# micahvista/VACmap

Measured on AMD Instinct MI355X. Metric: aligned Gbp/s (whole node) + reads/s, 15 kb ONT-shape reads vs hg38-size ref, 1/2/4/8 MI355X, higher is better.
Workload: dtype i16/i32 DP + f64 chains

## Files before the change

include/vacmapx.h:

```cpp
#ifndef VACMAPX_H
#define VACMAPX_H
#include <stdint.h>
#ifdef __cplusplus
extern "C" {
#endif

typedef enum vm_status {
    VM_OK = 0,
    VM_ERR_ARG = -1,
    VM_ERR_NO_DEVICE = -2,
    VM_ERR_NO_CTX = -3,
    VM_ERR_OOM = -4,
    VM_ERR_IO = -5,
    VM_ERR_HIP = -6,
    VM_ERR_UNSUPPORTED = -7,
    VM_READ_RAISED = -10,
    VM_READ_CAPACITY = -20,
    VM_READ_FASTPATH = -21,
    VM_READ_UNSUPPORTED = -22
} vm_status;

enum { VM_MODE_H = 0, VM_MODE_L = 1, VM_MODE_S = 2, VM_MODE_R = 3,
       VM_MODE_ASM = 4 };

// ... 57 lines not shown
typedef struct vm_chains_out {
    int32_t* need_reverse;
    int32_t* mapq;
    double* score;
    int32_t* fast_used;
    int64_t* read_path_off;
    int64_t* path_off;
    int64_t* path_anchors;
    double* S; int64_t* P; int64_t* S_arg; int64_t* gmax; int64_t* opcount;
} vm_chains_out;
int vm_chain_global_batch(vm_ctx*, const vm_params*, int kmersize, int64_t n, const int64_t* anchors,
                          const int64_t* anchor_off, const int64_t* readlens, int want_raw, vm_chains_out* out);
void vm_chains_out_free(vm_chains_out*);

typedef struct vm_local_out {
    int32_t* status;
    int32_t* variant;
    double* score;
    int64_t* chain_off;
    int64_t* chain;
    int64_t* raw_off;
    int64_t* raw;
} vm_local_out;
int vm_local_chain_batch(vm_ctx*, const vm_index*, const vm_params*, int64_t n, const char* seqs, const int64_t* offsets,
                         const int64_t* read_path_off, const int64_t* path_off, const int64_t* path_anchors, vm_local_out* out);
void vm_local_out_free(vm_local_out*);

typedef struct vm_linked_out {
    int64_t gmax, n_hot, n_cold, opcount; double cold_max;
    double* S; int64_t* P; int64_t* S_arg_hot;
    int32_t carry_status, saved; int64_t n_carry; double* carry_S; int64_t* carry_P; int64_t* carry_rows; double carry_g_max_scores; int64_t carry_prereadloc;
} vm_linked_out;
int vm_chain_linked(vm_ctx*, int which, int kmersize, double skipcost, int maxdiff, int maxgap, int64_t n, const int64_t* rows, int64_t n_pre,
                    const double* pre_S, const int64_t* pre_P, double g_max_scores, int64_t g_max_index, int64_t prereadloc, vm_linked_out* out);
void vm_linked_out_free(vm_linked_out*);

typedef struct vm_score { int32_t match, mismatch, o1, e1, o2, e2; } vm_score;
int vm_k_cigar_batch(vm_ctx*, const vm_score*, int eqx, int64_t n, const char* t, const int64_t* t_off, const char* q,
                     const int64_t* q_off, char** cigars, int64_t** cigar_off, int32_t** scores);
int vm_k_cigar_batch_banded(vm_ctx*, const vm_score*, int eqx, int64_t n, const char* t, const int64_t* t_off, const char* q,
                            const int64_t* q_off, char** cigars, int64_t** cigar_off, int32_t** band_flag, int64_t* stats);
int vm_k_extend_batch(vm_ctx*, int match, int mismatch, int o, int e, int bw, int zdrop, int64_t n, const char* t,
                      const int64_t* t_off, const char* q, const int64_t* q_off, int32_t** t_e, int32_t** q_e, int32_t** score);
typedef struct vm_cigar_out { char* cigar; int32_t q_e, t_e, score; } vm_cigar_out;
int vm_k_cigar(vm_ctx*, const char* t, int64_t tl, const char* q, int64_t ql, const vm_score* sc, int bw, int zdrop,
               int eqx, vm_cigar_out* out);
int vm_edit_distance_batch(vm_ctx*, int64_t n, const char* q, const int64_t* q_off, const char* t, const int64_t* t_off,
                           int64_t** dist);
int64_t vm_edit_distance(vm_ctx*, const char* q, int64_t ql, const char* t, int64_t tl);
int vm_edit_distance_bound_batch(vm_ctx*, int tier, int64_t n, const char* q, const int64_t* q_off, const char* t, const int64_t* t_off,
                                 int64_t** bound);

typedef struct vm_record {
    int32_t read_idx;
    int32_t contig;
    int32_t strand;
    int32_t mapq;
    int64_t q_st, q_en;
    int64_t r_st, r_en;
    int64_t cigar_off, cigar_len;
} vm_record;

typedef struct vm_batch_stats {
    int64_t n_reads, read_bases, n_minimizers, n_hits, n_anchors, n_local_hits, n_local_anchors;
    int64_t n_segments, n_ed_problems, ed_cells, n_ext_problems, ext_cells, n_dp_problems, dp_cells;
    int64_t n_records, cigar_bytes, aligned_bases, n_unmapped, n_failed;
    int64_t dp_string_bytes;
    double ms_total;
    double ms_stage[16];
    double ms_gapfill_fill;
    double ms_gapfill_trace;
    int64_t n_gapfill_launches;
    int64_t n_ed_full;
    int64_t n_ed_tier2;
    int64_t n_ed_tier1;
    int64_t n_dp_redo;
    int64_t dp_redo_tb_bytes;
    double ms_local_seed;
    double ms_cluster;
    int64_t n_host_syncs;
    int64_t n_local_general;
    int64_t n_ext_retries;
    int64_t n_batch_retries;
} vm_batch_stats;

int vm_align_batch(vm_ctx*, const vm_index*, const vm_params*, int64_t n_reads, const char* seqs, const int64_t* offsets,
                   vm_record** recs, int64_t* n_recs, char** cigar_blob, int32_t* status_per_read, vm_batch_stats* stats);
typedef struct vm_reads vm_reads;
int vm_reads_upload(vm_ctx*, int64_t n_reads, const char* seqs, const int64_t* offsets, vm_reads** out);
int vm_reads_reupload(vm_ctx*, vm_reads*, int64_t n_reads, const char* seqs, const int64_t* offsets);
void vm_reads_free(vm_reads*);
int vm_align_resident(vm_ctx*, const vm_index*, const vm_params*, const vm_reads*, vm_record** recs, int64_t* n_recs,
                      char** cigar_blob, int32_t* status_per_read, vm_batch_stats* stats);

int vm_align_asm(vm_ctx*, const vm_index*, const vm_params* p, const char* contig, int64_t len, int64_t split_len, int64_t batch_anchors, int64_t window,
                 vm_record** recs, int64_t* n_recs, char** cigar_blob, int32_t* status);

int vm_align_trace(vm_ctx*, const vm_index*, const vm_params*, int64_t n_reads, const char* seqs, const int64_t* offsets, int stage,
                   int64_t** rows, int64_t** row_off);

typedef struct vm_sam_opts {
    int32_t md, shortcs, cigar2cg, markunbalancetra, hardclip, fakecigar;
    const char* rg_id;
    int32_t asm_mode;
} vm_sam_opts;
int vm_sam_emit(const vm_index*, const vm_sam_opts*, int64_t n_reads, const char* names, const int64_t* name_off, const char* seqs, const int64_t* seq_off,
                const char* quals, const int64_t* qual_off, const char* comments, const int64_t* com_off, const vm_record* recs, int64_t n_recs,
                const char* cigar_blob, const int32_t* status, int nthreads, char** text, int64_t** text_off, int64_t* n_lines, int64_t* n_skipped);
int64_t vm_blob_gather(const char* blob, const int64_t* off, const int64_t* idx, int64_t n, char* out, int64_t* out_off);
int64_t vm_blob_write_parts_mmap(int fd, int64_t file_off, const char* const* blobs, const int64_t* const* offs, const int32_t* part, const int64_t* idx, int64_t n, int nthreads);
int64_t vm_blob_gather_parts(const char* const* blobs, const int64_t* const* offs, const int32_t* part, const int64_t* idx, int64_t n, char* out);
void* vm_pinned_alloc(int64_t bytes, int device);
void vm_pinned_free(void* p);
int64_t vm_blob_write_parts(int fd, const char* const* blobs, const int64_t* const* offs, const int32_t* part, const int64_t* idx, int64_t n);
typedef struct vm_fastx vm_fastx;
int vm_fastx_open(const char* path, vm_fastx** out);
int vm_fastx_open_range(const char* path, int64_t begin, int64_t end, vm_fastx** out);
void vm_fastx_close(vm_fastx*);
int64_t vm_fastx_read(vm_fastx*, int64_t max_reads, int64_t max_bases, char** names, int64_t** name_off, char** seqs, int64_t** seq_off, char** quals,
                      int64_t** qual_off, char** comments, int64_t** com_off);

typedef struct vm_bam_writer vm_bam_writer;
int vm_bam_writer_create(vm_ctx*, const char* sam_header, int64_t len, vm_bam_writer** out);
void vm_bam_writer_free(vm_bam_writer*);
int vm_bam_header(vm_bam_writer*, char** out, int64_t* n);
int vm_bam_encode(vm_bam_writer*, const char* sam, int64_t len, char** out, int64_t* n);
int vm_bam_compress_parts(vm_bam_writer*, const char* const* blobs, const int64_t* const* offs, const int32_t* part, const int64_t* idx, int64_t n,
                          char** out, int64_t* n_out);
int vm_bgzf_compress(vm_ctx*, const void* in, int64_t n, char** out, int64_t* n_out);

int vm_bgzf_decompress(vm_ctx*, const void* in, int64_t n, char** out, int64_t* n_out);
typedef struct vm_bam_reader vm_bam_reader;
int vm_bam_reader_open(vm_ctx*, const char* path, vm_bam_reader** out);
int64_t vm_bam_reader_read(vm_bam_reader*, int64_t max_reads, int64_t max_bases, char** names, int64_t** name_off, char** seqs, int64_t** seq_off, char** quals,
                           int64_t** qual_off, char** comments, int64_t** com_off);
int vm_bam_reader_stats(const vm_bam_reader*, double* out, int n);
void vm_bam_reader_close(vm_bam_reader*);

typedef struct vm_bam_sorter vm_bam_sorter;
int vm_bam_sorter_create(vm_bam_writer*, int64_t chunk_bytes, vm_bam_sorter** out);
void vm_bam_sorter_free(vm_bam_sorter*);
int vm_bam_sorter_add_parts(vm_bam_sorter*, const char* const* blobs, const int64_t* const* offs, const int32_t* part, const int64_t* idx, int64_t n,
                            char** out, int64_t* n_out);
int vm_bam_sorter_plan(vm_bam_sorter*, const char* const* run_paths, int64_t n_paths, int64_t file_base, int64_t* n_chunks);
int vm_bam_sorter_chunk(vm_bam_sorter*, int64_t k, char** out, int64_t* n_out);
int vm_bam_sorter_index(vm_bam_sorter*, char** out, int64_t* n_out);

int64_t vm_table(vm_ctx*, int which, void** data);

void vm_free(void*);
const char* vm_last_error(void);
const char* vm_version(void);

#ifdef __cplusplus
}
#endif
#endif
```

vacmap_amd/csrc/k_dp.hip:

```cpp
#include "vmx_device.h"
#include "vmx_kernels.h"

__device__ __forceinline__ int vmx_tcode(uint8_t c) { return c < 4 ? (int)c : 6; }


__global__ void k_encode(const char* __restrict__ in, uint8_t* __restrict__ out, int64_t n) {
    int64_t i = (int64_t)blockIdx.x * blockDim.x + threadIdx.x;
    int64_t stride = (int64_t)gridDim.x * blockDim.x;
    for (; i < n; i += stride) out[i] = vmx_code((uint8_t)in[i]);
}

#define VMX_EXT_RING 512
__global__ void __launch_bounds__(64) k_extend(const uint8_t* __restrict__ tcodes, const int64_t* __restrict__ t_off,
                                               const uint8_t* __restrict__ qcodes, const int64_t* __restrict__ q_off, int n_prob,
                                               int match, int mismatch, int o, int e, int bw_in, int zdrop,
                                               int32_t* __restrict__ out_te, int32_t* __restrict__ out_qe, int32_t* __restrict__ out_sc, const int32_t* __restrict__ n_ptr) {
    if (n_ptr) n_prob = *n_ptr;
    __shared__ int sH[3][VMX_EXT_RING];
    __shared__ int sE[2][VMX_EXT_RING];
    __shared__ int sF[2][VMX_EXT_RING];
    const int lane = vmx_lane();
    const int RM = VMX_EXT_RING - 1;
    for (int p = blockIdx.x; p < n_prob; p += gridDim.x) {
        const uint8_t* T = tcodes + t_off[p];
// ... 278 lines not shown
        const uint8_t* T = tcodes + pr.t_off;
        const uint8_t* Q = qcodes + pr.q_off;
        const int tl = vmx_uniform_i32(pr.tl), ql = vmx_uniform_i32(pr.ql);
        const bool trivial = tl == 0 || ql == 0;
        if (trivial && lane == 0) out_score[p] = (tl + ql) ? vmx_gap_open_row(tl + ql, o1, e1, o2, e2) : 0;
        if (!SCORE && !trivial && lane == 0) out_score[p] = flag_value;
        uint8_t* tb = vmx_tb_ptr(tb_pool, redo_pool, pr.tb_off);
        int32_t* bH = bnd_pool + pr.bnd_off;
        int32_t* bE1 = bH + (ql + 1);
        int32_t* bE2 = bE1 + (ql + 1);
        const bool pk = !trivial && VMX_DP16_OK(tl, ql);
        const int W = ql + 63;
        const int nstr = (trivial || pk) ? 0 : (tl + 63) >> 6;
        int outH = 0;
        for (int s = 0; s < nstr; ++s) {
            const int i = s * 64 + lane + 1;
            const int ti = i <= tl ? (int)T[i - 1] : 4;
            int Hleft = vmx_gap_open_row(i, o1, e1, o2, e2);
            int F1 = VMX_NEG, F2 = VMX_NEG;
            int Hdiag = (i - 1 == 0) ? 0 : vmx_gap_open_row(i - 1, o1, e1, o2, e2);
            int outE1 = VMX_NEG, outE2 = VMX_NEG;
            outH = 0;
            int qc_cur = 4;
            int sH = 0, sE1 = 0, sE2 = 0;
            const bool store_bnd = s + 1 < nstr;
            uint8_t* tbs = tb + (size_t)s * (size_t)W * 64 + lane;
#define VMX_GF_STEP(PRED)                                                                                             \
            {                                                                                                         \
                const int upH = vmx_shr1_in(outH, cH), upE1 = vmx_shr1_in(outE1, cE1), upE2 = vmx_shr1_in(outE2, cE2); \
                qc_cur = vmx_shr1_in(qc_cur, qchunk);                                                                 \
                cH = vmx_rol1(cH); cE1 = vmx_rol1(cE1); cE2 = vmx_rol1(cE2); qchunk = vmx_rol1(qchunk);               \
                if (PRED) {                                                                                           \
                    int b = 0;                                                                                        \
                    const int a1 = upH - o1, a2 = upH - o2;                                                           \
                    if (upE1 > a1) b |= 8;                                                                            \
                    if (upE2 > a2) b |= 16;                                                                           \
                    const int e1v = (a1 > upE1 ? a1 : upE1) - e1, e2v = (a2 > upE2 ? a2 : upE2) - e2;                 \
                    const int c1 = Hleft - o1, c2 = Hleft - o2;                                                       \
                    if (F1 > c1) b |= 32;                                                                             \
                    if (F2 > c2) b |= 64;                                                                             \
                    F1 = (c1 > F1 ? c1 : F1) - e1; F2 = (c2 > F2 ? c2 : F2) - e2;                                     \
                    int h = Hdiag + ((ti == qc_cur && ti < 4) ? match : mismatch);                                    \
                    int src = 0;                                                                                      \
                    if (e1v > h) { h = e1v; src = 1; }                                                                \
                    if (F1 > h) { h = F1; src = 3; }                                                                  \
                    if (e2v > h) { h = e2v; src = 2; }                                                                \
                    if (F2 > h) { h = F2; src = 4; }                                                                  \
                    tbs[(size_t)t * 64] = (uint8_t)(b | src);                                                         \
                    Hdiag = upH; Hleft = h;                                                                           \
                    outH = h; outE1 = e1v; outE2 = e2v;                                                               \
                }                                                                                                     \
                if (store_bnd) {                                                                                      \
                    sH = vmx_ror1(lane == 63 ? outH : sH); sE1 = vmx_ror1(lane == 63 ? outE1 : sE1); sE2 = vmx_ror1(lane == 63 ? outE2 : sE2); \
                    const int j63 = t - 62;                                         \
                    if (j63 >= 1 && j63 <= ql && ((j63 & 63) == 0 || j63 == ql)) {                                    \
                        const int col = j63 - lane;                      \
                        if (col > ((j63 - 1) & ~63)) { bH[col] = sH; bE1[col] = sE1; bE2[col] = sE2; }                \
                    }                                                                                                 \
                }                                                                                                     \
            }
            for (int t0 = 0; t0 < W; t0 += 64) {
                const int jj = t0 + lane;
                int qchunk = jj < ql ? (int)Q[jj] : 4;
                int cH = 0, cE1 = VMX_NEG, cE2 = VMX_NEG;
                if (jj + 1 <= ql) {
                    if (s == 0) cH = vmx_gap_open_row(jj + 1, o1, e1, o2, e2);
                    else { cH = bH[jj + 1]; cE1 = bE1[jj + 1]; cE2 = bE2[jj + 1]; }
                }
                if (t0 >= 64 && t0 + 64 <= ql) {
                    for (int tt = 0; tt < 64; ++tt) { const int t = t0 + tt; VMX_GF_STEP(true) }
                } else {
                    int tend = W - t0; if (tend > 64) tend = 64;
                    for (int tt = 0; tt < tend; ++tt) { const int t = t0 + tt; const int j = t - lane + 1; VMX_GF_STEP(j >= 1 && j <= ql) }
                }
            }
#undef VMX_GF_STEP
            __syncthreads();
        }
        if (!trivial && !pk && lane == ((tl - 1) & 63)) out_score[p] = outH;
        int32_t sink = 0;
        if (pk) vmx_gapfill_fill16(T, Q, tl, ql, match, mismatch, o1, e1, o2, e2, tb, bH, SCORE ? &out_score[p] : &sink, lane);
}

template <bool SCORE>
__device__ __forceinline__ void vmx_gapfill_fill_body(const uint8_t* __restrict__ tcodes, const uint8_t* __restrict__ qcodes,
                                                     const vmx_dp_prob* __restrict__ probs, int n_prob, int match, int mismatch,
                                                     int o1, int e1, int o2, int e2, uint8_t* __restrict__ tb_pool,
                                                     int32_t* __restrict__ bnd_pool, int32_t* __restrict__ out_score,
                                                     const int32_t* __restrict__ order, int32_t* __restrict__ counter,
                                                     int32_t* __restrict__ redo_list = nullptr, int32_t* __restrict__ redo_cnt = nullptr, int redo_pass = 0,
                                                     uint8_t* __restrict__ redo_pool = nullptr) {
    const int lane = vmx_lane();
    int static_next = 4 * (int)blockIdx.x;
    if (redo_pass) {
        n_prob = redo_cnt[0]; order = redo_list; counter = redo_cnt + 1;
        while (true) {
            int q; { int v = 0; if (lane == 0) v = atomicAdd(redo_cnt + 2, 1); q = vmx_bcast0(v); }
            if (q >= n_prob) break;
            const int p = order[q];
            const int tl = probs[p].tl, ql = probs[p].ql;
            if (VMX_REDO_PK(tl, ql)) vmx_gapfill_fill_one<SCORE>(tcodes, qcodes, probs, p, match, mismatch, o1, e1, o2, e2, tb_pool, bnd_pool, out_score, lane, VMX_PK_FLAG, redo_pool);
        }
    }
    while (true) {
        int q0;
        if (order) { int v = 0; if (lane == 0) v = atomicAdd(counter, 4); q0 = vmx_bcast0(v); }
        else { q0 = static_next; static_next += 4 * (int)gridDim.x; }
        if (q0 >= n_prob) break;
        const int qg = q0 + (lane >> 4);
        const int pg = qg < n_prob ? (order ? order[qg] : qg) : -1;
        bool x4 = false, skip = false;
        {
            vmx_dp_prob pr; pr.tl = 0; pr.ql = 0; pr.t_off = 0; pr.q_off = 0; pr.tb_off = 0; pr.bnd_off = 0;
            if (pg >= 0) pr = probs[pg];
            skip = redo_pass && pg >= 0 && VMX_REDO_PK(pr.tl, pr.ql);
            x4 = pg >= 0 && !skip && pr.tl > 0 && pr.ql > 0 && VMX_DP16X4_OK(pr.tl, pr.ql);
            if (!SCORE && x4 && (lane & 15) == 0) out_score[pg] = 0;
            if (__any(x4))
                vmx_gapfill_fill16x4<SCORE>(tcodes + pr.t_off, qcodes + pr.q_off, x4 ? pr.tl : 0, x4 ? pr.ql : 0, match, mismatch, o1, e1, o2, e2, vmx_tb_ptr(tb_pool, redo_pool, pr.tb_off),
                                            bnd_pool + pr.bnd_off, &out_score[pg < 0 ? 0 : pg], lane);
        }
        for (int gk = 0; gk < 4; ++gk) {
            const int p = vmx_readlane(pg, 16 * gk);
            if (p < 0 || vmx_readlane((int)(x4 || skip), 16 * gk)) continue;
            vmx_gapfill_fill_one<SCORE>(tcodes, qcodes, probs, p, match, mismatch, o1, e1, o2, e2, tb_pool, bnd_pool, out_score, lane, 0, redo_pool);
        }
    }
}

__device__ __forceinline__ void vmx_gapfill_ad_pass(const uint8_t* __restrict__ tcodes, const uint8_t* __restrict__ qcodes, vmx_dp_prob* __restrict__ probs, int n_prob,
                                                   int match, int mismatch, int o1, int e1, int o2, int e2, uint8_t* __restrict__ tb_pool, int32_t* __restrict__ bnd_pool,
                                                   int32_t* __restrict__ out_score, const int32_t* __restrict__ order, const int32_t* __restrict__ range, int32_t* __restrict__ counter,
                                                   int32_t* __restrict__ redo_list, int32_t* __restrict__ redo_cnt, int ad_pct, unsigned long long* __restrict__ redo_bytes,
                                                   unsigned long long redo_cap, int tb_by_ns) {
    const int lane = vmx_lane();
    const int pct = ad_pct & 0xffff, pct_min = (ad_pct >> 16) & 0xffff;
    const bool ad_ok = vmx_ad_scores_ok(match, mismatch, o1, e1, o2, e2);
    const int n_head = range[0] < n_prob ? range[0] : n_prob;
    bool head = n_head > 0;
    while (true) {
        int pX = -1, pY = -1;
        if (head) {
            int q; { int v = 0; if (lane == 0) v = atomicAdd(counter + 1, 1); q = vmx_bcast0(v); }
            if (q >= n_head) { head = false; continue; }
            if (lane < 16) pX = order[q];
        } else {
            int q0; { int v = 0; if (lane == 0) v = atomicAdd(counter, 8); q0 = n_head + vmx_bcast0(v); }
            if (q0 >= n_prob) break;
            const int qX = q0 + 2 * (lane >> 4), qY = qX + 1;
            if (qX < n_prob) pX = order[qX];
            if (qY < n_prob) pY = order[qY];
        }
        vmx_dp_prob prX, prY;
        prX.tl = 0; prX.ql = 0; prX.t_off = 0; prX.q_off = 0; prX.tb_off = 0; prY = prX;
        if (pX >= 0) prX = probs[pX];
        if (pY >= 0) prY = probs[pY];
        const bool x4X = pX >= 0 && prX.tl > 0 && prX.ql > 0 && VMX_DP16X4_OK(prX.tl, prX.ql), x4Y = pY >= 0 && prY.tl > 0 && prY.ql > 0 && VMX_DP16X4_OK(prY.tl, prY.ql);
        const int nsX = x4X && ad_ok ? vmx_ad_ns(prX.tl, prX.ql, match, o1, e1, o2, e2, pct, pct_min) : 0, nsY = x4Y && ad_ok ? vmx_ad_ns(prY.tl, prY.ql, match, o1, e1, o2, e2, pct, pct_min) : 0;
        const int ns = vmx_uniform_i32(vmx_wave_max_i32(nsX > nsY ? nsX : nsY));
        bool keepX = false, keepY = false, triedX = false, triedY = false;
        if (ns > 0) {
            int dloX = 0, dloY = 0;
            const bool fitX = !tb_by_ns || VMX_AD_W(nsX) == VMX_AD_W(ns), fitY = !tb_by_ns || VMX_AD_W(nsY) == VMX_AD_W(ns);
            const int gX = (nsX > 0 && fitX) ? vmx_ad_geom(prX.tl, prX.ql, ns, &dloX) : 0, gY = (nsY > 0 && fitY) ? vmx_ad_geom(prY.tl, prY.ql, ns, &dloY) : 0;
            const int tlX = gX > 0 ? prX.tl : 0, qlX = gX > 0 ? prX.ql : 0, tlY = gY > 0 ? prY.tl : 0, qlY = gY > 0 ? prY.ql : 0;
            int scX = 0, scY = 0;
#define VMX_AD_RUN(NSV) vmx_gapfill_fill_ad<NSV>(tcodes + prX.t_off, qcodes + prX.q_off, tlX, qlX, dloX, tb_pool + prX.tb_off, tcodes + prY.t_off, qcodes + prY.q_off, tlY, qlY, dloY, \
                                                 tb_pool + prY.tb_off, match, mismatch, o1, e1, o2, e2, lane, scX, scY)
            if (ns == 1) VMX_AD_RUN(1); else if (ns == 2) VMX_AD_RUN(2); else if (ns == 3) VMX_AD_RUN(3); else VMX_AD_RUN(4);
#undef VMX_AD_RUN
            triedX = gX > 0; triedY = gY > 0;
            keepX = gX > 0 && vmx_ad_proven(scX, prX.tl, prX.ql, gX, match, o1, e1, o2, e2);
            keepY = gY > 0 && vmx_ad_proven(scY, prY.tl, prY.ql, gY, match, o1, e1, o2, e2);
        }
        if ((lane & 15) == 0) {
            if (x4X) {
                out_score[pX] = keepX ? VMX_AD_FLAG + ns : 0;
                if (!keepX) {
                    if (triedX) atomicAdd(redo_cnt + 3, 1);
                    const unsigned long long need = (unsigned long long)VMX_REDO_TB_BYTES(prX.tl, prX.ql), at = atomicAdd(redo_bytes, need);
                    if (at + need > redo_cap) { probs[pX].tl = 0; probs[pX].ql = 0; probs[pX].tb_off = 0; }
                    else { probs[pX].tb_off = -(int64_t)at - 1; redo_list[atomicAdd(redo_cnt, 1)] = pX; }
                }
            }
            if (x4Y) {
                out_score[pY] = keepY ? VMX_AD_FLAG + ns : 0;
                if (!keepY) {
                    if (triedY) atomicAdd(redo_cnt + 3, 1);
                    const unsigned long long need = (unsigned long long)VMX_REDO_TB_BYTES(prY.tl, prY.ql), at = atomicAdd(redo_bytes, need);
                    if (at + need > redo_cap) { probs[pY].tl = 0; probs[pY].ql = 0; probs[pY].tb_off = 0; }
                    else { probs[pY].tb_off = -(int64_t)at - 1; redo_list[atomicAdd(redo_cnt, 1)] = pY; }
                }
            }
        }
        for (int gk = 0; gk < 8; ++gk) {
            const int p = vmx_readlane((gk & 1) ? pY : pX, 16 * (gk >> 1));
            if (p < 0 || vmx_readlane((int)((gk & 1) ? x4Y : x4X), 16 * (gk >> 1))) continue;
            vmx_gapfill_fill_one<false>(tcodes, qcodes, probs, p, match, mismatch, o1, e1, o2, e2, tb_pool, bnd_pool, out_score, lane);
        }
    }
}

__global__ void __launch_bounds__(64) k_gapfill_fill(const uint8_t* __restrict__ tcodes, const uint8_t* __restrict__ qcodes,
                                                     const vmx_dp_prob* __restrict__ probs, int n_prob, int match, int mismatch,
                                                     int o1, int e1, int o2, int e2, uint8_t* __restrict__ tb_pool,
                                                     int32_t* __restrict__ bnd_pool, int32_t* __restrict__ out_score,
                                                     const int32_t* __restrict__ order, int32_t* __restrict__ counter) {
    vmx_gapfill_fill_body<true>(tcodes, qcodes, probs, n_prob, match, mismatch, o1, e1, o2, e2, tb_pool, bnd_pool, out_score, order, counter);
}
__global__ void __launch_bounds__(64, 4) k_gapfill_fill_ns(const uint8_t* __restrict__ tcodes, const uint8_t* __restrict__ qcodes,
                                                        vmx_dp_prob* __restrict__ probs, int n_prob, int match, int mismatch,
                                                        int o1, int e1, int o2, int e2, uint8_t* __restrict__ tb_pool,
                                                        int32_t* __restrict__ bnd_pool, int32_t* __restrict__ out_score,
                                                        const int32_t* __restrict__ order, const int32_t* __restrict__ range, int32_t* __restrict__ counter,
                                                        int32_t* __restrict__ redo_list, int32_t* __restrict__ redo_cnt, int redo_pass, int ad_pct,
                                                        uint8_t* __restrict__ redo_pool, unsigned long long* __restrict__ redo_bytes, const int32_t* __restrict__ n_ptr,
                                                        unsigned long long redo_cap, int tb_by_ns) {
    if (n_ptr) n_prob = *n_ptr;
    if (redo_pass) vmx_gapfill_fill_body<false>(tcodes, qcodes, probs, n_prob, match, mismatch, o1, e1, o2, e2, tb_pool, bnd_pool, out_score, order, counter, redo_list, redo_cnt, 1, redo_pool);
    else vmx_gapfill_ad_pass(tcodes, qcodes, probs, n_prob, match, mismatch, o1, e1, o2, e2, tb_pool, bnd_pool, out_score, order, range, counter, redo_list, redo_cnt, ad_pct, redo_bytes, redo_cap, tb_by_ns);
}

__global__ void k_gapfill_trace(const uint8_t* __restrict__ tcodes, const uint8_t* __restrict__ qcodes,
                                const vmx_dp_prob* __restrict__ probs, int n_prob, int eqx, const uint8_t* __restrict__ tb_pool,
                                uint32_t* __restrict__ run_pool, char* __restrict__ cig_pool, int32_t* __restrict__ cig_len,
                                const int32_t* __restrict__ band_flag, const uint8_t* __restrict__ redo_pool, int spread, int32_t* __restrict__ cig_q,
                                const int32_t* __restrict__ n_ptr) {
    VMX_SETPRIO(3);
    if (n_ptr) n_prob = *n_ptr;
    const int gt = (int)(blockIdx.x * blockDim.x + threadIdx.x);
    if (spread > 1 && gt % spread) return;
    int p = spread > 1 ? gt / spread : gt;
    if (p >= n_prob) return;
    const vmx_dp_prob pr = probs[p];
    const uint8_t* T = tcodes + pr.t_off;
    const uint8_t* Q = qcodes + pr.q_off;
    const int tl = pr.tl, ql = pr.ql;
    const uint8_t* tb = vmx_tb_ptr(tb_pool, redo_pool, pr.tb_off);
    uint32_t* runs = run_pool + pr.run_off;
    char* cig = cig_pool + pr.cig_off;
    bool x4 = tl > 0 && ql > 0 && VMX_DP16X4_OK(tl, ql);
    bool pk = !x4 && tl > 0 && ql > 0 && VMX_DP16_OK(tl, ql);
    const int flag = (x4 && band_flag != nullptr) ? band_flag[p] : 0;
    const int ns = flag > VMX_AD_FLAG ? flag - VMX_AD_FLAG : 0;
    if (flag == VMX_PK_FLAG) { x4 = false; pk = true; }
    int dlo = 0;
    if (ns) vmx_ad_geom(tl, ql, ns, &dlo);
    const int AW = ns ? VMX_AD_W(ns) : 4;
    const int W = x4 ? VMX_X4_W(ql) : ql + (pk ? 127 : 63);
    int nruns = 0; int cur_op = -1; uint32_t cur_len = 0;
#define VMX_EMIT(op)                                                                   \
    do {                                                                               \
        if ((op) == cur_op) ++cur_len;                                                 \
        else { if (cur_op >= 0) runs[nruns++] = (cur_len << 8) | (uint32_t)cur_op; cur_op = (op); cur_len = 1; } \
    } while (0)
    int i = tl, j = ql, state = 0;
    while (i > 0 && j > 0) {
        int b;
        if (ns && state == 0) {
            const int x = (j - i) - dlo, l = x / (2 * ns), k = (x - 2 * ns * l) >> 1;
            const uint8_t* cell = tb + VMX_AD_TB_OFF_W(0, l, AW) + k;
            const int s0 = i + j - 1;
            int m = i < j ? i : j; if (m > 8) m = 8;
            uint8_t bb[8], ta[8], qa[8];
#pragma unroll
            for (int u = 0; u < 8; ++u) if (u < m) { bb[u] = cell[VMX_AD_TB_OFF_W(s0 - 2 * u, 0, AW)]; if (eqx) { ta[u] = T[i - 1 - u]; qa[u] = Q[j - 1 - u]; } }
            int u = 0;
#pragma unroll
            for (int v = 0; v < 8; ++v) {
                if (v == u && v < m) {
                    const int src = bb[v] & 7;
                    if (src == 0) { int op = 'M'; if (eqx) op = (ta[v] == qa[v] && ta[v] < 4) ? '=' : 'X'; VMX_EMIT(op); --i; --j; ++u; }
                    else state = src;
                }
            }
            if (state == 0) continue;
        }
        if (ns) { const int x = (j - i) - dlo, l = x / (2 * ns), k = (x - 2 * ns * l) >> 1; b = tb[VMX_AD_TB_OFF_W(i + j - 1, l, AW) + k]; }
        else if (x4) { const int s = (i - 1) >> 5, r = (i - 1) & 31, t = (j - 1) + r; b = tb[(((size_t)s * (size_t)W + (size_t)t) * 16 + (r >> 1)) * 2 + (r & 1)]; }
        else if (pk) { const int s = (i - 1) >> 7, r = (i - 1) & 127, t = (j - 1) + r; b = tb[(((size_t)s * (size_t)W + (size_t)t) * 64 + (r >> 1)) * 2 + (r & 1)]; }
        else { const int s = (i - 1) >> 6, l = (i - 1) & 63, t = (j - 1) + l; b = tb[((size_t)s * (size_t)W + (size_t)t) * 64 + l]; }
        if (state == 0) {
            int src = b & 7;
            if (src == 0) {
                int op = 'M';
                if (eqx) { uint8_t a = T[i - 1], c = Q[j - 1]; op = (a == c && a < 4) ? '=' : 'X'; }
                VMX_EMIT(op); --i; --j;
            } else state = src;
        } else if (state <= 2) {
            VMX_EMIT('D');
            int ext = state == 1 ? (b >> 3) & 1 : (b >> 4) & 1;
            --i; if (!ext) state = 0;
        } else {
            VMX_EMIT('I');
            int ext = state == 3 ? (b >> 5) & 1 : (b >> 6) & 1;
            --j; if (!ext) state = 0;
        }
    }
    while (i > 0) { VMX_EMIT('D'); --i; }
    while (j > 0) { VMX_EMIT('I'); --j; }
    if (cur_op >= 0) runs[nruns++] = (cur_len << 8) | (uint32_t)cur_op;
#undef VMX_EMIT
    int w = 0; long long qsum = 0;
// ... 13 lines not shown
```

vacmap_amd/csrc/vmx_align.hip:

```cpp
#include "vmx_host.h"
#include "vmx_stage.h"
#include "vmx_select.h"
#include "vmx_ext_state.h"
#include "vmx_round.h"
#include <algorithm>
#include <cstdio>
#include <cstdlib>
#include <cstddef>
#include <cstring>
#include <string>

using namespace vmx;

__global__ void k_orient(const uint8_t* codes, const int64_t* roff, const double* gscore, int n_reads, uint8_t* ocodes);
__global__ void k_scan_i64(const int64_t* in, int64_t* out, int64_t n, int pow2_round);
__global__ void k_ext_phase(vmx_ext_args A, int phase);
__global__ void k_ed_anchor_bound(vmx_ext_args A, const int32_t* probread, const uint8_t* qpool, const int64_t* qoff, const uint8_t* tpool, const int64_t* toff,
                                  int64_t* ub_out);
__global__ void k_desc_lens(const vmx_pair_desc* desc, const int32_t* n_prob, int64_t* tl, int64_t* ql);
__global__ void k_gather(const vmx_pair_desc* desc, const int32_t* n_prob, const int32_t* prob_read, const uint8_t* ocodes, const int64_t* roff,
                         const uint8_t* ref, const int64_t* t_off, const int64_t* q_off, uint8_t* tpool, uint8_t* qpool, int64_t pool_cap, vmx_ext_read* er);
__global__ void k_prob_owner(const vmx_ext_read* er, int n_reads, int use_dp, int32_t* prob_read);
__global__ void k_dp_sizes(const vmx_pair_desc* desc, const int32_t* n_prob, int64_t* tb_sz, int64_t* bnd_sz, int64_t* run_sz, int64_t* cig_sz);
__global__ void k_dp_table(const vmx_pair_desc* desc, const int32_t* n_prob, const int64_t* t_off, const int64_t* q_off, const int64_t* tb_off,
// ... 76 lines not shown
    const HostTables& T = host_tables();
    {
        if (prm->global_maxdiff > 62) { set_error("global_maxdiff > 62 unsupported"); return VM_ERR_UNSUPPORTED; }
        std::vector<double> gap(64, 0.0);
        for (int g = 1; g <= prm->global_maxdiff; ++g) gap[g] = (0.01 * k * g + 0.5 * T.log2int[g]);
        VMX_TRY(vmx_push(c, B.gap, gap.data(), 64));
    }
    if (rmode == 1) { VMX_TRY(B.fp.reserve(8 * (size_t)(tot + 1))); VMX_TRY(B.pp.reserve(8 * (size_t)(tot + 1))); }
    constexpr int NB = 10;
    const int caps[NB] = {384, 512, 768, 1024, 1536, 2048, 3072, 4096, 8192, 13056};
    std::vector<int32_t> lists[NB + 1];
    std::vector<int64_t> asm_long;
    static const int gc_lds_env = [] { const char* e = getenv("VMX_GC_LDS_MAX"); return e ? atoi(e) : -1; }();
    const int gc_lds_max = gc_lds_env >= 0 ? gc_lds_env : VMX_CHAIN_LDS_MAX_SHARED;
    const bool rows_kernel = vmx_chain_rows_on() && rmode != 2;
    for (int64_t r = 0; r < n; ++r) {
        int64_t m = h_aoff[r + 1] - h_aoff[r]; const int64_t L = h_roff[r + 1] - h_roff[r];
        if (m <= 2) continue;
        if (prm->mode == VM_MODE_ASM && L >= 500000) { asm_long.push_back(r); continue; }
        if ((double)m / (double)L > 5.0) continue;
        int bk = NB; for (int q = 0; q < NB; ++q) if (m <= caps[q] && caps[q] <= gc_lds_max) { bk = q; break; }
        if (rows_kernel) bk = NB;
        lists[bk].push_back((int32_t)r);
    }
    {
        std::vector<int32_t> rl; int64_t rl_off[NB + 2];
        for (int q = 0; q <= NB; ++q) {
            std::stable_sort(lists[q].begin(), lists[q].end(), [&](int32_t a, int32_t b) { return h_aoff[a + 1] - h_aoff[a] > h_aoff[b + 1] - h_aoff[b]; });
            rl_off[q] = (int64_t)rl.size(); rl.insert(rl.end(), lists[q].begin(), lists[q].end());
        }
        VMX_TRY(vmx_push(c, B.rl, rl.data(), rl.size()));
        VMX_HIP(hipMemsetAsync(B.gmax.p, 0xff, 8 * (size_t)n, c->stream));
        { static const int64_t kUnsupported = -4; for (int64_t r : asm_long) VMX_HIP(hipMemcpyAsync(B.gmax.as<int64_t>() + r, &kUnsupported, 8, hipMemcpyHostToDevice, c->stream)); }
#ifndef VMX_EMU
        VMX_HIP(hipFuncSetAttribute((const void*)k_chain_global, hipFuncAttributeMaxDynamicSharedMemorySize, (int)((size_t)caps[NB - 1] * VMX_GC_BYTES_PER_ANCHOR + 64)));
#endif
        vmx_fork fk(c);
        for (int q = NB; q >= 0; --q) {
            int cnt = (int)lists[q].size(); if (!cnt) continue;
            int cap = q < NB ? caps[q] : 0; size_t shmem = (size_t)cap * VMX_GC_BYTES_PER_ANCHOR + 64;
            if (rows_kernel) {
                hipLaunchKernelGGL((vmx_chain_rows_win3() ? k_chain_global_rows_w3 : k_chain_global_rows), dim3((unsigned)((cnt + 3) / 4)), dim3(64), 0, fk.next(), B.sorted.as<vmx_anchor>(), B.aoff.as<int64_t>(),
                                   B.rl.as<int32_t>() + rl_off[q], cnt, c->tables, B.gap.as<double>(), prm->global_skipcost, prm->global_maxdiff, 1000, B.S.as<double>(),
                                   B.P.as<int32_t>(), B.SA.as<int32_t>(), B.cov.as<uint8_t>(), B.gmax.as<int64_t>(), B.opc.as<int64_t>(), rmode, B.fp.as<double>(), B.pp.as<double>(),
                                   vmx_chain_dbg());
                continue;
            }
            hipLaunchKernelGGL(k_chain_global, dim3((unsigned)cnt), dim3(64), shmem, fk.next(), B.sorted.as<vmx_anchor>(), B.aoff.as<int64_t>(),
                               B.rl.as<int32_t>() + rl_off[q], cnt, cap, c->tables, B.gap.as<double>(), prm->global_skipcost, prm->global_maxdiff, 1000, B.S.as<double>(),
                               B.P.as<int32_t>(), B.SA.as<int32_t>(), B.cov.as<uint8_t>(), B.gmax.as<int64_t>(), B.opc.as<int64_t>(), rmode, B.fp.as<double>(), B.pp.as<double>());
        }
        fk.join();
        vmx_chain_dbg_report(c->stream);
        VMX_TRY(B.si.reserve(4 * (size_t)(tot + 1))); VMX_TRY(B.tg.reserve(8 * (size_t)(tot + 1))); VMX_TRY(B.cntp.reserve(4 * (size_t)(total_bases + 50 * n + 64)));
        hipLaunchKernelGGL(k_chain_global_fast, dim3((unsigned)n), dim3(64), 0, c->stream, B.sorted.as<vmx_anchor>(), B.aoff.as<int64_t>(), (int)n, d_roff, c->tables,
                           B.gap.as<double>(), prm->global_skipcost, prm->global_maxdiff, 1000, B.S.as<double>(), B.P.as<int32_t>(), B.SA.as<int32_t>(), B.cov.as<uint8_t>(),
                           B.si.as<int32_t>(), B.tg.as<int64_t>(), B.cntp.as<int32_t>(), B.gmax.as<int64_t>(), d_ran, rmode, B.fp.as<double>(), B.pp.as<double>());
    }
    VMX_TRY(B.scr.reserve((size_t)stt + 64)); VMX_TRY(vmx_push(c, B.soff, soff.data(), (size_t)n + 1));
    VMX_TRY(B.res.reserve(16 * (size_t)(n + 2) + 64));
    double* d_gscore; int32_t* d_mapq; int32_t* d_np; vmx_res_ptrs(B, n, &d_gscore, &d_mapq, &d_np);
    VMX_TRY(B.plen.reserve(4 * (size_t)(tot + 1))); VMX_TRY(B.prow.reserve(sizeof(vmx_anchor) * (size_t)(tot + 1)));
    return vmx_launch_chain_select(c, n, h_aoff.data(), B.sellist, B.sorted.as<vmx_anchor>(), B.aoff.as<int64_t>(), B.lens.as<int64_t>(), B.S.as<double>(), B.P.as<int32_t>(), B.SA.as<int32_t>(),
                                   B.gmax.as<int64_t>(), B.flip.as<int32_t>(), prm->mode, B.scr.as<char>(), B.soff.as<int64_t>(), d_mapq, d_gscore, d_np, B.plen.as<int32_t>(), B.prow.as<vmx_anchor>());
}

void vmx_gapfill_chunk(vm_ctx* c, vmx_batch_bufs& B, const vm_score& sc, int ad_pct, int eqx, int p0, int64_t pn, const int32_t* n_ptr, int64_t tb_off0,
                       int32_t* ctl, int32_t* redo_list, int64_t redo_cap, hipEvent_t* ke) {
    int fill_waves = 16;
    if (const char* e = getenv("VMX_FILL_WAVES")) { const int v = atoi(e); if (v >= 1 && v <= 32) fill_waves = v; }
    static const int tr_spread = [] { const char* e = getenv("VMX_TRACE_SPREAD"); const int v = e ? atoi(e) : 1; return v >= 1 && v <= 64 ? v : 1; }();
    int32_t* d_range = ctl; int32_t* d_cnt = ctl + 4; int32_t* d_redo_cnt = ctl + 12;
    unsigned long long* d_redo_bytes = (unsigned long long*)(ctl + 16); int32_t* scratch = ctl + 32;
    uint8_t* tb_base = B.tb.as<uint8_t>() - tb_off0;
    vmx_dp_prob* probs = B.dptab.as<vmx_dp_prob>() + p0; int32_t* score = B.dpscore.as<int32_t>() + p0;
    const unsigned Gs = (unsigned)std::max<int64_t>(1, std::min<int64_t>((pn + 1023) / 1024, (int64_t)c->num_cu * 2));
    hipLaunchKernelGGL(k_size_hist, dim3(Gs), dim3(256), 0, c->stream, B.dpsz[0].as<int64_t>() + p0, n_ptr, (int64_t)((1LL << 42) - 1), scratch);
    hipLaunchKernelGGL(k_size_scatter, dim3(Gs), dim3(256), 0, c->stream, B.dpsz[0].as<int64_t>() + p0, n_ptr, (const int32_t*)scratch, scratch + 257, B.order.as<int32_t>(), d_range, d_cnt);
    if (ke) (void)hipEventRecord(ke[0], c->stream);
    {
        vmx_lowprio lp(c);
        hipLaunchKernelGGL(k_gapfill_fill_ns, dim3((unsigned)std::max<int64_t>(1, std::min<int64_t>(pn, (int64_t)c->num_cu * fill_waves))), dim3(64), 0, lp.stream(), B.tpool.as<uint8_t>(), B.qpool.as<uint8_t>(),
                           probs, (int)pn, sc.match, sc.mismatch, sc.o1, sc.e1, sc.o2, sc.e2, tb_base, B.bnd.as<int32_t>(), score, B.order.as<int32_t>(), d_range, d_cnt,
                           redo_list, d_redo_cnt, 0, ad_pct, (uint8_t*)nullptr, d_redo_bytes, n_ptr, (unsigned long long)redo_cap, 1);
        lp.join();
    }
    hipLaunchKernelGGL(k_gapfill_fill_ns, dim3((unsigned)std::max<int64_t>(1, std::min<int64_t>(pn, (int64_t)c->num_cu * 4))), dim3(64), 0, c->stream, B.tpool.as<uint8_t>(), B.qpool.as<uint8_t>(),
                       probs, (int)pn, sc.match, sc.mismatch, sc.o1, sc.e1, sc.o2, sc.e2, tb_base, B.bnd.as<int32_t>(), score, B.order.as<int32_t>(), d_range, d_cnt,
                       redo_list, d_redo_cnt, 1, ad_pct, B.tbredo.as<uint8_t>(), d_redo_bytes, n_ptr, (unsigned long long)redo_cap, 1);
    if (ke) (void)hipEventRecord(ke[1], c->stream);
    hipLaunchKernelGGL(k_gapfill_trace, dim3((unsigned)std::max<int64_t>(1, (pn * tr_spread + 63) / 64)), dim3(64), 0, c->stream, B.tpool.as<uint8_t>(), B.qpool.as<uint8_t>(), probs, (int)pn, eqx,
                       tb_base, B.run.as<uint32_t>(), B.cig.as<char>(), B.ciglen.as<int32_t>() + p0, score, B.tbredo.as<uint8_t>(), tr_spread, B.cigq.as<int32_t>() + p0, n_ptr);
    if (ke) (void)hipEventRecord(ke[2], c->stream);
}

#define LAUNCH1D(kernel, n, ...) hipLaunchKernelGGL(kernel, dim3((unsigned)std::max<int64_t>(1, std::min<int64_t>(((n) + 255) / 256, 4096))), dim3(256), 0, c->stream, __VA_ARGS__)

__global__ void k_ext_geometry(const int32_t* la_cnt, const int64_t* roff, int n, int mul, int tmask, long long tdiv, long long capA, long long capS, long long capB, int64_t* coff3,
                               int64_t* soff2, int64_t* bloboff, int64_t* tot);
__global__ void k_scan_part_dev(const int64_t* in, int64_t* part, const int32_t* n_ptr);
__global__ void k_scan_apply_dev(const int64_t* in, int64_t* out, const int64_t* part_off, const int32_t* n_ptr);
__global__ void k_scan_part(const int64_t* in, int64_t* part, int64_t n, int64_t chunk);
__global__ void k_scan_apply(const int64_t* in, int64_t* out, const int64_t* part_off, int64_t n, int64_t chunk);

static int dev_scan(vm_ctx* c, vmx_batch_bufs& B, const int64_t* in, int64_t* out, int64_t n) {
    if (n <= 16384) { hipLaunchKernelGGL(k_scan_i64, dim3(1), dim3(256), 0, c->stream, in, out, n, 0); return 0; }
    int64_t chunk = (n + 511) / 512; const int64_t nb = (n + chunk - 1) / chunk;
    VMX_TRY(B.scanpart.reserve(8 * (size_t)(nb + 2))); VMX_TRY(B.scanoff.reserve(8 * (size_t)(nb + 2)));
    hipLaunchKernelGGL(k_scan_part, dim3((unsigned)nb), dim3(256), 0, c->stream, in, B.scanpart.as<int64_t>(), n, chunk);
    hipLaunchKernelGGL(k_scan_i64, dim3(1), dim3(256), 0, c->stream, B.scanpart.as<int64_t>(), B.scanoff.as<int64_t>(), nb, 0);
    hipLaunchKernelGGL(k_scan_apply, dim3((unsigned)nb), dim3(256), 0, c->stream, in, out, B.scanoff.as<int64_t>(), n, chunk);
    return 0;
}

static int dev_scan_dev(vm_ctx* c, vmx_batch_bufs& B, const int64_t* in, int64_t* out, const int32_t* n_ptr) {
    const int nb = 512;
    VMX_TRY(B.scanpart.reserve(8 * (size_t)(nb + 2))); VMX_TRY(B.scanoff.reserve(8 * (size_t)(nb + 2)));
    hipLaunchKernelGGL(k_scan_part_dev, dim3(nb), dim3(256), 0, c->stream, in, B.scanpart.as<int64_t>(), n_ptr);
    hipLaunchKernelGGL(k_scan_i64, dim3(1), dim3(256), 0, c->stream, B.scanpart.as<int64_t>(), B.scanoff.as<int64_t>(), (int64_t)nb, 0);
    hipLaunchKernelGGL(k_scan_apply_dev, dim3(nb), dim3(256), 0, c->stream, in, out, B.scanoff.as<int64_t>(), n_ptr);
    return 0;
}

static const vm_score gf_score = {2, -4, 4, 2, 24, 1};

static int ext_gather_round(vm_ctx* c, vmx_batch_bufs& B, const vm_index_view& ix, int64_t n, const uint8_t* d_ocodes, const int64_t* d_roff, int cur, int redo_only,
                            int64_t round_cap, int64_t pool_cap, int stat_slot, bool dp, int64_t tb_limit, const int64_t* caps = nullptr, int64_t* plan_out = nullptr, int ad_pct = 0) {
    (void)n; (void)redo_only; (void)round_cap;
    if (!B.roundpart.p) { VMX_TRY(B.roundpart.reserve(8 * (size_t)VMX_ROUND_PART_WORDS)); VMX_HIP(hipMemsetAsync(B.roundpart.p, 0, 8 * (size_t)VMX_ROUND_PART_WORDS, c->stream)); }
    vmx_round_args R; memset(&R, 0, sizeof R);
    R.desc = B.desc[cur].as<vmx_pair_desc>(); R.n_prob = c->rc_cur;
    R.off[0] = B.toff.as<int64_t>(); R.off[1] = B.qoff.as<int64_t>();
    R.part = B.roundpart.as<int64_t>(); R.stat_out = B.statblk.as<int32_t>() + stat_slot; R.epoch = ++c->round_epoch;
    if (dp) {
        for (int i = 0; i < 4; ++i) R.off[2 + i] = B.dpoff[i].as<int64_t>();
        R.tb_size = B.dpsz[0].as<int64_t>(); R.probs = B.dptab.as<vmx_dp_prob>(); R.plan_out = plan_out; R.tb_limit = tb_limit;
        if (caps) for (int i = 0; i < 4; ++i) R.cap[i] = caps[i];
        R.ad_on = 1; R.ad_match = gf_score.match; R.ad_o1 = gf_score.o1; R.ad_e1 = gf_score.e1; R.ad_o2 = gf_score.o2; R.ad_e2 = gf_score.e2; R.ad_pct = ad_pct;
        hipLaunchKernelGGL(k_round_prep<true>, dim3(VMX_ROUND_WGS), dim3(256), 0, c->stream, R);
    } else
        hipLaunchKernelGGL(k_round_prep<false>, dim3(VMX_ROUND_WGS), dim3(256), 0, c->stream, R);
    hipLaunchKernelGGL(k_gather, dim3((unsigned)((int64_t)c->num_cu * 8)), dim3(256), 0, c->stream, B.desc[cur].as<vmx_pair_desc>(), c->rc_cur,
                       B.probread.as<int32_t>(), d_ocodes, d_roff, ix.codes, B.toff.as<int64_t>(), B.qoff.as<int64_t>(), B.tpool.as<uint8_t>(), B.qpool.as<uint8_t>(), pool_cap,
                       B.er.as<vmx_ext_read>());
    return 0;
}

struct vmx_seg_trace { int stage; std::vector<int64_t> rows, off; };
int vmx_asm_resolve_ties(vm_ctx* c, const vm_index* mi, int64_t n, const std::vector<int64_t>& h_roff, const std::vector<int64_t>& h_aoff, const uint8_t* d_codes,
                         const vmx_anchor* d_sorted, const double* d_S, const int32_t* d_P, const int32_t* d_SA, const int64_t* d_gmax, const int32_t* d_flip,
                         int32_t* d_mapq, double* d_gscore, int32_t* d_np, int32_t* d_plen, vmx_anchor* d_prow, std::vector<int32_t>& status_override);
int vmx_align_batch_asm_mixed(vm_ctx* c, const vm_index* mi, const vm_params* prm, int64_t n, const char* seqs, const int64_t* offsets, vm_record** recs, int64_t* n_recs,
                              char** cigar_blob, int32_t* status_per_read, vm_batch_stats* stats);
int align_device(vm_ctx* c, const vm_index* mi, const vm_params* prm, int64_t n, const uint8_t* d_codes, const int64_t* d_roff, const std::vector<int64_t>& h_roff,
                 vm_record** recs, int64_t* n_recs, char** cigar_blob, int32_t* status_per_read, vm_batch_stats* stats, vmx_seg_trace* trace = nullptr, const vmx_preset* preset = nullptr);

#define VMX_EXT_EXACT_INTERNAL (-9002)
#define VMX_RETRY_BATCH (-9003)
#define VMX_EXT_SHORT_INTERNAL (-9001)
static int align_device_once(vm_ctx* c, const vm_index* mi, const vm_params* prm, int64_t n, const uint8_t* d_codes, const int64_t* d_roff, const std::vector<int64_t>& h_roff,
                             vm_record** recs, int64_t* n_recs, char** cigar_blob, int32_t* status_per_read, vm_batch_stats* stats, vmx_seg_trace* trace, const vmx_preset* preset);
__global__ void k_side_codes(const uint8_t* __restrict__ codes, const int64_t* __restrict__ roff, const int32_t* __restrict__ pick, const int64_t* __restrict__ soff, int n, uint8_t* __restrict__ out) {
    for (int j = blockIdx.x; j < n; j += gridDim.x) {
        const int64_t a = roff[pick[j]], len = roff[pick[j] + 1] - a; const uint8_t* s = codes + a; uint8_t* d = out + soff[j];
        for (int64_t i = threadIdx.x; i < len; i += blockDim.x) d[i] = s[i];
    }
}
int align_device(vm_ctx* c, const vm_index* mi, const vm_params* prm, int64_t n, const uint8_t* d_codes, const int64_t* d_roff, const std::vector<int64_t>& h_roff,
                 vm_record** recs, int64_t* n_recs, char** cigar_blob, int32_t* status_per_read, vm_batch_stats* stats, vmx_seg_trace* trace, const vmx_preset* preset) {
    c->ext_mul = 1;
    std::vector<int32_t> status((size_t)n + 1, 0);
    vm_batch_stats st; memset(&st, 0, sizeof st);
// ... 317 lines not shown
            const bool all_tiers = c->force_exact || always_all;
            hipLaunchKernelGGL(k_ed_flag, dim3((unsigned)std::min<int64_t>((cnt + 255) / 256, 1024)), dim3(256), 0, c->stream, B.dpsz[1].as<int64_t>(), B.qoff.as<int64_t>(), B.toff.as<int64_t>(),
                               c->rc_cur, prm->maxdivergence, B.dpsz[0].as<int64_t>(), B.edout.as<int64_t>(), d_n1, 1, B.probread.as<int32_t>(), all_tiers ? (vmx_ext_read*)nullptr : B.er.as<vmx_ext_read>());
            if (all_tiers) {
            vmx_size_order_wide(c, B.dpsz[0].as<int64_t>(), c->rc_cur, cnt, (int64_t)VMX_ED_LONG, B.order.as<int32_t>(), d_range, d_cnt, B.szh.as<int32_t>());
            hipLaunchKernelGGL(k_ed_banded4, dim3((unsigned)std::min<int64_t>((cnt + 3) / 4, (int64_t)c->num_cu * 16)), dim3(64), 0, c->stream, B.qpool.as<uint8_t>(), B.qoff.as<int64_t>(),
                               B.tpool.as<uint8_t>(), B.toff.as<int64_t>(), B.order.as<int32_t>(), d_range, d_cnt + 2, B.dpsz[1].as<int64_t>());
            hipLaunchKernelGGL(k_ed_flag, dim3((unsigned)std::min<int64_t>((cnt + 255) / 256, 1024)), dim3(256), 0, c->stream, B.dpsz[1].as<int64_t>(), B.qoff.as<int64_t>(), B.toff.as<int64_t>(),
                               c->rc_cur, prm->maxdivergence, B.dpsz[0].as<int64_t>(), B.edout.as<int64_t>(), d_n2, 0, (const int32_t*)nullptr, (vmx_ext_read*)nullptr);
            vmx_size_order_wide(c, B.dpsz[0].as<int64_t>(), c->rc_cur, cnt, (int64_t)VMX_ED_LONG, B.order.as<int32_t>(), d_range, d_cnt, B.szh.as<int32_t>());
            hipLaunchKernelGGL(k_ed_banded, dim3((unsigned)std::min<int64_t>(cnt, (int64_t)c->num_cu * 16)), dim3(64), 0, c->stream, B.qpool.as<uint8_t>(), B.qoff.as<int64_t>(),
                               B.tpool.as<uint8_t>(), B.toff.as<int64_t>(), B.order.as<int32_t>(), d_range, d_cnt + 2, B.dpsz[1].as<int64_t>());
            hipLaunchKernelGGL(k_ed_flag, dim3((unsigned)std::min<int64_t>((cnt + 255) / 256, 1024)), dim3(256), 0, c->stream, B.dpsz[1].as<int64_t>(), B.qoff.as<int64_t>(), B.toff.as<int64_t>(),
                               c->rc_cur, prm->maxdivergence, B.dpsz[0].as<int64_t>(), B.edout.as<int64_t>(), d_nfull, 0, (const int32_t*)nullptr, (vmx_ext_read*)nullptr);
            vmx_size_order_wide(c, B.dpsz[0].as<int64_t>(), c->rc_cur, cnt, (int64_t)VMX_ED_LONG, B.order.as<int32_t>(), d_range, d_cnt, B.szh.as<int32_t>());
            for (int which = 0; which < 2; ++which)
                hipLaunchKernelGGL(k_edit_distance, dim3((unsigned)std::min<int64_t>(cnt, ed_wgs * (which == 0 ? 1 : 2))), dim3(which == 0 ? 64 * VMX_ED_WAVES : 256), 0, c->stream,
                                   B.qpool.as<uint8_t>(), B.qoff.as<int64_t>(), B.tpool.as<uint8_t>(), B.toff.as<int64_t>(),
                                   B.carry.as<int8_t>() + (which ? (size_t)VMX_ED_WAVES * (size_t)carry_stride * (size_t)ed_wgs : 0), B.order.as<int32_t>(), d_range, d_cnt, which,
                                   B.edout.as<int64_t>(), carry_stride, B.oflow.as<int32_t>());
            }
        }
        cur ^= 1;
    }
    VMX_HIP(hipEventRecord(ev[nev++], c->stream));
    phase(1); VMX_TRY(ext_round(0));
    phase(2); VMX_TRY(ext_round(0));
    phase(3); VMX_TRY(ext_round(0));
    phase(4); VMX_TRY(ext_round(0));
    VMX_HIP(hipEventRecord(ev[nev++], c->stream));
    phase(5); VMX_TRY(gapfill(0));
    VMX_HIP(hipEventRecord(ev[nev++], c->stream));
    int64_t test_side_every = 0; if (const char* e = getenv("VMX_TEST_SIDE_EVERY")) test_side_every = atoll(e);
    static const bool always_pass1 = getenv("VMX_FORCE_PASS1") != nullptr;
    const bool do_pass1 = c->run_pass1 || always_pass1;
    if (do_pass1) {
        A.redo_only = 1;
        phase(3); phase(4); phase(5); VMX_TRY(gapfill(1));
        A.redo_only = 0;
    }
    VMX_HIP(hipEventRecord(ev[nev++], c->stream));

    VMX_TRY(B.dpsz[0].reserve(8 * (size_t)(n + 2))); VMX_TRY(B.dpsz[1].reserve(8 * (size_t)(n + 2))); VMX_TRY(B.dpoff[0].reserve(8 * (size_t)(n + 2))); VMX_TRY(B.dpoff[1].reserve(8 * (size_t)(n + 2)));
    hipLaunchKernelGGL(k_res_sizes, dim3(gridR), dim3(64), 0, c->stream, B.er.as<vmx_ext_read>(), B.rec.as<vm_record>(), B.soff2.as<int64_t>(), (int)n, B.dpsz[0].as<int64_t>(), B.dpsz[1].as<int64_t>());
    hipLaunchKernelGGL(k_scan_i64, dim3(1), dim3(256), 0, c->stream, B.dpsz[0].as<int64_t>(), B.dpoff[0].as<int64_t>(), n, 0);
    hipLaunchKernelGGL(k_scan_i64, dim3(1), dim3(256), 0, c->stream, B.dpsz[1].as<int64_t>(), B.dpoff[1].as<int64_t>(), n, 0);
    int64_t nr = 0, nb = 0; int32_t oflow = 0;
    int32_t n_full = 0, n_t2 = 0, n_t1 = 0;
    int64_t fin[14]; int64_t hstat[8];
    hipLaunchKernelGGL(k_final_scalars, dim3(1), dim3(1), 0, c->stream, B.dpoff[0].as<int64_t>() + n, B.dpoff[1].as<int64_t>() + n, B.oflow.as<int32_t>(), B.qrange.as<int32_t>() + 8,
                       B.statblk.as<int32_t>(), B.statblk.as<int64_t>() + 32);
    VMX_TRY(B.totals.reserve(sizeof(vm_record) * (size_t)(cS + 1))); VMX_TRY(B.dupd.reserve((size_t)cB + 64));
    hipLaunchKernelGGL(k_res_pack, dim3((unsigned)std::min<int64_t>(n, (int64_t)c->num_cu * 8)), dim3(64), 0, c->stream, B.er.as<vmx_ext_read>(), B.rec.as<vm_record>(), B.blob.as<char>(),
                       B.soff2.as<int64_t>(), B.bloboff.as<int64_t>(), (int)n, B.dpoff[0].as<int64_t>(), B.dpoff[1].as<int64_t>(), B.totals.as<vm_record>(), B.dupd.as<char>());
    int64_t g_nr = std::min<int64_t>(cS, (int64_t)(c->res_rec_per_read * 2.0 * (double)n) + 256), g_nb = std::min<int64_t>(cB, (int64_t)(c->res_blob_per_base * 1.5 * (double)total_bases) + 65536);
    if (c->res_rec_per_read <= 0.0) { g_nr = 0; g_nb = 0; }
    std::vector<vmx_ext_read> er((size_t)n);
    std::vector<int64_t> h_gmax((size_t)n);
    *recs = (vm_record*)malloc(sizeof(vm_record) * (size_t)std::max<int64_t>(g_nr, 1)); *cigar_blob = (char*)malloc((size_t)std::max<int64_t>(g_nb, 1));
    struct OutGuard { vm_record** r; char** b; bool keep = false; ~OutGuard() { if (!keep) { free(*r); free(*b); *r = nullptr; *b = nullptr; } } } out_guard{recs, cigar_blob};
    if (!*recs || !*cigar_blob) { set_error("out of host memory"); return VM_ERR_OOM; }
    VMX_TRY(vmx_fetch(c, fin, B.statblk.as<int64_t>() + 32, 14));
    int64_t geo[8] = {0, 0, 0, 0, 0, 0, 0, 0};
    if (fast_local) VMX_TRY(vmx_fetch(c, geo, B.geotot.p, 6));
    std::vector<int32_t> h_ctl(gfctl_bytes / 4);
    VMX_TRY(vmx_fetch(c, h_ctl.data(), B.gfctl.p, h_ctl.size()));
    VMX_TRY(vmx_fetch(c, er.data(), B.er.p, (size_t)n)); VMX_TRY(vmx_fetch(c, h_gmax.data(), B.gmax.p, (size_t)n));
    VMX_TRY(vmx_fetch(c, *recs, B.totals.p, (size_t)g_nr)); VMX_TRY(vmx_fetch(c, *cigar_blob, B.dupd.p, (size_t)g_nb));
    VMX_HIP(hipEventRecord(ev[nev++], c->stream));
    VMX_HIP(vmx_stream_sync(c));
    VMX_HIP(hipGetLastError());
    nr = fin[0]; nb = fin[1]; oflow = (int32_t)fin[2]; n_full = (int32_t)fin[3]; n_t2 = (int32_t)fin[4]; n_t1 = (int32_t)fin[5];
    if (fast_local) {
        st.n_local_anchors = geo[4];
        if (geo[5] > 0 || geo[3] + 16 > c->geo_cap[3]) c->geo_valid = false;
        if (geo[5] && getenv("VMX_DBG_POOLS")) fprintf(stderr, "[pools] extend stage: %lld read(s) did not fit the history-sized pools (run again alone)\n", (long long)geo[5]);
    }
    {
        bool again = false; int64_t need_max = 0, ad_failed = 0;
        for (int pass = 0; pass < 2; ++pass)
            for (int q = 0; q < gf_chunks[pass]; ++q) {
                const int32_t* ctl = h_ctl.data() + (size_t)(pass * (VMX_MAX_CHUNKS + 1) + q) * VMX_GF_SLOT;
                unsigned long long rb = 0; memcpy(&rb, ctl + 16, 8);
                st.n_dp_redo += ctl[12]; st.dp_redo_tb_bytes += (int64_t)rb; st.dp_cells += (int64_t)rb; ad_failed += ctl[15];
                need_max = std::max<int64_t>(need_max, (int64_t)rb);
            }
        c->redo_need_max = std::max<long long>(c->redo_need_max, need_max);
        if (need_max > gf_redo_cap) { again = true; if (getenv("VMX_DBG_POOLS")) fprintf(stderr, "[pools] gap fill: a chunk's second launch needs %.3f GB of traceback space, the pool held %.3f: running the batch again\n", need_max / 1e9, gf_redo_cap / 1e9); }
        if (again) return VMX_RETRY_BATCH;
        if (!ad_pinned && !c->force_exact && st.n_dp_problems >= 2000) {
            const double f = (double)ad_failed / (double)st.n_dp_problems;
            std::lock_guard<std::mutex> g(ad_m);
            if (ad_cur == adr.pct) {
                if (f > 0.03 && adr.pct < 100) { adr.pct = std::min(100, adr.pct + 10); adr.floor = adr.pct; adr.hold = 256; }
                else if (adr.hold > 0) { if (--adr.hold == 0) adr.floor = 20; }
                else if (f < 0.025 && adr.pct > adr.floor) adr.pct = std::max(adr.floor, adr.pct - (f < 0.01 ? 20 : 10));
            }
        }
    }
    for (int i = 0; i < 8; ++i) hstat[i] = fin[6 + i];
    st.n_segments = hstat[0]; st.n_ed_problems = hstat[0]; st.n_ext_problems = (int64_t)hstat[1] + hstat[2] + hstat[3] + hstat[4];
    st.n_ed_full = n_full; st.n_ed_tier2 = n_t2; st.n_ed_tier1 = n_t1;
    if (oflow) { set_error("extend stage: a per-batch work pool overflowed"); return VM_ERR_OOM; }
    if (nr > g_nr || nb > g_nb) {
        if (nr > g_nr) { vm_record* p2 = (vm_record*)realloc(*recs, sizeof(vm_record) * (size_t)nr); if (!p2) { set_error("out of host memory"); return VM_ERR_OOM; } *recs = p2;
                         VMX_TRY(vmx_fetch(c, *recs + g_nr, B.totals.as<vm_record>() + g_nr, (size_t)(nr - g_nr))); }
        if (nb > g_nb) { char* p2 = (char*)realloc(*cigar_blob, (size_t)nb); if (!p2) { set_error("out of host memory"); return VM_ERR_OOM; } *cigar_blob = p2;
                         VMX_TRY(vmx_fetch(c, *cigar_blob + g_nb, B.dupd.as<char>() + g_nb, (size_t)(nb - g_nb))); }
        VMX_HIP(vmx_stream_sync(c));
    }
    if (n > 0 && total_bases > 0) { c->res_rec_per_read = std::max(c->res_rec_per_read, (double)nr / (double)n); c->res_blob_per_base = std::max(c->res_blob_per_base, (double)nb / (double)total_bases); }
    for (int64_t r = 0; r < n; ++r) {
        int stt2 = er[r].status == VMX_EXT_CAPACITY_DEV ? VMX_EXT_SHORT_INTERNAL : (er[r].status == VMX_EXT_NEED_EXACT_DEV ? VMX_EXT_EXACT_INTERNAL : er[r].status);
        if (fast_local && (er[r].status == VM_READ_CAPACITY_DEV || er[r].status == VM_READ_BANDFALL_DEV)) stt2 = VMX_EXT_EXACT_INTERNAL;
        if (stt2 == 0 && !do_pass1 && er[r].active && er[r].redo == 1 && er[r].pass == 1) stt2 = VMX_EXT_EXACT_INTERNAL;
        if (stt2 == 0 && test_side_every > 0 && !c->force_exact && r % test_side_every == 0) stt2 = VMX_EXT_EXACT_INTERNAL;
        if (h_gmax[r] == -2 && (h_aoff[r + 1] - h_aoff[r]) > 2) stt2 = VM_READ_RAISED;
        if (h_gmax[r] == -4) stt2 = VM_READ_UNSUPPORTED;
        if (!asm_override.empty() && asm_override[(size_t)r] != 0) stt2 = asm_override[(size_t)r];
        if (rmode == 1 && (h_aoff[r + 1] - h_aoff[r]) <= 2) stt2 = VM_READ_RAISED;
        if (status_per_read) status_per_read[r] = stt2;
        if (stt2 != 0) { st.n_failed++; continue; }
        if (er[r].nrec == 0) st.n_unmapped++;
    }
    for (int64_t i = 0; i < nr; ++i) { st.aligned_bases += (*recs)[i].q_en - (*recs)[i].q_st; st.cigar_bytes += (*recs)[i].cigar_len; }
    *n_recs = nr; st.n_records = nr;
    float ms = 0;
    hipEventElapsedTime(&ms, ev[0], ev[nev - 1]); st.ms_total = ms;
    for (int i = 1; i < nev && i < 16; ++i) { hipEventElapsedTime(&ms, ev[i - 1], ev[i]); st.ms_stage[i - 1] = ms; }
    if ((c->kev_set & 1) && hipEventElapsedTime(&ms, c->kev[0], c->kev[1]) == hipSuccess) st.ms_local_seed = ms;
    if ((c->kev_set & 2) && hipEventElapsedTime(&ms, c->kev[2], c->kev[3]) == hipSuccess) st.ms_cluster = ms;
    st.n_host_syncs = c->n_syncs; st.n_local_general = c->n_bandfall;
    st.ms_stage[14] = (float)((c->sync_wait_ns + download_wait_ns()) * 1e-6);
    st.ms_stage[15] = (float)((std::chrono::duration_cast<std::chrono::nanoseconds>(std::chrono::steady_clock::now().time_since_epoch()).count() - c->call_t0_ns) * 1e-6);
    for (int pass = 0; pass < 2; ++pass)
        for (int q = 0; q < c->n_gev[pass]; ++q) {
            hipEvent_t* ke = c->gev + 24 * pass + 3 * q;
            if (hipEventElapsedTime(&ms, ke[0], ke[1]) == hipSuccess) st.ms_gapfill_fill += ms;
            if (hipEventElapsedTime(&ms, ke[1], ke[2]) == hipSuccess) st.ms_gapfill_trace += ms;
            st.n_gapfill_launches++;
        }
    if (stats) *stats = st;
    if (getenv("VMX_DBG_POOLS")) {
        const DevBuf* bb = (const DevBuf*)&B; size_t tot = 0;
        for (size_t i = 0; i < sizeof(B) / sizeof(DevBuf); ++i) { tot += bb[i].cap; if (bb[i].cap > ((size_t)128 << 20)) fprintf(stderr, "[pools] batch[%zu] %.2f GB\n", i, bb[i].cap / 1e9); }
        fprintf(stderr, "[pools] batch bufs total %.2f GB\n", tot / 1e9);
        const DevBuf* lb = (const DevBuf*)&L; size_t lt = 0; const size_t nl = (size_t)((const char*)&L.la_pool_rows - (const char*)&L) / sizeof(DevBuf);
        for (size_t i = 0; i < nl; ++i) { lt += lb[i].cap; if (lb[i].cap > ((size_t)128 << 20)) fprintf(stderr, "[pools] local[%zu] %.2f GB\n", i, lb[i].cap / 1e9); }
        fprintf(stderr, "[pools] local bufs total %.2f GB\n", lt / 1e9);
        fprintf(stderr, "[pools] process so far: %lld first allocations, %lld re-allocations, %.3f s in hipFree + hipMalloc\n", (long long)vmx::devbuf_stats().first.load(),
                (long long)vmx::devbuf_stats().grows.load(), vmx::devbuf_stats().ns.load() * 1e-9);
    }
    if (stats) *stats = st;
    out_guard.keep = true;
    return VM_OK;
}

template <class RunOne>
static int align_in_sub_batches(int64_t n, const int64_t* offsets, int64_t max_bases, RunOne run_one, vm_record** recs, int64_t* n_recs, char** cigar_blob, vm_batch_stats* stats) {
    if (n <= VMX_MAX_BATCH_READS && offsets[n] - offsets[0] <= max_bases) {
        const int rc = run_one(0, n, recs, n_recs, cigar_blob, stats);
        if (rc != VM_ERR_OOM || n <= 1) return rc;
        free(*recs); free(*cigar_blob);
    }
    *recs = nullptr; *n_recs = 0; *cigar_blob = nullptr;
    std::vector<vm_record> all; std::string blob;
    vm_batch_stats tot; memset(&tot, 0, sizeof tot);
    std::vector<std::pair<int64_t, int64_t>> work;
    for (int64_t a = 0; a < n;) {
        int64_t b = a + 1;
        while (b < n && b - a < VMX_MAX_BATCH_READS && offsets[b + 1] - offsets[a] <= max_bases) ++b;
        work.emplace_back(a, b); a = b;
    }
    for (size_t wi = 0; wi < work.size(); ++wi) {
        const int64_t a = work[wi].first, b = work[wi].second;
        vm_record* r = nullptr; int64_t nr = 0; char* cb = nullptr; vm_batch_stats st;
        const int rc = run_one(a, b, &r, &nr, &cb, &st);
        if (rc == VM_ERR_OOM && b - a > 1) {
            free(r); free(cb);
            vmx::devbuf_retired().flush();
            const int64_t mid = a + (b - a) / 2;
            work[wi] = std::make_pair(a, mid); work.insert(work.begin() + (std::ptrdiff_t)wi + 1, std::make_pair(mid, b));
            --wi; continue;
        }
        if (rc < 0) { free(r); free(cb); return rc; }
        int64_t bl = 0; for (int64_t i = 0; i < nr; ++i) bl = std::max(bl, r[i].cigar_off + r[i].cigar_len);
        for (int64_t i = 0; i < nr; ++i) { vm_record x = r[i]; x.read_idx += (int32_t)a; x.cigar_off += (int64_t)blob.size(); all.push_back(x); }
        blob.append(cb, (size_t)bl); blob.push_back('\0');
        free(r); free(cb);
        {
            int64_t* d = (int64_t*)&tot; const int64_t* s2 = (const int64_t*)&st;
            for (size_t i = 0; i < offsetof(vm_batch_stats, ms_total) / 8; ++i) d[i] += s2[i];
            tot.ms_total += st.ms_total; for (int i = 0; i < 16; ++i) tot.ms_stage[i] += st.ms_stage[i];
            tot.ms_gapfill_fill += st.ms_gapfill_fill; tot.ms_gapfill_trace += st.ms_gapfill_trace; tot.n_gapfill_launches += st.n_gapfill_launches;
            tot.n_ed_full += st.n_ed_full; tot.n_ed_tier2 += st.n_ed_tier2; tot.n_ed_tier1 += st.n_ed_tier1;
            tot.n_dp_redo += st.n_dp_redo; tot.dp_redo_tb_bytes += st.dp_redo_tb_bytes; tot.ms_local_seed += st.ms_local_seed; tot.ms_cluster += st.ms_cluster; tot.n_host_syncs += st.n_host_syncs; tot.n_local_general += st.n_local_general; tot.n_ext_retries += st.n_ext_retries; tot.n_batch_retries += st.n_batch_retries;
        }
    }
    *recs = (vm_record*)malloc(sizeof(vm_record) * std::max<size_t>(all.size(), 1)); *cigar_blob = (char*)malloc(std::max<size_t>(blob.size(), 1));
    if (!*recs || !*cigar_blob) { free(*recs); free(*cigar_blob); *recs = nullptr; *cigar_blob = nullptr; set_error("out of host memory"); return VM_ERR_OOM; }
    memcpy(*recs, all.data(), sizeof(vm_record) * all.size()); memcpy(*cigar_blob, blob.data(), blob.size());
    *n_recs = (int64_t)all.size();
    if (stats) *stats = tot;
    return VM_OK;
}
static int64_t vmx_pass_bases() {
    static const int64_t v = [] { const char* e = getenv("VMX_MAX_BATCH_BASES"); const long long x = e ? atoll(e) : 0; return x > 0 ? (int64_t)x : (int64_t)VMX_MAX_BATCH_BASES; }();
    return v;
}

extern "C" {

int vm_reads_upload(vm_ctx* c, int64_t n, const char* seqs, const int64_t* offsets, vm_reads** out) {
    *out = nullptr;
    if (!c) { set_error("no context"); return VM_ERR_NO_CTX; }
    VMX_HIP(hipSetDevice(c->device));
    vm_reads* R = new vm_reads(); R->ctx = c; R->n = n; R->h_off.assign(offsets, offsets + n + 1);
    const int64_t tot = offsets[n];
    int rc = 0;
    if ((rc = upload(R->raw, seqs, (size_t)tot, c->stream)) < 0 || (rc = R->codes.reserve((size_t)tot + 64)) < 0 || (rc = upload(R->off, offsets, (size_t)n + 1, c->stream)) < 0) { delete R; return rc; }
    if (tot) LAUNCH1D(k_encode, tot, R->raw.as<char>(), R->codes.as<uint8_t>(), tot);
    VMX_HIP(vmx_stream_sync(c));
    R->raw.release();
    *out = R;
    return VM_OK;
}
int vm_reads_reupload(vm_ctx* c, vm_reads* R, int64_t n, const char* seqs, const int64_t* offsets) {
    if (!c || !R) { set_error("no context / reads object"); return VM_ERR_NO_CTX; }
    VMX_HIP(hipSetDevice(c->device));
    R->n = n; R->h_off.assign(offsets, offsets + n + 1);
    const int64_t tot = offsets[n];
    VMX_TRY(upload(R->raw, seqs, (size_t)tot, c->stream)); VMX_TRY(R->codes.reserve((size_t)tot + 64)); VMX_TRY(upload(R->off, offsets, (size_t)n + 1, c->stream));
    if (tot) LAUNCH1D(k_encode, tot, R->raw.as<char>(), R->codes.as<uint8_t>(), tot);
    VMX_HIP(vmx_stream_sync(c));
    return VM_OK;
}
void vm_reads_free(vm_reads* R) { if (!R) return; R->raw.release(); R->codes.release(); R->off.release(); delete R; }

int vm_align_resident(vm_ctx* c, const vm_index* mi, const vm_params* prm, const vm_reads* R, vm_record** recs, int64_t* n_recs, char** cigar_blob,
                      int32_t* status_per_read, vm_batch_stats* stats) {
    if (!c) { set_error("no context"); return VM_ERR_NO_CTX; }
    VMX_HIP(hipSetDevice(c->device));
    if (R->n <= VMX_MAX_BATCH_READS && R->h_off[(size_t)R->n] <= vmx_pass_bases())
        return align_device(c, mi, prm, R->n, R->codes.as<uint8_t>(), R->off.as<int64_t>(), R->h_off, recs, n_recs, cigar_blob, status_per_read, stats);
    vmx_batch_bufs& B = *vmx_ctx_batch_bufs(c);
    auto run_one = [&](int64_t a, int64_t b, vm_record** r, int64_t* nr, char** cb, vm_batch_stats* st) -> int {
        std::vector<int64_t> h((size_t)(b - a) + 1);
        for (int64_t i = a; i <= b; ++i) h[(size_t)(i - a)] = R->h_off[(size_t)i] - R->h_off[(size_t)a];
        VMX_TRY(vmx_push(c, B.off, h.data(), h.size()));
        return align_device(c, mi, prm, b - a, R->codes.as<uint8_t>() + R->h_off[(size_t)a], B.off.as<int64_t>(), h, r, nr, cb, status_per_read ? status_per_read + a : nullptr, st);
    };
    return align_in_sub_batches(R->n, R->h_off.data(), vmx_pass_bases(), run_one, recs, n_recs, cigar_blob, stats);
}

int vm_align_trace(vm_ctx* c, const vm_index* mi, const vm_params* prm, int64_t n, const char* seqs, const int64_t* offsets, int stage, int64_t** rows, int64_t** row_off) {
    *rows = nullptr; *row_off = nullptr;
    if (!c) { set_error("no context"); return VM_ERR_NO_CTX; }
    if (stage != 0 && stage != 3 && stage != 5) { set_error("vm_align_trace: stage must be 0, 3 or 5"); return VM_ERR_ARG; }
    VMX_HIP(hipSetDevice(c->device));
    vmx_batch_bufs& B = *vmx_ctx_batch_bufs(c);
    const int64_t tot = offsets[n];
    VMX_TRY(upload(B.raw, seqs, (size_t)tot, c->stream)); VMX_TRY(B.codes.reserve((size_t)tot + 64)); VMX_TRY(upload(B.off, offsets, (size_t)n + 1, c->stream));
    if (tot) LAUNCH1D(k_encode, tot, B.raw.as<char>(), B.codes.as<uint8_t>(), tot);
    std::vector<int64_t> h_off(offsets, offsets + n + 1);
    vmx_seg_trace tr; tr.stage = stage;
    vm_record* recs = nullptr; int64_t nrec = 0; char* blob = nullptr;
    std::vector<int32_t> status((size_t)n + 1);
    const int rc = align_device(c, mi, prm, n, B.codes.as<uint8_t>(), B.off.as<int64_t>(), h_off, &recs, &nrec, &blob, status.data(), nullptr, &tr);
    free(recs); free(blob);
    if (rc < 0) return rc;
    if (tr.off.empty()) tr.off.assign((size_t)n + 1, 0);
    *rows = (int64_t*)malloc(8 * std::max<size_t>(tr.rows.size(), 1)); *row_off = (int64_t*)malloc(8 * tr.off.size());
    memcpy(*rows, tr.rows.data(), 8 * tr.rows.size()); memcpy(*row_off, tr.off.data(), 8 * tr.off.size());
    return VM_OK;
}

static int align_batch_one(vm_ctx* c, const vm_index* mi, const vm_params* prm, int64_t n, const char* seqs, const int64_t* offsets, vm_record** recs, int64_t* n_recs,
                           char** cigar_blob, int32_t* status_per_read, vm_batch_stats* stats) {
    vmx_batch_bufs& B = *vmx_ctx_batch_bufs(c);
// ... 26 lines not shown
```

vacmap_amd/csrc/vmx_capi.hip:

```cpp
#include "vmx_host.h"
#include <time.h>
#include "vmx_select.h"
#include "vmx_stage.h"
#include "vmx_round.h"
#include <algorithm>
#include <cmath>
#include <cstdlib>
#include <cstring>
#include <numeric>

namespace vmx {
static thread_local std::string g_err;
void set_error(const std::string& s) { g_err = s; }
int hip_fail(hipError_t e, const char* what, const char* file, int line) {
    g_err = std::string("HIP error: ") + hipGetErrorString(e) + " at " + what + " (" + file + ":" + std::to_string(line) + ")";
    return e == hipErrorOutOfMemory ? VM_ERR_OOM : VM_ERR_HIP;
}
}
using namespace vmx;

void vmx_ctx_free_local_bufs(vm_ctx* c);
void vmx_ctx_free_batch_bufs(vm_ctx* c);

static inline int grid_for(const vm_ctx* c, int64_t n_items, int per_cu = 8) {
// ... 447 lines not shown
                     const int64_t* q_off, char** cigars, int64_t** cigar_off, int32_t** scores) {
    if (!c) { set_error("no context"); return VM_ERR_NO_CTX; }
    if (n > 0x7fffffff) { set_error("too many problems"); return VM_ERR_ARG; }
    VMX_HIP(hipSetDevice(c->device));
    VMX_TRY(upload_encode(c, t, t_off, n, c->b[0], c->b[1], c->b[2]));
    VMX_TRY(upload_encode(c, q, q_off, n, c->b[3], c->b[4], c->b[5]));
    std::vector<vmx_dp_prob> probs((size_t)n);
    int64_t tb = 0, bnd = 0, run = 0, cig = 0;
    for (int64_t i = 0; i < n; ++i) {
        vmx_dp_prob& p = probs[i];
        p.t_off = t_off[i]; p.q_off = q_off[i]; p.tl = (int32_t)(t_off[i + 1] - t_off[i]); p.ql = (int32_t)(q_off[i + 1] - q_off[i]);
        p.tb_off = tb; p.bnd_off = bnd; p.run_off = run; p.cig_off = cig;
        tb += VMX_TB_BYTES((int64_t)p.tl, (int64_t)p.ql);
        bnd += 3 * (int64_t)(p.ql + 1); run += (int64_t)p.tl + p.ql + 2; cig += 2 * ((int64_t)p.tl + p.ql) + 16;
    }
    VMX_TRY(upload(c->b[6], probs.data(), (size_t)n, c->stream));
    VMX_TRY(c->b[7].reserve((size_t)tb + 64)); VMX_TRY(c->b[8].reserve(sizeof(int32_t) * (size_t)(bnd + 4)));
    VMX_TRY(c->b[9].reserve(sizeof(uint32_t) * (size_t)(run + 4))); VMX_TRY(c->b[10].reserve((size_t)cig + 16));
    VMX_TRY(c->b[11].reserve(sizeof(int32_t) * 2 * (size_t)(n + 1)));
    int32_t* d_score = c->b[11].as<int32_t>(); int32_t* d_len = d_score + n;
    if (n) {
        hipLaunchKernelGGL(k_gapfill_fill, dim3(grid_for(c, n, 16)), dim3(64), 0, c->stream, c->b[1].as<uint8_t>(), c->b[4].as<uint8_t>(),
                           c->b[6].as<vmx_dp_prob>(), (int)n, sc->match, sc->mismatch, sc->o1, sc->e1, sc->o2, sc->e2, c->b[7].as<uint8_t>(),
                           c->b[8].as<int32_t>(), d_score, (const int32_t*)nullptr, (int32_t*)nullptr);
        hipLaunchKernelGGL(k_gapfill_trace, dim3((unsigned)((n + 63) / 64)), dim3(64), 0, c->stream, c->b[1].as<uint8_t>(), c->b[4].as<uint8_t>(),
                           c->b[6].as<vmx_dp_prob>(), (int)n, eqx, c->b[7].as<uint8_t>(), c->b[9].as<uint32_t>(), c->b[10].as<char>(), d_len, (const int32_t*)nullptr, (const uint8_t*)nullptr, 1, (int32_t*)nullptr);
    }
    std::vector<char> hc((size_t)cig + 16); std::vector<int32_t> hl((size_t)n);
    *scores = host_alloc<int32_t>((size_t)n);
    VMX_TRY(download(hc.data(), c->b[10].p, (size_t)cig, c->stream));
    VMX_TRY(download(hl.data(), d_len, (size_t)n, c->stream));
    VMX_TRY(download(*scores, d_score, (size_t)n, c->stream));
    VMX_HIP(hipStreamSynchronize(c->stream));
    VMX_HIP(hipGetLastError());
    cigar_strings(n, probs.data(), hc.data(), hl.data(), cigars, cigar_off);
    return VM_OK;
}

int vm_k_cigar_batch_banded(vm_ctx* c, const vm_score* sc, int eqx, int64_t n, const char* t, const int64_t* t_off, const char* q,
                            const int64_t* q_off, char** cigars, int64_t** cigar_off, int32_t** band_flag, int64_t* stats) {
    if (!c) { set_error("no context"); return VM_ERR_NO_CTX; }
    if (n > 0x7fffffff) { set_error("too many problems"); return VM_ERR_ARG; }
    VMX_HIP(hipSetDevice(c->device));
    vmx_fetch_scope fetch_scope(c);
    vmx_batch_bufs& B = *vmx_ctx_batch_bufs(c);
    VMX_TRY(upload_encode(c, t, t_off, n, c->b[0], B.tpool, c->b[2]));
    VMX_TRY(upload_encode(c, q, q_off, n, c->b[3], B.qpool, c->b[5]));
    const int ad_pct = vmx_ad_pct_env();
    vmx_round_args R; memset(&R, 0, sizeof R);
    R.ad_on = 1; R.ad_match = sc->match; R.ad_o1 = sc->o1; R.ad_e1 = sc->e1; R.ad_o2 = sc->o2; R.ad_e2 = sc->e2; R.ad_pct = ad_pct;
    std::vector<vmx_dp_prob> probs((size_t)n);
    std::vector<int64_t> keys((size_t)n);
    int64_t tb = 0, bnd = 0, run = 0, cig = 0, redo = 0;
    for (int64_t i = 0; i < n; ++i) {
        vmx_dp_prob& p = probs[i];
        p.t_off = t_off[i]; p.q_off = q_off[i]; p.tl = (int32_t)(t_off[i + 1] - t_off[i]); p.ql = (int32_t)(q_off[i + 1] - q_off[i]);
        p.tb_off = tb; p.bnd_off = bnd; p.run_off = run; p.cig_off = cig;
        tb += vmx_round_tb_bytes(R, p.tl, p.ql); keys[i] = vmx_round_key(R, p.tl, p.ql);
        if (p.tl > 0 && p.ql > 0 && VMX_DP16X4_OK(p.tl, p.ql)) redo += VMX_REDO_TB_BYTES((int64_t)p.tl, (int64_t)p.ql);
        bnd += 3 * (int64_t)(p.ql + 1); run += (int64_t)p.tl + p.ql + 2; cig += 2 * ((int64_t)p.tl + p.ql) + 16;
    }
    const int32_t nn = (int32_t)n;
    VMX_TRY(upload(B.dptab, probs.data(), (size_t)n, c->stream)); VMX_TRY(upload(B.dpsz[0], keys.data(), (size_t)n, c->stream)); VMX_TRY(upload(B.chunkn, &nn, 1, c->stream));
    VMX_TRY(B.tb.reserve((size_t)tb + 64)); VMX_TRY(B.tbredo.reserve((size_t)redo + 64)); VMX_TRY(B.bnd.reserve(sizeof(int32_t) * (size_t)(bnd + 4)));
    VMX_TRY(B.run.reserve(sizeof(uint32_t) * (size_t)(run + 4))); VMX_TRY(B.cig.reserve((size_t)cig + 16));
    VMX_TRY(B.ciglen.reserve(4 * (size_t)(n + 1))); VMX_TRY(B.cigq.reserve(4 * (size_t)(n + 1))); VMX_TRY(B.dpscore.reserve(4 * (size_t)(n + 1)));
    VMX_TRY(B.order.reserve(4 * (size_t)(2 * n + 64)));
    VMX_TRY(B.gfctl.reserve(4 * VMX_GF_SLOT)); VMX_HIP(hipMemsetAsync(B.gfctl.p, 0, 4 * VMX_GF_SLOT, c->stream));
    if (n) vmx_gapfill_chunk(c, B, *sc, ad_pct, eqx, 0, n, B.chunkn.as<int32_t>(), 0, B.gfctl.as<int32_t>(), B.order.as<int32_t>() + n + 32, redo, nullptr);
    std::vector<char> hc((size_t)cig + 16); std::vector<int32_t> hl((size_t)n), flag((size_t)n), ctl(32);
    VMX_TRY(download(hc.data(), B.cig.p, (size_t)cig, c->stream));
    VMX_TRY(download(hl.data(), B.ciglen.p, (size_t)n, c->stream));
    VMX_TRY(download(flag.data(), B.dpscore.p, (size_t)n, c->stream));
    VMX_TRY(download(ctl.data(), B.gfctl.p, ctl.size(), c->stream));
    VMX_HIP(vmx_stream_sync(c));
    VMX_HIP(hipGetLastError());
    int64_t nb = 0, eligible = 0, small = 0;
    for (int64_t i = 0; i < n; ++i) {
        const bool sm = probs[i].tl > 0 && probs[i].ql > 0 && VMX_DP16X4_OK(probs[i].tl, probs[i].ql);
        if (!sm) flag[i] = 0;
        small += sm; nb += sm && flag[i] > VMX_AD_FLAG;
        eligible += sm && vmx_ad_ns(probs[i].tl, probs[i].ql, sc->match, sc->o1, sc->e1, sc->o2, sc->e2, ad_pct & 0xffff, (ad_pct >> 16) & 0xffff) > 0;
    }
    if (stats) { stats[0] = eligible; stats[1] = nb; stats[2] = ctl[12]; stats[3] = n - small; }
    if (band_flag) { *band_flag = host_alloc<int32_t>((size_t)n); memcpy(*band_flag, flag.data(), sizeof(int32_t) * (size_t)n); }
    cigar_strings(n, probs.data(), hc.data(), hl.data(), cigars, cigar_off);
    return VM_OK;
}

int vm_k_cigar(vm_ctx* c, const char* t, int64_t tl, const char* q, int64_t ql, const vm_score* sc, int bw, int zdrop, int eqx, vm_cigar_out* out) {
    memset(out, 0, sizeof(*out));
    int64_t to[2] = {0, tl}, qo[2] = {0, ql};
    if (zdrop < 0) {
        char* cg = nullptr; int64_t* co = nullptr; int32_t* s = nullptr;
        int rc = vm_k_cigar_batch(c, sc, eqx, 1, t, to, q, qo, &cg, &co, &s);
        if (rc < 0) return rc;
        out->cigar = cg; out->q_e = (int32_t)ql; out->t_e = (int32_t)tl; out->score = s[0];
        free(co); free(s);
        return VM_OK;
    }
    if (sc->o1 != sc->o2 || sc->e1 != sc->e2) { set_error("vm_k_cigar: z-drop extension needs identical gap pieces (the reference calls it with 4,4,4,4)"); return VM_ERR_UNSUPPORTED; }
    int32_t *te = nullptr, *qe = nullptr, *s = nullptr;
    int rc = vm_k_extend_batch(c, sc->match, sc->mismatch, sc->o1, sc->e1, bw, zdrop, 1, t, to, q, qo, &te, &qe, &s);
    if (rc < 0) return rc;
    out->cigar = (char*)calloc(1, 1); out->t_e = te[0]; out->q_e = qe[0]; out->score = s[0];
    free(te); free(qe); free(s);
    return VM_OK;
}

void vm_chains_out_free(vm_chains_out* o) {
    free(o->need_reverse); free(o->mapq); free(o->score); free(o->fast_used); free(o->read_path_off); free(o->path_off);
    free(o->path_anchors); free(o->S); free(o->P); free(o->S_arg); free(o->gmax); free(o->opcount);
    memset(o, 0, sizeof(*o));
}

int vm_chain_global_batch(vm_ctx* c, const vm_params* prm, int kmersize, int64_t n, const int64_t* anchors, const int64_t* aoff,
                          const int64_t* readlens, int want_raw, vm_chains_out* out) {
    memset(out, 0, sizeof(*out));
    if (!c) { set_error("no context"); return VM_ERR_NO_CTX; }
    if (prm->global_maxdiff > 62) { set_error("global_maxdiff > 62 unsupported"); return VM_ERR_UNSUPPORTED; }
    const int64_t tot = aoff[n];
    if (const int64_t bad = vmx_rows_misfit(anchors, tot); bad >= 0) {
        char msg[192]; snprintf(msg, sizeof msg, "vm_chain_global_batch: anchor row %lld does not fit the device row (l in 0 ... 65535, q and q + l in int32, s in int16)", (long long)bad);
        set_error(msg); return VM_ERR_UNSUPPORTED;
    }
    VMX_HIP(hipSetDevice(c->device));
    vmx_fetch_scope fetch_scope(c);
    vmx_batch_bufs& B = *vmx_ctx_batch_bufs(c);
    const std::vector<int64_t> h_aoff(aoff, aoff + n + 1);
    std::vector<int64_t> h_roff((size_t)n + 1, 0);
    for (int64_t r = 0; r < n; ++r) h_roff[(size_t)r + 1] = h_roff[(size_t)r] + readlens[r];
    VMX_TRY(upload(B.rows, anchors, (size_t)tot * 4, c->stream)); VMX_TRY(upload(B.aoff, aoff, (size_t)n + 1, c->stream));
    VMX_TRY(upload(B.lens, readlens, (size_t)n, c->stream)); VMX_TRY(upload(B.off, h_roff.data(), (size_t)n + 1, c->stream));
    DevBuf& d_ran = c->b[0];
    VMX_TRY(d_ran.reserve(4 * (size_t)(n + 1))); VMX_HIP(hipMemsetAsync(d_ran.p, 0, 4 * (size_t)n, c->stream));
    const int rmode = prm->mode == VM_MODE_R ? 1 : (prm->mode == VM_MODE_ASM ? 2 : 0);
    double* d_score = nullptr; int32_t* d_mapq = nullptr; int32_t* d_np = nullptr;
    if (n) {
        VMX_TRY(vmx_global_stage(c, B, prm, kmersize, n, B.off.as<int64_t>(), h_roff, h_aoff, rmode, d_ran.as<int32_t>()));
        vmx_res_ptrs(B, n, &d_score, &d_mapq, &d_np);
    }
    std::vector<int32_t> h_np((size_t)n), h_plen((size_t)tot);
    std::vector<vmx_anchor> h_prow((size_t)tot);
    out->need_reverse = host_alloc<int32_t>((size_t)n); out->mapq = host_alloc<int32_t>((size_t)n); out->score = host_alloc<double>((size_t)n);
    out->fast_used = host_alloc<int32_t>((size_t)n); out->gmax = host_alloc<int64_t>((size_t)n); out->opcount = host_alloc<int64_t>((size_t)n);
    VMX_TRY(download(out->need_reverse, B.flip.p, (size_t)n, c->stream)); VMX_TRY(download(out->mapq, d_mapq, (size_t)n, c->stream));
    VMX_TRY(download(out->score, d_score, (size_t)n, c->stream)); VMX_TRY(download(h_np.data(), d_np, (size_t)n, c->stream));
    VMX_TRY(download(h_plen.data(), B.plen.p, (size_t)tot, c->stream)); VMX_TRY(download(h_prow.data(), B.prow.p, (size_t)tot, c->stream));
    VMX_TRY(download(out->gmax, B.gmax.p, (size_t)n, c->stream)); VMX_TRY(download(out->opcount, B.opc.p, (size_t)n, c->stream));
    VMX_TRY(download(out->fast_used, d_ran.p, (size_t)n, c->stream));
    std::vector<int32_t> hP, hSA;
    if (want_raw) {
        out->S = host_alloc<double>((size_t)tot); out->P = host_alloc<int64_t>((size_t)tot); out->S_arg = host_alloc<int64_t>((size_t)tot);
        hP.resize((size_t)tot); hSA.resize((size_t)tot);
        VMX_TRY(download(out->S, B.S.p, (size_t)tot, c->stream)); VMX_TRY(download(hP.data(), B.P.p, (size_t)tot, c->stream));
        VMX_TRY(download(hSA.data(), B.SA.p, (size_t)tot, c->stream));
    }
    VMX_HIP(vmx_stream_sync(c));
    VMX_HIP(hipGetLastError());
    if (want_raw) for (int64_t i = 0; i < tot; ++i) { out->P[i] = hP[i]; out->S_arg[i] = hSA[i]; }
    for (int64_t r = 0; r < n; ++r) if (h_np[r] < 0) h_np[r] = 0;
    int64_t npaths = 0, nrows = 0;
    for (int64_t r = 0; r < n; ++r) { npaths += h_np[r]; for (int p = 0; p < h_np[r]; ++p) nrows += h_plen[aoff[r] + p]; }
    out->read_path_off = host_alloc<int64_t>((size_t)n + 1); out->path_off = host_alloc<int64_t>((size_t)npaths + 1);
    out->path_anchors = host_alloc<int64_t>((size_t)nrows * 4);
    int64_t pi = 0, ro = 0;
    for (int64_t r = 0; r < n; ++r) {
// ... 17 lines not shown
```

vacmap_amd/csrc/vmx_device.h:

```cpp
#ifndef VMX_DEVICE_H
#define VMX_DEVICE_H
#ifdef VMX_EMU
#include "hip_emu.h"
#define VMX_DYN_SHARED(type, name) type* name = (type*)hipemu::cur()->dynshared
#else
#include <hip/hip_runtime.h>
#define VMX_DYN_SHARED(type, name) extern __shared__ __attribute__((aligned(16))) type name[]
#endif
#include <stdint.h>

#define VMX_WAVE 64
#define VMX_NEG (-(1 << 28))
#define VMX_NOPRE (-9999999)

__device__ __forceinline__ int vmx_lane() { return (int)(threadIdx.x & 63); }

#ifdef VMX_EMU
__device__ __forceinline__ int vmx_shr1(int v) { return __shfl_up(v, 1); }
__device__ __forceinline__ int vmx_readlane(int v, int l) { return __shfl(v, l); }
#define VMX_SPIN_PAUSE() hipemu::yield()
#define VMX_CLOCK() 0LL
#else
__device__ __forceinline__ int vmx_shr1(int v) { return __builtin_amdgcn_update_dpp(v, v, 0x138, 0xf, 0xf, false); }
__device__ __forceinline__ int vmx_readlane(int v, int l) { return __builtin_amdgcn_readlane(v, l); }
#define VMX_SPIN_PAUSE() __builtin_amdgcn_s_sleep(1)
#define VMX_CLOCK() ((long long)wall_clock64())
#endif
#ifdef VMX_EMU
__device__ __forceinline__ int vmx_shr1_in(int v, int in) { int e = __shfl_up(v, 1); return vmx_lane() == 0 ? in : e; }
__device__ __forceinline__ int vmx_rol1(int v) { return __shfl(v, (vmx_lane() + 1) & 63); }
__device__ __forceinline__ int vmx_ror1(int v) { return __shfl(v, (vmx_lane() + 63) & 63); }
#else
__device__ __forceinline__ int vmx_shr1_in(int v, int in) { return __builtin_amdgcn_update_dpp(in, v, 0x138, 0xf, 0xf, false); }
__device__ __forceinline__ int vmx_rol1(int v) { return __builtin_amdgcn_update_dpp(v, v, 0x134, 0xf, 0xf, false); }
__device__ __forceinline__ int vmx_ror1(int v) { return __builtin_amdgcn_update_dpp(v, v, 0x13C, 0xf, 0xf, false); }
#endif
#ifdef VMX_EMU
__device__ __forceinline__ unsigned vmx_pk(int lo, int hi) { return ((unsigned)lo & 0xffffu) | ((unsigned)hi << 16); }
__device__ __forceinline__ int vmx_pk_lo(unsigned a) { return (int)(short)(a & 0xffffu); }
__device__ __forceinline__ int vmx_pk_hi(unsigned a) { return (int)(short)(a >> 16); }
__device__ __forceinline__ unsigned vmx_pk_add(unsigned a, unsigned b) { return vmx_pk(vmx_pk_lo(a) + vmx_pk_lo(b), vmx_pk_hi(a) + vmx_pk_hi(b)); }
__device__ __forceinline__ unsigned vmx_pk_sub(unsigned a, unsigned b) { return vmx_pk(vmx_pk_lo(a) - vmx_pk_lo(b), vmx_pk_hi(a) - vmx_pk_hi(b)); }
__device__ __forceinline__ unsigned vmx_pk_max(unsigned a, unsigned b) {
    const int l = vmx_pk_lo(a) > vmx_pk_lo(b) ? vmx_pk_lo(a) : vmx_pk_lo(b), h = vmx_pk_hi(a) > vmx_pk_hi(b) ? vmx_pk_hi(a) : vmx_pk_hi(b);
    return vmx_pk(l, h);
}
__device__ __forceinline__ unsigned vmx_pk_neg(unsigned a) { return (vmx_pk_lo(a) < 0 ? 0xffffu : 0u) | (vmx_pk_hi(a) < 0 ? 0xffff0000u : 0u); }
__device__ __forceinline__ unsigned vmx_pk_min_u16(unsigned a, unsigned b) { const unsigned al = a & 0xffffu, bl = b & 0xffffu, ah = a >> 16, bh = b >> 16; return (al < bl ? al : bl) | ((ah < bh ? ah : bh) << 16); }
__device__ __forceinline__ unsigned vmx_pk_max_u16(unsigned a, unsigned b) { const unsigned al = a & 0xffffu, bl = b & 0xffffu, ah = a >> 16, bh = b >> 16; return (al > bl ? al : bl) | ((ah > bh ? ah : bh) << 16); }
__device__ __forceinline__ unsigned vmx_pk_mad(unsigned a, unsigned b, unsigned c) { return vmx_pk(vmx_pk_lo(a) * vmx_pk_lo(b) + vmx_pk_lo(c), vmx_pk_hi(a) * vmx_pk_hi(b) + vmx_pk_hi(c)); }
__device__ __forceinline__ unsigned vmx_alignbit16(unsigned hi, unsigned lo) { return (hi << 16) | (lo >> 16); }
#else
typedef short vmx_v2s __attribute__((ext_vector_type(2)));
__device__ __forceinline__ unsigned vmx_pk(int lo, int hi) { return ((unsigned)lo & 0xffffu) | ((unsigned)hi << 16); }
__device__ __forceinline__ int vmx_pk_lo(unsigned a) { return (int)(short)(a & 0xffffu); }
__device__ __forceinline__ int vmx_pk_hi(unsigned a) { return (int)(short)(a >> 16); }
__device__ __forceinline__ unsigned vmx_pk_add(unsigned a, unsigned b) { return __builtin_bit_cast(unsigned, (vmx_v2s)(__builtin_bit_cast(vmx_v2s, a) + __builtin_bit_cast(vmx_v2s, b))); }
__device__ __forceinline__ unsigned vmx_pk_sub(unsigned a, unsigned b) { return __builtin_bit_cast(unsigned, (vmx_v2s)(__builtin_bit_cast(vmx_v2s, a) - __builtin_bit_cast(vmx_v2s, b))); }
__device__ __forceinline__ unsigned vmx_pk_max(unsigned a, unsigned b) { return __builtin_bit_cast(unsigned, __builtin_elementwise_max(__builtin_bit_cast(vmx_v2s, a), __builtin_bit_cast(vmx_v2s, b))); }
__device__ __forceinline__ unsigned vmx_pk_neg(unsigned a) { unsigned r; asm("v_pk_ashrrev_i16 %0, 15, %1 op_sel_hi:[0,1]" : "=v"(r) : "v"(a)); return r; }
__device__ __forceinline__ unsigned vmx_pk_min_u16(unsigned a, unsigned b) { unsigned r; asm("v_pk_min_u16 %0, %1, %2" : "=v"(r) : "v"(a), "v"(b)); return r; }
typedef unsigned short vmx_v2u __attribute__((ext_vector_type(2)));
__device__ __forceinline__ unsigned vmx_pk_max_u16(unsigned a, unsigned b) { return __builtin_bit_cast(unsigned, __builtin_elementwise_max(__builtin_bit_cast(vmx_v2u, a), __builtin_bit_cast(vmx_v2u, b))); }
__device__ __forceinline__ unsigned vmx_pk_mad(unsigned a, unsigned b, unsigned c) { unsigned r; asm("v_pk_mad_i16 %0, %1, %2, %3" : "=v"(r) : "v"(a), "v"(b), "v"(c)); return r; }
__device__ __forceinline__ unsigned vmx_alignbit16(unsigned hi, unsigned lo) { return __builtin_amdgcn_alignbit(hi, lo, 16); }
#endif
#ifdef VMX_EMU
__device__ __forceinline__ unsigned vmx_pk_bytes(unsigned b) { return (b & 0xffu) | ((b >> 8) & 0xff00u); }
#else
__device__ __forceinline__ unsigned vmx_pk_bytes(unsigned b) { return __builtin_amdgcn_perm(b, b, 0x0c0c0200u); }
#endif
#if defined(VMX_EMU) || defined(VMX_NOPRIO)
#define VMX_SETPRIO(p) ((void)0)
#else
#define VMX_SETPRIO(p) __builtin_amdgcn_s_setprio(p)
#endif
#ifdef VMX_EMU
__device__ __forceinline__ void vmx_wave_lds_fence() { __syncthreads(); }
#else
__device__ __forceinline__ void vmx_wave_lds_fence() { asm volatile("" ::: "memory"); }
#endif
__device__ __forceinline__ unsigned vmx_bfi(unsigned m, unsigned a, unsigned b) { return (m & a) | (~m & b); }
#ifdef VMX_EMU
__device__ __forceinline__ int vmx_uniform_i32(int v) { return v; }
#else
__device__ __forceinline__ int vmx_uniform_i32(int v) { return __builtin_amdgcn_readfirstlane(v); }
#endif
__device__ __forceinline__ long long vmx_uniform_i64(long long v) {
    union { long long d; int i[2]; } u; u.d = v;
    u.i[0] = vmx_uniform_i32(u.i[0]); u.i[1] = vmx_uniform_i32(u.i[1]);
    return u.d;
}
__device__ __forceinline__ double vmx_uniform_f64(double v) {
    union { double d; int i[2]; } u; u.d = v;
    u.i[0] = vmx_uniform_i32(u.i[0]); u.i[1] = vmx_uniform_i32(u.i[1]);
    return u.d;
}
#ifdef VMX_EMU
#define VMX_GLOBAL_PTR(T, p) (p)
#else
#define VMX_GLOBAL_PTR(T, p) ((T*)(__attribute__((address_space(1))) T*)(unsigned long long)vmx_uniform_i64((long long)(p)))
#endif
#ifdef VMX_EMU
__device__ __forceinline__ int vmx_bcast0(int v) { return __shfl(v, 0); }
#else
__device__ __forceinline__ int vmx_bcast0(int v) { return __builtin_amdgcn_readfirstlane(v); }
#endif
__device__ __forceinline__ double vmx_shr1_f64(double v) {
    union { double d; int i[2]; } u; u.d = v;
    u.i[0] = vmx_shr1(u.i[0]); u.i[1] = vmx_shr1(u.i[1]);
    return u.d;
}
__device__ __forceinline__ long long vmx_shr1_i64(long long v) {
    union { long long d; int i[2]; } u; u.d = v;
    u.i[0] = vmx_shr1(u.i[0]); u.i[1] = vmx_shr1(u.i[1]);
    return u.d;
// ... 380 lines not shown
```

vacmap_amd/csrc/vmx_dp_ad.h:

```cpp
#ifndef VMX_DP_AD_H
#define VMX_DP_AD_H

#ifdef VMX_EMU
__device__ __forceinline__ int vmx_r16_shl1_in(int v, int in) { const int l = vmx_lane(); const int e = __shfl(v, (l & 48) | ((l + 1) & 15)); return (l & 15) == 15 ? in : e; }
__device__ __forceinline__ unsigned vmx_perm(unsigned s0, unsigned s1, unsigned sel) {
    unsigned r = 0;
    for (int b = 0; b < 4; ++b) {
        const unsigned c = (sel >> (8 * b)) & 0xffu;
        const unsigned v = c < 4 ? (s1 >> (8 * c)) & 0xffu : c < 8 ? (s0 >> (8 * (c - 4))) & 0xffu : 0u;
        r |= v << (8 * b);
    }
    return r;
}
#else
__device__ __forceinline__ int vmx_r16_shl1_in(int v, int in) { return __builtin_amdgcn_update_dpp(in, v, 0x101, 0xf, 0xf, false); }
__device__ __forceinline__ unsigned vmx_perm(unsigned s0, unsigned s1, unsigned sel) { return __builtin_amdgcn_perm(s0, s1, sel); }
#endif

#define VMX_AD_NEGINF (-4096)
#define VMX_AD_CSH 12
#define VMX_AD_TE1 6u
#define VMX_AD_TF1 3u
#define VMX_AD_TE2 1u
#define VMX_AD_TF2 0u
__host__ __device__ constexpr long long vmx_ad_imax(long long a, long long b) { return a > b ? a : b; }
__host__ __device__ constexpr long long vmx_ad_imin(long long a, long long b) { return a < b ? a : b; }
__host__ __device__ constexpr long long vmx_ad_bias(int mismatch, int o1, int e1, int o2, int e2) {
    return -((long long)VMX_AD_NEGINF - (long long)(VMX_DP16X4_MAX + 1) * vmx_ad_imax(e1, e2) - vmx_ad_imax(vmx_ad_imax(o1, o2), -(long long)mismatch));
}
__host__ __device__ constexpr bool vmx_ad_scores_ok(int match, int mismatch, int o1, int e1, int o2, int e2) {
    return match >= 0 && mismatch <= match && 8LL * (match - mismatch) <= (1 << VMX_AD_CSH) && o1 >= 0 && e1 >= 0 && o2 >= 0 && e2 >= 0 &&
           (long long)match * (VMX_DP16X4_MAX / 2 + 1) + vmx_ad_bias(mismatch, o1, e1, o2, e2) <= 8191 &&
           vmx_ad_imin(mismatch, 0) * (VMX_DP16X4_MAX / 2) - vmx_ad_imin(o1 + (long long)e1 * VMX_DP16X4_MAX, o2 + (long long)e2 * VMX_DP16X4_MAX)
               - vmx_ad_imax(o1, o2) - vmx_ad_imax(e1, e2) > (long long)VMX_AD_NEGINF + vmx_ad_imax(o1, o2);
}
static_assert(vmx_ad_scores_ok(2, -4, 4, 2, 24, 1), "the gap fill's own scoring (vmx_align.hip: gf_score) must fit the tagged 16-bit domain");
struct vmx_ad_consts { unsigned O1, O2, E1, E2, MATCH, PEN, NH, NE1, NE2, NF1, NF2; };

__device__ __forceinline__ void vmx_ad_cell(const vmx_ad_consts& K, unsigned upH, unsigned upE1, unsigned upE2, unsigned leftH, unsigned leftF1,
                                            unsigned leftF2, unsigned tc, unsigned qc, unsigned& H, unsigned& E1, unsigned& E2, unsigned& F1, unsigned& F2,
                                            unsigned (&w)[5]) {
    const unsigned e1v = vmx_pk_max_u16(upH - K.O1, upE1) - K.E1, e2v = vmx_pk_max_u16(upH - K.O2, upE2) - K.E2;
    const unsigned f1v = vmx_pk_max_u16(leftH - K.O1, leftF1) - K.E1, f2v = vmx_pk_max_u16(leftH - K.O2, leftF2) - K.E2;
    E1 = e1v & ~((7u ^ VMX_AD_TE1) * 0x00010001u); E2 = e2v & ~((7u ^ VMX_AD_TE2) * 0x00010001u);
    F1 = f1v & ~((7u ^ VMX_AD_TF1) * 0x00010001u); F2 = f2v & ~((7u ^ VMX_AD_TF2) * 0x00010001u);
    const unsigned hd = H + K.MATCH - vmx_pk_min_u16(tc ^ qc, K.PEN);
    const unsigned h = vmx_pk_max_u16(vmx_pk_max_u16(hd, E1), vmx_pk_max_u16(vmx_pk_max_u16(F1, E2), F2));
    H = h | 0x00070007u;
    w[0] = h; w[1] = e1v; w[2] = e2v; w[3] = f1v; w[4] = f2v;
}

__device__ __forceinline__ unsigned vmx_ad_bytes(const unsigned (&a)[5], const unsigned (&b)[5]) {
    constexpr unsigned SEL = 0x06020400u;
    const unsigned gh = vmx_perm(b[0], a[0], SEL), ge1 = vmx_perm(b[1], a[1], SEL), ge2 = vmx_perm(b[2], a[2], SEL);
    const unsigned gf1 = vmx_perm(b[3], a[3], SEL), gf2 = vmx_perm(b[4], a[4], SEL);
    const unsigned src = vmx_perm(0x00010000u, 0x03000204u, gh & 0x07070707u);
    unsigned op = vmx_bfi(0x01010101u, ge1, ge2);
    op = vmx_bfi(0x04040404u, gf1, op);
    op = vmx_bfi(0x08080808u, (gf2 << 3) | (gf2 >> 29), op);
    return src | (((op & 0x0f0f0f0fu) ^ 0x0f0f0f0fu) << 3);
}

template <int NS>
__device__ __forceinline__ void vmx_ad_pack(const unsigned (&w)[NS][5], unsigned& w01, unsigned& w23) {
    w01 = vmx_ad_bytes(w[0], w[NS > 1 ? 1 : 0]);
    w23 = 0;
    if (NS > 2) w23 = vmx_ad_bytes(w[NS > 2 ? 2 : 0], w[NS > 3 ? 3 : 0]);
    if (NS == 3) w23 &= 0x00ff00ffu;
}

template <int NS>
__device__ __forceinline__ unsigned vmx_ad_pick(const unsigned (&v)[NS], int k) {
    unsigned r = 0;
#pragma unroll
    for (int i = 0; i < NS; ++i) r |= v[i] & (unsigned)-(int)(k == i);
    return r;
}

template <int NS>
__device__ __forceinline__ void vmx_gapfill_fill_ad(const uint8_t* __restrict__ TX, const uint8_t* __restrict__ QX, int tlX, int qlX, int dloX, uint8_t* __restrict__ tbX,
                                                   const uint8_t* __restrict__ TY, const uint8_t* __restrict__ QY, int tlY, int qlY, int dloY, uint8_t* __restrict__ tbY,
                                                   int match, int mismatch, int o1, int e1, int o2, int e2, int lane, int& scoreX, int& scoreY) {
    const int l = lane & 15;
    vmx_ad_consts K;
    K.O1 = vmx_pk(8 * o1, 8 * o1); K.O2 = vmx_pk(8 * o2, 8 * o2); K.E1 = vmx_pk(8 * e1, 8 * e1); K.E2 = vmx_pk(8 * e2, 8 * e2);
    K.MATCH = vmx_pk(8 * match, 8 * match); K.PEN = vmx_pk(8 * (match - mismatch), 8 * (match - mismatch));
    const int bias = (int)vmx_ad_bias(mismatch, o1, e1, o2, e2);
    const unsigned neg = 8u * (unsigned)(VMX_AD_NEGINF + bias);
    K.NH = (neg + 7u) * 0x00010001u; K.NE1 = (neg + VMX_AD_TE1) * 0x00010001u; K.NE2 = (neg + VMX_AD_TE2) * 0x00010001u;
    K.NF1 = (neg + VMX_AD_TF1) * 0x00010001u; K.NF2 = (neg + VMX_AD_TF2) * 0x00010001u;
    const int afX = (tlX > 0 && qlX > 0) ? tlX + qlX : 0, afY = (tlY > 0 && qlY > 0) ? tlY + qlY : 0;
    const int total = vmx_uniform_i32(vmx_wave_max_i32(afX > afY ? afX : afY));
    const int npairs = (total + 1) >> 1;
    const int poX = (afX + 1) >> 1, peX = afX >> 1, poY = (afY + 1) >> 1, peY = afY >> 1;
    const int hX = dloX >> 1, hY = dloY >> 1;
    auto tcf = [&](const uint8_t* T, int tl, int i) -> int { return ((i >= 1 && i <= tl) ? vmx_tcode(T[i - 1]) : 5) << VMX_AD_CSH; };
    auto qcf = [&](const uint8_t* Q, int ql, int j) -> int { return ((j >= 1 && j <= ql) ? (int)Q[j - 1] : 4) << VMX_AD_CSH; };
    unsigned tcode[NS], qcode[NS];
#pragma unroll
    for (int k = 0; k < NS; ++k) {
        tcode[k] = vmx_pk(tcf(TX, tlX, -hX - NS * l - k), tcf(TY, tlY, -hY - NS * l - k));
        qcode[k] = vmx_pk(qcf(QX, qlX, hX + NS * l + k), qcf(QY, qlY, hY + NS * l + k));
    }
    unsigned HA[NS], E1A[NS], E2A[NS], F1A[NS], F2A[NS], HC[NS], E1C[NS], E2C[NS], F1C[NS], F2C[NS];
    {
        const int l0X = (-dloX) / (2 * NS), k0X = ((-dloX) % (2 * NS)) >> 1, l0Y = (-dloY) / (2 * NS), k0Y = ((-dloY) % (2 * NS)) >> 1;
#pragma unroll
        for (int k = 0; k < NS; ++k) {
            const unsigned m = ((l == l0X && k == k0X) ? 0xffffu : 0u) | ((l == l0Y && k == k0Y) ? 0xffff0000u : 0u);
            HA[k] = vmx_bfi(m, (8u * (unsigned)bias + 7u) * 0x00010001u, K.NH);
            E1A[k] = K.NE1; E2A[k] = K.NE2; F1A[k] = K.NF1; F2A[k] = K.NF2;
            HC[k] = K.NH; E1C[k] = K.NE1; E2C[k] = K.NE2; F1C[k] = K.NF1; F2C[k] = K.NF2;
        }
    }
    const int xfX = (qlX - tlX) - dloX, xfY = (qlY - tlY) - dloY;
    const int lfX = xfX / (2 * NS), kfX = (xfX % (2 * NS)) >> 1, lfY = xfY / (2 * NS), kfY = (xfY % (2 * NS)) >> 1;
    int finX = 0, finY = 0;
    constexpr int W = VMX_AD_W(NS);
    uint8_t* const pX = tbX + VMX_AD_TB_OFF_W(0, l, W);
    uint8_t* const pY = tbY + VMX_AD_TB_OFF_W(0, l, W);
    auto put = [&](uint8_t* at, unsigned w01, unsigned w23, bool hi) {
        if constexpr (W == 1) *at = (uint8_t)(hi ? (w01 >> 16) : w01);
        else if constexpr (W == 2) *(uint16_t*)at = (uint16_t)(hi ? (w01 >> 16) : w01);
        else *(uint32_t*)at = vmx_perm(w23, w01, hi ? 0x07060302u : 0x05040100u);
    };
    auto load_chunks = [&](int b16, unsigned& tch, unsigned& qch) {
        tch = vmx_pk(tcf(TX, tlX, b16 + 1 + l - hX), tcf(TY, tlY, b16 + 1 + l - hY));
        qch = vmx_pk(qcf(QX, qlX, b16 + 15 - l + hX + 16 * NS), qcf(QY, qlY, b16 + 15 - l + hY + 16 * NS));
    };
    unsigned tch, qch, ntch, nqch;
    load_chunks(0, ntch, nqch);
    for (int p0 = 0; p0 < npairs; p0 += 16) {
        tch = ntch; qch = nqch;
        load_chunks(p0 + 16, ntch, nqch);
        int pend = npairs - p0; if (pend > 16) pend = 16;
        for (int pp = 0; pp < pend; ++pp) {
            const int p = p0 + pp + 1;
            {
                const unsigned in = (unsigned)vmx_r16_shl1_in((int)qcode[0], (int)qch);
#pragma unroll
                for (int k = 0; k + 1 < NS; ++k) qcode[k] = qcode[k + 1];
                qcode[NS - 1] = in;
                qch = (unsigned)vmx_r16_ror1((int)qch);
            }
            unsigned w[NS][5];
            {
                const unsigned nH = (unsigned)vmx_r16_shl1_in((int)HA[0], (int)K.NH), nE1 = (unsigned)vmx_r16_shl1_in((int)E1A[0], (int)K.NE1),
                               nE2 = (unsigned)vmx_r16_shl1_in((int)E2A[0], (int)K.NE2);
#pragma unroll
                for (int k = 0; k < NS; ++k) {
                    const unsigned uH = k + 1 < NS ? HA[k + 1 < NS ? k + 1 : 0] : nH, uE1 = k + 1 < NS ? E1A[k + 1 < NS ? k + 1 : 0] : nE1, uE2 = k + 1 < NS ? E2A[k + 1 < NS ? k + 1 : 0] : nE2;
                    vmx_ad_cell(K, uH, uE1, uE2, HA[k], F1A[k], F2A[k], tcode[k], qcode[k], HC[k], E1C[k], E2C[k], F1C[k], F2C[k], w[k]);
                }
            }
            {
                unsigned w01, w23;
                vmx_ad_pack<NS>(w, w01, w23);
                const size_t so = VMX_AD_TB_OFF_W(2 * p - 2, 0, W);
                if (p <= poX) put(pX + so, w01, w23, false);
                if (p <= poY) put(pY + so, w01, w23, true);
            }
            {
                const unsigned in = (unsigned)vmx_r16_shr1_in((int)tcode[NS - 1], (int)tch);
#pragma unroll
                for (int k = NS - 1; k > 0; --k) tcode[k] = tcode[k - 1];
                tcode[0] = in;
                tch = (unsigned)vmx_r16_rol1((int)tch);
            }
            {
                const unsigned nH = (unsigned)vmx_r16_shr1_in((int)HC[NS - 1], (int)K.NH), nF1 = (unsigned)vmx_r16_shr1_in((int)F1C[NS - 1], (int)K.NF1),
                               nF2 = (unsigned)vmx_r16_shr1_in((int)F2C[NS - 1], (int)K.NF2);
#pragma unroll
                for (int k = 0; k < NS; ++k) {
                    const unsigned lH = k > 0 ? HC[k > 0 ? k - 1 : 0] : nH, lF1 = k > 0 ? F1C[k > 0 ? k - 1 : 0] : nF1, lF2 = k > 0 ? F2C[k > 0 ? k - 1 : 0] : nF2;
                    vmx_ad_cell(K, HC[k], E1C[k], E2C[k], lH, lF1, lF2, tcode[k], qcode[k], HA[k], E1A[k], E2A[k], F1A[k], F2A[k], w[k]);
                }
            }
            {
                unsigned w01, w23;
                vmx_ad_pack<NS>(w, w01, w23);
                const size_t so = VMX_AD_TB_OFF_W(2 * p - 1, 0, W);
                if (p <= peX) put(pX + so, w01, w23, false);
                if (p <= peY) put(pY + so, w01, w23, true);
            }
            if (__any(p == poX || p == poY)) {
                const unsigned aX = vmx_ad_pick<NS>(HA, kfX), cX = vmx_ad_pick<NS>(HC, kfX), aY = vmx_ad_pick<NS>(HA, kfY), cY = vmx_ad_pick<NS>(HC, kfY);
                const unsigned vX = (afX & 1) ? cX : aX, vY = (afY & 1) ? cY : aY;
                if (p == poX && l == lfX) finX = (int)((vX & 0xffffu) >> 3) - bias;
                if (p == poY && l == lfY) finY = (int)(vY >> 19) - bias;
            }
        }
    }
    scoreX = __shfl(finX, (lane & 48) | (lfX & 15));
    scoreY = __shfl(finY, (lane & 48) | (lfY & 15));
}

__device__ __forceinline__ bool vmx_ad_proven(int score, int tl, int ql, int g, int match, int o1, int e1, int o2, int e2) {
    const int mn = tl < ql ? tl : ql;
    if (g < 1) return false;
    if (g > mn) return true;
    const long long U = (long long)match * mn - vmx_ad_margin(g, match, o1, e1, o2, e2);
    return (long long)score > U;
}
#endif
```

vacmap_amd/csrc/vmx_host.h:

```cpp
#ifndef VMX_HOST_H
#define VMX_HOST_H
#include "vmx_device.h"
#include "vmx_kernels.h"
#include "../../include/vacmapx.h"
#include <algorithm>
#include <map>
#include <cstring>
#include <string>
#include <vector>
#include <chrono>
#include <atomic>
#include <mutex>
#include <execinfo.h>

namespace vmx {

void set_error(const std::string& s);
int hip_fail(hipError_t e, const char* what, const char* file, int line);

#define VMX_HIP(expr)                                                              \
    do {                                                                           \
        hipError_t _e = (expr);                                                    \
        if (_e != hipSuccess) return vmx::hip_fail(_e, #expr, __FILE__, __LINE__);  \
    } while (0)
// ... 162 lines not shown
    m.up_used = at;
    if (A.n) hipLaunchKernelGGL(k_import, dim3((unsigned)std::max<unsigned long long>(1, std::min<unsigned long long>((tot + 16383ULL) >> 14, 32ULL))), dim3(256), 0, c->stream, A);
    return 0;
}
template <class T> int vmx_push(vm_ctx* c, vmx::DevBuf& b, const T* host, size_t n, int line = __builtin_LINE(), const char* file = __builtin_FILE()) {
    const size_t bytes = sizeof(T) * n;
    if (!c->mb.on || !n) return vmx::upload(b, host, n, c->stream, line, file);
    VMX_TRY(b.reserve(bytes));
    vmx::copy_census().add(file, line, bytes);
    const vmx_push_piece pc{b.p, host, bytes};
    return vmx_push_pieces(c, &pc, 1);
}
struct vmx_push_req { vmx::DevBuf* b; const void* host; size_t bytes; };
static inline int vmx_push_many(vm_ctx* c, const vmx_push_req* rq, int np) {
    vmx_push_piece pc[4];
    for (int i = 0; i < np; ++i) { VMX_TRY(rq[i].b->reserve(rq[i].bytes ? rq[i].bytes : 1)); pc[i] = vmx_push_piece{rq[i].b->p, rq[i].host, rq[i].bytes}; }
    return vmx_push_pieces(c, pc, np);
}
template <class T> int vmx_push_to(vm_ctx* c, void* dev, const T* host, size_t n) {
    if (!n) return 0;
    const vmx_push_piece pc{dev, host, sizeof(T) * n};
    return vmx_push_pieces(c, &pc, 1);
}
int vmx_fetch_bytes(vm_ctx* c, void* host, const void* dev, size_t bytes);
template <class T> int vmx_fetch(vm_ctx* c, T* host, const void* dev, size_t n, int line = __builtin_LINE(), const char* file = __builtin_FILE()) {
    if (!n) return 0;
    if (!c->mb.on) return vmx::download(host, dev, n, c->stream, line, file);
    vmx::copy_census().add(file, -line, sizeof(T) * n);
    return vmx_fetch_bytes(c, (void*)host, dev, sizeof(T) * n);
}
struct vmx_fetch_scope {
    vm_ctx* c;
    explicit vmx_fetch_scope(vm_ctx* ctx) : c(ctx) { drop(); }
    ~vmx_fetch_scope() { drop(); }
    void drop() { c->mb.pend.clear(); c->mb.dn_used = 0; c->mb.big_used = 0; }
};

struct vmx_fork {
    vm_ctx* c; int used = 0;
    explicit vmx_fork(vm_ctx* ctx) : c(ctx) { (void)hipEventRecord(c->fork_ev, c->stream); }
    hipStream_t next() {
        hipStream_t s = c->aux[used & 3];
        if (used < 4) (void)hipStreamWaitEvent(s, c->fork_ev, 0);
        ++used;
        return s;
    }
    void join() {
        const int n = used < 4 ? used : 4;
        for (int i = 0; i < n; ++i) { (void)hipEventRecord(c->join_ev[i], c->aux[i]); (void)hipStreamWaitEvent(c->stream, c->join_ev[i], 0); }
        used = 0;
    }
};

__global__ void k_encode(const char* in, uint8_t* out, int64_t n);
__global__ void k_edit_distance(const uint8_t* qcodes, const int64_t* q_off, const uint8_t* tcodes, const int64_t* t_off,
                                int8_t* carry_pool, const int32_t* order, const int32_t* range, int32_t* counters, int which, int64_t* out,
                                int64_t carry_stride, int32_t* oflow);
__global__ void k_size_order(const int64_t* size, const int32_t* n_ptr, int64_t thresh, int32_t* order, int32_t* range, int32_t* counters);
__global__ void k_size_hist(const int64_t* size, const int32_t* n_ptr, int64_t thresh, int32_t* ghist);
__global__ void k_size_scatter(const int64_t* size, const int32_t* n_ptr, const int32_t* ghist, int32_t* gcur, int32_t* order, int32_t* range, int32_t* counters);
static inline void vmx_size_order_wide(vm_ctx* c, const int64_t* size, const int32_t* n_ptr, int64_t n_upper, int64_t thresh, int32_t* order, int32_t* range, int32_t* counters,
                                       int32_t* scratch) {
    static const bool one_wg = getenv("VMX_SIZE_ORDER_ONE") != nullptr;
    if (one_wg) { hipLaunchKernelGGL(k_size_order, dim3(1), dim3(1024), 0, c->stream, size, n_ptr, thresh, order, range, counters); return; }
    (void)hipMemsetAsync(scratch, 0, 4 * 513, c->stream);
    const unsigned G = (unsigned)std::max<int64_t>(1, std::min<int64_t>((n_upper + 1023) / 1024, (int64_t)c->num_cu * 2));
    hipLaunchKernelGGL(k_size_hist, dim3(G), dim3(256), 0, c->stream, size, n_ptr, thresh, scratch);
    hipLaunchKernelGGL(k_size_scatter, dim3(G), dim3(256), 0, c->stream, size, n_ptr, (const int32_t*)scratch, scratch + 257, order, range, counters);
}
__global__ void k_ed_banded(const uint8_t* qcodes, const int64_t* q_off, const uint8_t* tcodes, const int64_t* t_off, const int32_t* order,
                            const int32_t* range, int32_t* counter, int64_t* ub_out);
struct vmx_ext_args;
__global__ void k_ed_banded4(const uint8_t* qcodes, const int64_t* q_off, const uint8_t* tcodes, const int64_t* t_off, const int32_t* order,
                             const int32_t* range, int32_t* counter, int64_t* ub_out);
__global__ void k_ed_flag(const int64_t* ub, const int64_t* q_off, const int64_t* t_off, const int32_t* n_ptr, double maxdiv, int64_t* sizes,
                          int64_t* ed_out, int32_t* n_flagged, int first, const int32_t* prob_read, struct vmx_ext_read* er);
__global__ void k_extend(const uint8_t* tcodes, const int64_t* t_off, const uint8_t* qcodes, const int64_t* q_off, int n_prob,
                         int match, int mismatch, int o, int e, int bw_in, int zdrop, int32_t* out_te, int32_t* out_qe, int32_t* out_sc, const int32_t* n_ptr);
__global__ void k_gapfill_fill(const uint8_t* tcodes, const uint8_t* qcodes, const vmx_dp_prob* probs, int n_prob, int match,
                               int mismatch, int o1, int e1, int o2, int e2, uint8_t* tb_pool, int32_t* bnd_pool, int32_t* out_score,
                               const int32_t* order, int32_t* counter);
__global__ void k_gapfill_fill_ns(const uint8_t* tcodes, const uint8_t* qcodes, vmx_dp_prob* probs, int n_prob, int match,
                                  int mismatch, int o1, int e1, int o2, int e2, uint8_t* tb_pool, int32_t* bnd_pool, int32_t* out_score,
                                  const int32_t* order, const int32_t* range, int32_t* counter, int32_t* redo_list, int32_t* redo_cnt, int redo_pass, int ad_pct,
                                  uint8_t* redo_pool, unsigned long long* redo_bytes, const int32_t* n_ptr = nullptr, unsigned long long redo_cap = ~0ULL, int tb_by_ns = 0);
static inline int vmx_ad_pct_env(int mode = 0) {
    int pct = mode == 1 ? 40 : 90, pmin = mode == 1 ? 40 : VMX_AD_PCT_MIN_DEFAULT;
    if (const char* e = getenv("VMX_AD_PCT")) { const int v = atoi(e); if (v >= 0 && v <= 60000) pct = v; }
    if (const char* e = getenv("VMX_AD_PCT_MIN")) { const int v = atoi(e); if (v >= 0 && v <= 60000) pmin = v; }
    return pct | (pmin << 16);
}
__global__ void k_gapfill_trace(const uint8_t* tcodes, const uint8_t* qcodes, const vmx_dp_prob* probs, int n_prob, int eqx,
                                const uint8_t* tb_pool, uint32_t* run_pool, char* cig_pool, int32_t* cig_len, const int32_t* band_flag, const uint8_t* redo_pool, int spread, int32_t* cig_q, const int32_t* n_ptr = nullptr);
__global__ void k_flip_sort(const int64_t* rows, const int64_t* aoff, const int64_t* readlens, int n_reads, uint64_t* key_pool,
                            const int64_t* key_off, vmx_anchor* sorted, int32_t* need_reverse);
__global__ void k_chain_global(const vmx_anchor* anchors, const int64_t* aoff, const int32_t* rlist, int nlist, int lds_cap,
                               vmx_tables tab, const double* gapcost_list, double oskipcost, int omaxdiff, int maxgap,
                               double* S_out, int32_t* P_out, int32_t* SA_out, uint8_t* cov_pool, int64_t* gmax_out, int64_t* opcount_out, int rmode,
                               double* FP_pool, double* PP_pool);
static inline int64_t vmx_rows_misfit(const int64_t* rows, int64_t n) {
    for (int64_t i = 0; i < n; ++i) {
        const int64_t q = rows[4 * i], s = rows[4 * i + 2], l = rows[4 * i + 3];
        if (l < 0 || l > 65535 || q < INT32_MIN || q > INT32_MAX || q + l > INT32_MAX || s < INT16_MIN || s > INT16_MAX) return i;
    }
    return -1;
}
__global__ void k_chain_global_rows(const vmx_anchor* anchors, const int64_t* aoff, const int32_t* rlist, int nlist, vmx_tables tab, const double* gapcost_list,
                                    double oskipcost, int omaxdiff, int maxgap, double* S_out, int32_t* P_out, int32_t* SA_out, uint8_t* cov_pool,
                                    int64_t* gmax_out, int64_t* opcount_out, int rmode, double* FP_pool, double* PP_pool, unsigned long long* dbg);
__global__ void k_chain_global_rows_w3(const vmx_anchor* anchors, const int64_t* aoff, const int32_t* rlist, int nlist, vmx_tables tab, const double* gapcost_list,
                                       double oskipcost, int omaxdiff, int maxgap, double* S_out, int32_t* P_out, int32_t* SA_out, uint8_t* cov_pool,
                                       int64_t* gmax_out, int64_t* opcount_out, int rmode, double* FP_pool, double* PP_pool, unsigned long long* dbg);
static inline bool vmx_chain_rows_win3() { const char* e = getenv("VMX_RW_WIN"); return e && atoi(e) == 3; }
unsigned long long* vmx_chain_dbg();
void vmx_chain_dbg_report(hipStream_t st);
static inline bool vmx_chain_rows_on() { static const bool on = [] { const char* e = getenv("VMX_CHAIN_ROWS"); return !e || atoi(e) != 0; }(); return on; }
__global__ void k_chain_global_fast(const vmx_anchor* anchors, const int64_t* aoff, int n_reads, const int64_t* roff, vmx_tables tab,
                                    const double* gapcost_list, double oskipcost, int omaxdiff, int maxgap, double* S_out, int32_t* P_out, int32_t* SA_out,
                                    uint8_t* cov_pool, int32_t* si_pool, int64_t* t_pool, int32_t* cnt_pool, int64_t* gmax_out, int32_t* ran, int rmode,
                                    double* FP_pool, double* PP_pool);
__global__ void k_chain_select(const vmx_anchor* anchors, const int64_t* aoff, const int64_t* readlens, const int32_t* rlist, int nlist, int lds_cap,
                               const double* S, const int32_t* P, const int32_t* SA, const int64_t* gmax, const int32_t* need_reverse, int mode,
                               char* scratch, const int64_t* scratch_off, int32_t* out_mapq, double* out_score, int32_t* out_npaths,
                               int32_t* out_path_len, vmx_anchor* out_path_anchors);

#endif
```

vacmap_amd/csrc/vmx_kernels.h:

```cpp
#ifndef VMX_KERNELS_H
#define VMX_KERNELS_H
#include <stdint.h>

struct vmx_dp_prob {
    int64_t t_off, q_off;
    int32_t tl, ql;
    int64_t tb_off;
    int64_t bnd_off;
    int64_t run_off;
    int64_t cig_off;
};

struct vmx_anchor {
    int32_t q;
    int16_t l;
    int16_t s;
    int64_t r;
};

struct vmx_slot { uint64_t key; uint32_t start; uint32_t count; };

struct vmx_tables {
    const float* extra; int32_t extra_n;
    const float* readgap_h; const float* readgap_r; const float* large_readgap;
// ... 24 lines not shown
    int c; long long t;
    if (si == 1) { c = (same ? -lj : (ASMV ? 0 : 1)) - m; t = d; }
    else { c = same ? -li - m : li - lj + (ASMV ? -m : m - 1); t = same ? -d : d; }
    refgap = t + (long long)c;
}
struct vmx_lseed_args {
    const uint8_t* ocodes; const int64_t* roff;
    const uint8_t* ref; const int64_t* coff; int32_t nseq;
    const vmx_anchor* guide_rows; const int32_t* guide_len; const int32_t* n_guides_used; const int64_t* aoff;
    int32_t n_reads, k, look_span, read_span, sort_by_start;
    const int32_t* order; int32_t* queue;
    int64_t la_slot_len;
    int32_t* head_pool; int32_t* next_pool;
    int64_t head_stride;
    int32_t* epoch_pool;
    int32_t* sq_pool; int32_t* dst_pool;
    int64_t* tpos_pool; int64_t tpos_cap;
    unsigned long long* dbg;
    uint64_t* hkey2_pool;
    uint64_t* hkey_pool; int64_t* hval_pool; int32_t* goff_pool; int64_t hit_cap;
    int32_t* pcnt_pool; int64_t pcnt_cap; int32_t* pc2_pool; int64_t* stg_pool;
    uint64_t* gkey_pool; int32_t* gq_pool; int64_t* gr_pool; int64_t gkey_cap;
    vmx_anchor* la_rows; uint64_t* la_ekey; vmx_anchor* la_sorted; const int64_t* la_off; int32_t* la_cnt; int32_t* status;
    const int64_t* rd_off; const int64_t* rd_len; const int32_t* r_st; const int32_t* r_en;
};

#ifdef VMX_EMU
#define VMX_LB_QC 128
#define VMX_LB_HCAP 256
#define VMX_LB_GS 20
#define VMX_LB_NBLOG 8
#define VMX_LB_SORTK 512
#else
#ifndef VMX_LB_QC
#define VMX_LB_QC 512
#define VMX_LB_HCAP 512
#define VMX_LB_NBLOG 9
#define VMX_LB_SORTK 1024
#endif
#ifndef VMX_LB_GS
#define VMX_LB_GS 64
#endif
#endif
#ifndef VMX_LB_BMLOG
#define VMX_LB_BMLOG 14
#endif
#ifndef VMX_LB_WAVES
#define VMX_LB_WAVES 2
#endif
#define VMX_LB_TABLE_U64 (((1 << VMX_LB_NBLOG) + 2 * VMX_LB_QC + (1 << (VMX_LB_BMLOG - 5))) / 2)
#define VMX_LB_REGION_U64 (VMX_LB_SORTK > VMX_LB_TABLE_U64 ? VMX_LB_SORTK : VMX_LB_TABLE_U64)
#define VMX_LB_CQ_BYTES (128 + 2 * VMX_LB_HCAP > 2304 ? 128 + 2 * VMX_LB_HCAP : 2304)
#define VMX_LB_LDS_BYTES (8 * (VMX_LB_REGION_U64 + VMX_LB_HCAP) + VMX_LB_CQ_BYTES)
#define VMX_ED_WAVES 16
#define VMX_ED_LONG 16384
#define VMX_EDB_HW 768
#define VMX_EDB_MAXD 512
#define VMX_EDB4_HW 320
#define VMX_EDB4_MAXD 256
#ifndef VMX_LSEED_WAVES
#define VMX_LSEED_WAVES 6
#endif
#define VMX_SORT_LDS 4096
#ifdef VMX_EMU
#define VMX_SORT_LDS_BIG 8192
#else
#define VMX_SORT_LDS_BIG 16384
#endif
#define VM_READ_FASTPATH_DEV (-21)
#ifdef VMX_EMU
#define VMX_DP16_MAX 420
#else
#define VMX_DP16_MAX 6000
#endif
#define VMX_DP16_OK(tl, ql) ((tl) + (ql) <= VMX_DP16_MAX)
#ifdef VMX_EMU
#define VMX_DP16X4_MAX 160
#else
#define VMX_DP16X4_MAX 1024
#endif
#define VMX_DP16X4_OK(tl, ql) ((tl) + (ql) <= VMX_DP16X4_MAX)
#define VMX_X4_W(ql) ((((ql) + 31) + 15) & ~15)
#define VMX_AD_NS_MAX 4
__host__ __device__ static inline int vmx_ad_geom(int tl, int ql, int ns, int* dlo_out) {
    const int dl = ql - tl, lo = dl < 0 ? dl : 0, hi = dl > 0 ? dl : 0;
    const int slack = 32 * ns - (hi - lo + 1);
    if (slack < 0) return 0;
    int mb = slack / 2, dlo = lo - mb;
    if (dlo & 1) {
        if (mb + 1 <= slack) { ++mb; --dlo; }
        else if (mb >= 1) { --mb; ++dlo; }
        else return 0;
    }
    *dlo_out = dlo;
    const int ma = slack - mb;
    return (mb < ma ? mb : ma) + 1;
}
__host__ __device__ static inline long long vmx_ad_margin(int g, int match, int o1, int e1, int o2, int e2) {
    const long long c1 = o1 + (long long)g * e1, c2 = o2 + (long long)g * e2;
    return (long long)match * g + 2 * (c1 < c2 ? c1 : c2);
}
__host__ __device__ static inline int vmx_ad_ns(int tl, int ql, int match, int o1, int e1, int o2, int e2, int pct, int pct_min) {
    if (tl <= 0 || ql <= 0) return 0;
    const int mn = tl < ql ? tl : ql;
    int dlo, g = 0;
    for (int ns = 1; ns <= VMX_AD_NS_MAX; ++ns) {
        g = vmx_ad_geom(tl, ql, ns, &dlo);
        if (g >= 1 && (g > mn || vmx_ad_margin(g, match, o1, e1, o2, e2) * 100 >= (long long)pct * mn)) return ns;
    }
    return (g >= 1 && vmx_ad_margin(g, match, o1, e1, o2, e2) * 100 >= (long long)pct_min * mn) ? VMX_AD_NS_MAX : 0;
}
#define VMX_AD_PCT_DEFAULT 100
#define VMX_AD_PCT_MIN_DEFAULT 65
#define VMX_AD_FLAG 16
#define VMX_PK_FLAG 1
#ifdef VMX_EMU
#define VMX_REDO_PK(tl, ql) ((tl) > 0 && (ql) > 0 && VMX_DP16X4_OK(tl, ql) && (tl) + (ql) >= 120)
#else
#ifndef VMX_REDO_PK_MIN
#define VMX_REDO_PK_MIN 384
#endif
#define VMX_REDO_PK(tl, ql) ((tl) > 0 && (ql) > 0 && VMX_DP16X4_OK(tl, ql) && (tl) + (ql) >= VMX_REDO_PK_MIN)
#endif
#define VMX_PK_TB_BYTES(tl, ql) ((int64_t)(((tl) + 127) / 128) * ((ql) + 127) * 128)
#ifndef VMX_AD_AB
#define VMX_AD_AB 4
#endif
static_assert(VMX_AD_AB == 1 || 64 / VMX_AD_AB <= 16, "a 64-byte line of the anti-diagonal traceback holds at most the 16 lanes of a row per anti-diagonal (1-byte slots): AB = 1, 4 or 8");
#define VMX_AD_TB_OFF(s, l) ((((size_t)(s) & ~(size_t)(VMX_AD_AB - 1)) << 6) + ((size_t)(s) & (VMX_AD_AB - 1)) * (64 / VMX_AD_AB) + ((size_t)(l) / (16 / VMX_AD_AB)) * 64 + ((size_t)(l) % (16 / VMX_AD_AB)) * 4)
#define VMX_AD_TB_BYTES(tl, ql) ((int64_t)(((tl) + (ql) + VMX_AD_AB - 1) & ~(VMX_AD_AB - 1)) * 64)
#define VMX_AD_W(ns) ((ns) <= 0 ? 0 : ((ns) == 1 ? 1 : ((ns) == 2 ? 2 : 4)))
#define VMX_AD_TB_OFF_W(s, l, W) (((size_t)(s) / VMX_AD_AB) * (size_t)(VMX_AD_AB * 16 * (W)) + ((size_t)(l) / (64 / (VMX_AD_AB * (W)))) * 64 + ((size_t)(s) % VMX_AD_AB) * (64 / VMX_AD_AB) + ((size_t)(l) % (64 / (VMX_AD_AB * (W)))) * (W))
#define VMX_AD_TB_BYTES_W(tl, ql, W) ((int64_t)(((tl) + (ql) + VMX_AD_AB - 1) & ~(VMX_AD_AB - 1)) * 16 * (W))
#define VMX_X4_TB_BYTES(tl, ql) ((int64_t)(((tl) + 31) / 32) * VMX_X4_W(ql) * 32)
#define VMX_TB_BYTES(tl, ql) (((tl) > 0 && (ql) > 0) ? (VMX_DP16X4_OK(tl, ql) ? VMX_X4_TB_BYTES(tl, ql) : \
                              VMX_DP16_OK(tl, ql) ? VMX_PK_TB_BYTES(tl, ql) : (int64_t)(((tl) + 63) / 64) * ((ql) + 63) * 64) : 0)
#define VMX_TB_BYTES_NS(tl, ql) (((tl) > 0 && (ql) > 0 && VMX_DP16X4_OK(tl, ql)) ? VMX_AD_TB_BYTES(tl, ql) : VMX_TB_BYTES(tl, ql))
#define VMX_REDO_TB_BYTES(tl, ql) (VMX_REDO_PK(tl, ql) ? VMX_PK_TB_BYTES(tl, ql) : VMX_X4_TB_BYTES(tl, ql))
__device__ __forceinline__ uint8_t* vmx_tb_ptr(const uint8_t* tb_pool, const uint8_t* redo_pool, int64_t off) {
    const unsigned long long base = off >= 0 ? (unsigned long long)tb_pool : (unsigned long long)redo_pool;
    return (uint8_t*)(base + (unsigned long long)(off >= 0 ? off : -off - 1));
}
#define VMX_HEAD_THRESH (((int64_t)1 << 18) - 1)
#define VMX_TB_CHUNK ((int64_t)4 << 30)
#ifdef VMX_EMU
#define VMX_MAX_BATCH_BASES 20000
#define VMX_MAX_BATCH_READS 6
#else
#define VMX_MAX_BATCH_BASES ((int64_t)160 << 20)
#define VMX_MAX_BATCH_READS 16384
#endif
#define VMX_LA_SLOT(len) ((len) / 2 + 4096)
#define VMX_SELECT_LDS 3072
#define VMX_LC_LDS_MAX_DEFAULT 13056
#define VMX_GC_LDS_MAX_DEFAULT 13056
#define VMX_CHAIN_LDS_MAX_SHARED 512
#define VMX_LC_BYTES_PER_ANCHOR 12
#define VMX_GC_BYTES_PER_ANCHOR 12

#endif
```

vacmap_amd/lib.py:

```python
import ctypes as C
import os
import numpy as np

_HERE = os.path.dirname(os.path.abspath(__file__))
DEFAULT_SO = os.environ.get('VACMAPX_LIB') or os.path.join(_HERE, 'libvacmapx.so')

VM_ERR_NO_DEVICE = -2
MODES = {'H': 0, 'L': 1, 'S': 2, 'R': 3, 'asm': 4}


class VmxError(RuntimeError):
    def __init__(self, code, msg):
        super().__init__('vacmapx error %d: %s' % (code, msg))
        self.code = code


class Params(C.Structure):
    _fields_ = [('mode', C.c_int32), ('check_num', C.c_int32), ('mid_occ', C.c_int32), ('global_maxdiff', C.c_int32),
                ('local_maxdiff', C.c_int32), ('local_kmersize', C.c_int32), ('eqx', C.c_int32), ('hardclip', C.c_int32),
                ('nodiscard', C.c_int32), ('reserved', C.c_int32), ('global_skipcost', C.c_double),
                ('local_skipcost', C.c_double), ('maxdivergence', C.c_double)]


class Score(C.Structure):
    _fields_ = [('match', C.c_int32), ('mismatch', C.c_int32), ('o1', C.c_int32), ('e1', C.c_int32), ('o2', C.c_int32), ('e2', C.c_int32)]


class CigarOut(C.Structure):
    _fields_ = [('cigar', C.c_void_p), ('q_e', C.c_int32), ('t_e', C.c_int32), ('score', C.c_int32)]


class ChainsOut(C.Structure):
    _fields_ = [('need_reverse', C.POINTER(C.c_int32)), ('mapq', C.POINTER(C.c_int32)), ('score', C.POINTER(C.c_double)),
                ('fast_used', C.POINTER(C.c_int32)), ('read_path_off', C.POINTER(C.c_int64)), ('path_off', C.POINTER(C.c_int64)),
                ('path_anchors', C.POINTER(C.c_int64)), ('S', C.POINTER(C.c_double)), ('P', C.POINTER(C.c_int64)),
                ('S_arg', C.POINTER(C.c_int64)), ('gmax', C.POINTER(C.c_int64)), ('opcount', C.POINTER(C.c_int64))]


class LinkedOut(C.Structure):
    _fields_ = [('gmax', C.c_int64), ('n_hot', C.c_int64), ('n_cold', C.c_int64), ('opcount', C.c_int64), ('cold_max', C.c_double),
                ('S', C.POINTER(C.c_double)), ('P', C.POINTER(C.c_int64)), ('S_arg_hot', C.POINTER(C.c_int64)),
                ('carry_status', C.c_int32), ('saved', C.c_int32), ('n_carry', C.c_int64), ('carry_S', C.POINTER(C.c_double)),
                ('carry_P', C.POINTER(C.c_int64)), ('carry_rows', C.POINTER(C.c_int64)), ('carry_g_max_scores', C.c_double), ('carry_prereadloc', C.c_int64)]


class LocalOut(C.Structure):
    _fields_ = [('status', C.POINTER(C.c_int32)), ('variant', C.POINTER(C.c_int32)), ('score', C.POINTER(C.c_double)),
                ('chain_off', C.POINTER(C.c_int64)), ('chain', C.POINTER(C.c_int64)), ('raw_off', C.POINTER(C.c_int64)),
                ('raw', C.POINTER(C.c_int64))]


class Record(C.Structure):
    _fields_ = [('read_idx', C.c_int32), ('contig', C.c_int32), ('strand', C.c_int32), ('mapq', C.c_int32),
                ('q_st', C.c_int64), ('q_en', C.c_int64), ('r_st', C.c_int64), ('r_en', C.c_int64),
                ('cigar_off', C.c_int64), ('cigar_len', C.c_int64)]


class SamOpts(C.Structure):
    _fields_ = [('md', C.c_int32), ('shortcs', C.c_int32), ('cigar2cg', C.c_int32), ('markunbalancetra', C.c_int32), ('hardclip', C.c_int32),
                ('fakecigar', C.c_int32), ('rg_id', C.c_char_p), ('asm_mode', C.c_int32)]


class BatchStats(C.Structure):
    _fields_ = [(n, C.c_int64) for n in ('n_reads', 'read_bases', 'n_minimizers', 'n_hits', 'n_anchors', 'n_local_hits', 'n_local_anchors',
                                          'n_segments', 'n_ed_problems', 'ed_cells', 'n_ext_problems', 'ext_cells', 'n_dp_problems',
                                          'dp_cells', 'n_records', 'cigar_bytes', 'aligned_bases', 'n_unmapped', 'n_failed',
                                          'dp_string_bytes')] + \
               [('ms_total', C.c_double), ('ms_stage', C.c_double * 16), ('ms_gapfill_fill', C.c_double), ('ms_gapfill_trace', C.c_double),
                ('n_gapfill_launches', C.c_int64), ('n_ed_full', C.c_int64), ('n_ed_tier2', C.c_int64), ('n_ed_tier1', C.c_int64),
                ('n_dp_redo', C.c_int64), ('dp_redo_tb_bytes', C.c_int64), ('ms_local_seed', C.c_double), ('ms_cluster', C.c_double), ('n_host_syncs', C.c_int64), ('n_local_general', C.c_int64), ('n_ext_retries', C.c_int64), ('n_batch_retries', C.c_int64)]


def _b(s):
    return s if isinstance(s, (bytes, bytearray)) else s.encode()


def _cat(seqs):
    bs = [_b(s) for s in seqs]
    off = np.zeros(len(bs) + 1, np.int64)
    if bs:
        off[1:] = np.cumsum([len(b) for b in bs])
    return b''.join(bs), off


def _seq_ptrs(seqs):
    keep, ptrs, lens = [], [], []
    for x in seqs:
        if isinstance(x, np.ndarray):
            a = np.ascontiguousarray(x, dtype=np.uint8)
            keep.append(a); ptrs.append(a.ctypes.data); lens.append(a.size)
        else:
            b = C.create_string_buffer(_b(x), len(x)) if len(x) else C.create_string_buffer(1)
            keep.append(b); ptrs.append(C.addressof(b)); lens.append(len(x))
    n = len(ptrs)
    arr = (C.c_void_p * max(n, 1))(*ptrs)
    return keep, C.cast(arr, C.POINTER(C.c_char_p)), (C.c_int64 * max(n, 1))(*lens)


class VmxLib:

    def __init__(self, path=None):
        path = path or DEFAULT_SO
        try:
            if os.environ.get('VACMAPX_SKIP_TORCH') == '1' and 'torch' not in __import__('sys').modules:
                raise ImportError('single-GPU command line: no torch, the library brings the system HIP runtime (saves ~1.5 s of start-up)')
            import torch
        except ImportError:
            pass
        if not os.path.exists(path):
            raise FileNotFoundError('%s not built: run `python -m vacmap_amd.build` (hipcc, gfx950). No fallback exists.' % path)
        L = self.L = C.CDLL(path)
        vp, i32, i64, dbl, cp, P = C.c_void_p, C.c_int32, C.c_int64, C.c_double, C.c_char_p, C.POINTER
        L.vm_last_error.restype = cp
        L.vm_version.restype = cp
        L.vm_free.argtypes = [vp]
        L.vm_params_default.argtypes = [P(Params), C.c_int]
        L.vm_ctx_create.argtypes = [C.c_int, P(vp)]
        L.vm_ctx_destroy.argtypes = [vp]
        L.vm_ctx_set_inflight.argtypes = [vp, C.c_int]
        L.vm_ctx_set_blocking_sync.argtypes = [vp, C.c_int]
        L.vm_debug_chain_counters.argtypes = [C.c_int, C.POINTER(C.c_ulonglong)]
        L.vm_ctx_mem_info.argtypes = [vp, P(i64), P(i64)]
        L.vm_table.argtypes = [vp, C.c_int, P(vp)]; L.vm_table.restype = i64
        L.vm_edit_distance_batch.argtypes = [vp, i64, cp, vp, cp, vp, P(P(i64))]
        L.vm_edit_distance_bound_batch.argtypes = [vp, C.c_int, i64, cp, vp, cp, vp, P(P(i64))]
        L.vm_edit_distance.argtypes = [vp, cp, i64, cp, i64]; L.vm_edit_distance.restype = i64
        L.vm_k_extend_batch.argtypes = [vp] + [C.c_int] * 6 + [i64, cp, vp, cp, vp, P(P(i32)), P(P(i32)), P(P(i32))]
        L.vm_k_cigar_batch.argtypes = [vp, P(Score), C.c_int, i64, cp, vp, cp, vp, P(vp), P(P(i64)), P(P(i32))]
        L.vm_k_cigar.argtypes = [vp, cp, i64, cp, i64, P(Score), C.c_int, C.c_int, C.c_int, P(CigarOut)]
        L.vm_k_cigar_batch_banded.argtypes = [vp, P(Score), C.c_int, i64, cp, vp, cp, vp, P(vp), P(P(i64)), P(P(i32)), vp]
        L.vm_chain_global_batch.argtypes = [vp, P(Params), C.c_int, i64, vp, vp, vp, C.c_int, P(ChainsOut)]
        L.vm_chain_linked.argtypes = [vp, C.c_int, C.c_int, C.c_double, C.c_int, C.c_int, i64, vp, i64, vp, vp, C.c_double, i64, i64, P(LinkedOut)]
        L.vm_linked_out_free.argtypes = [P(LinkedOut)]
        L.vm_align_asm.argtypes = [vp, vp, P(Params), C.c_char_p, i64, i64, i64, i64, P(P(Record)), P(i64), P(vp), P(C.c_int32)]
        L.vm_chains_out_free.argtypes = [P(ChainsOut)]
        L.vm_index_build_fasta.argtypes = [vp, cp, C.c_int, C.c_int, P(vp)]
        L.vm_index_build_mem.argtypes = [vp, C.c_int, P(cp), P(cp), P(i64), C.c_int, C.c_int, P(vp)]
        L.vm_index_save.argtypes = [vp, cp]; L.vm_index_load.argtypes = [vp, cp, P(vp)]
        L.vm_index_save_mmi.argtypes = [vp, cp, C.c_int]; L.vm_index_load_mmi.argtypes = [vp, cp, P(vp)]
        L.vm_index_free.argtypes = [vp]
        for f in ('vm_index_k', 'vm_index_w', 'vm_index_nseq', 'vm_index_mid_occ', 'vm_index_blob_count'):
            getattr(L, f).argtypes = [vp]
        L.vm_index_n_minimizers.argtypes = [vp]; L.vm_index_n_minimizers.restype = i64
        L.vm_index_n_distinct.argtypes = [vp]; L.vm_index_n_distinct.restype = i64
        L.vm_index_seq_info.argtypes = [vp, C.c_int, P(cp), P(i64), P(i64)]
        L.vm_index_seq.argtypes = [vp, C.c_int, i64, i64, vp]; L.vm_index_seq.restype = i64
        L.vm_index_minimizers.argtypes = [vp, P(P(C.c_uint64)), P(P(C.c_uint64)), P(i64)]
        L.vm_index_blob.argtypes = [vp, C.c_int, P(vp), P(i64)]
        L.vm_index_meta_size.argtypes = [vp, P(i64)]; L.vm_index_meta_get.argtypes = [vp, vp, i64]
        L.vm_index_from_meta.argtypes = [vp, vp, i64, P(vp)]
        L.vm_sketch_batch.argtypes = [vp, C.c_int, C.c_int, i64, cp, vp, P(P(C.c_uint64)), P(P(i32)), P(P(C.c_int8)), P(P(i64))]
        L.vm_map_batch.argtypes = [vp, vp, C.c_int, C.c_int, i64, cp, vp, P(P(i64)), P(P(i64))]
        L.vm_map.argtypes = [vp, vp, cp, i64, C.c_int, C.c_int, P(P(i64)), P(i64)]
# ... 69 lines not shown

    def __init__(self, device=0, lib=None):
        self.lib = lib or load()
        h = C.c_void_p()
        self.lib.check(self.lib.L.vm_ctx_create(device, C.byref(h)))
        self.h = h; self.device = int(device)

    def set_inflight(self, n_contexts):
        self.lib.check(self.lib.L.vm_ctx_set_inflight(self.h, int(n_contexts)))

    def set_blocking_sync(self, on=True):
        self.lib.check(self.lib.L.vm_ctx_set_blocking_sync(self.h, int(bool(on))))

    def mem_info(self):
        f = C.c_int64(); t = C.c_int64()
        self.lib.check(self.lib.L.vm_ctx_mem_info(self.h, C.byref(f), C.byref(t)))
        return f.value, t.value

    def close(self):
        if self.h:
            self.lib.L.vm_ctx_destroy(self.h)
            self.h = None

    def __del__(self):
        try:
            self.close()
        except Exception:
            pass

    def _take(self, ptr, n, dtype):
        a = np.ctypeslib.as_array(ptr, shape=(max(int(n), 1),))[:int(n)].astype(dtype, copy=True)
        self.lib.L.vm_free(ptr)
        return a

    def table(self, which):
        p = C.c_void_p()
        n = self.lib.check(self.lib.L.vm_table(self.h, which, C.byref(p)))
        ty = C.c_float if which < 4 else C.c_double
        a = np.ctypeslib.as_array(C.cast(p, C.POINTER(ty)), shape=(n,)).copy()
        self.lib.L.vm_free(p)
        return a

    def edit_distance_batch(self, queries, targets):
        q, qo = _cat(queries); t, to = _cat(targets)
        out = C.POINTER(C.c_int64)()
        self.lib.check(self.lib.L.vm_edit_distance_batch(self.h, len(queries), q, qo.ctypes.data, t, to.ctypes.data, C.byref(out)))
        return self._take(out, len(queries), np.int64)

    def edit_distance_bound_batch(self, queries, targets, tier=2):
        q, qo = _cat(queries); t, to = _cat(targets)
        out = C.POINTER(C.c_int64)()
        self.lib.check(self.lib.L.vm_edit_distance_bound_batch(self.h, tier, len(queries), q, qo.ctypes.data, t, to.ctypes.data, C.byref(out)))
        return self._take(out, len(queries), np.int64)

    def edit_distance(self, q, t):
        q, t = _b(q), _b(t)
        return self.lib.check(self.lib.L.vm_edit_distance(self.h, q, len(q), t, len(t)))

    def k_extend_batch(self, targets, queries, match=2, mismatch=-4, o=4, e=4, bw=100, zdrop=50):
        t, to = _cat(targets); q, qo = _cat(queries)
        te = C.POINTER(C.c_int32)(); qe = C.POINTER(C.c_int32)(); sc = C.POINTER(C.c_int32)()
        n = len(targets)
        self.lib.check(self.lib.L.vm_k_extend_batch(self.h, match, mismatch, o, e, bw, zdrop, n, t, to.ctypes.data, q, qo.ctypes.data,
                                                    C.byref(te), C.byref(qe), C.byref(sc)))
        return self._take(sc, n, np.int32), self._take(te, n, np.int32), self._take(qe, n, np.int32)

    def k_cigar_batch(self, targets, queries, match=2, mismatch=-4, o1=4, e1=2, o2=24, e2=1, eqx=False):
        t, to = _cat(targets); q, qo = _cat(queries)
        n = len(targets)
        sc = Score(match, mismatch, o1, e1, o2, e2)
        cg = C.c_void_p(); co = C.POINTER(C.c_int64)(); ss = C.POINTER(C.c_int32)()
        self.lib.check(self.lib.L.vm_k_cigar_batch(self.h, C.byref(sc), int(eqx), n, t, to.ctypes.data, q, qo.ctypes.data,
                                                   C.byref(cg), C.byref(co), C.byref(ss)))
        off = self._take(co, n + 1, np.int64)
        blob = C.string_at(cg.value, int(off[-1])) if off[-1] else b''
        self.lib.L.vm_free(cg)
        cigars = [blob[off[i]:off[i + 1] - 1].decode() for i in range(n)]
        return cigars, self._take(ss, n, np.int32)

    def k_cigar_batch_banded(self, targets, queries, match=2, mismatch=-4, o1=4, e1=2, o2=24, e2=1, eqx=False):
        t, to = _cat(targets); q, qo = _cat(queries)
        n = len(targets)
        sc = Score(match, mismatch, o1, e1, o2, e2)
        cg = C.c_void_p(); co = C.POINTER(C.c_int64)(); fl = C.POINTER(C.c_int32)(); st = (C.c_int64 * 4)()
        self.lib.check(self.lib.L.vm_k_cigar_batch_banded(self.h, C.byref(sc), int(eqx), n, t, to.ctypes.data, q, qo.ctypes.data,
                                                          C.byref(cg), C.byref(co), C.byref(fl), st))
        off = self._take(co, n + 1, np.int64)
        blob = C.string_at(cg.value, int(off[-1])) if off[-1] else b''
        self.lib.L.vm_free(cg)
        cigars = [blob[off[i]:off[i + 1] - 1].decode() for i in range(n)]
        return cigars, self._take(fl, n, np.int32), {'eligible': st[0], 'proven': st[1], 'redo': st[2], 'not_eligible': st[3]}

    def k_cigar(self, target, query, match=2, mismatch=-4, gap_open_1=4, gap_extend_1=2, gap_open_2=24, gap_extend_2=1,
                bw=-1, zdropvalue=-1, eqx=False):
        t, q = _b(target), _b(query)
        sc = Score(match, mismatch, gap_open_1, gap_extend_1, gap_open_2, gap_extend_2)
        out = CigarOut()
        self.lib.check(self.lib.L.vm_k_cigar(self.h, t, len(t), q, len(q), C.byref(sc), bw, zdropvalue, int(eqx), C.byref(out)))
        cg = C.string_at(out.cigar).decode() if out.cigar else ''
        self.lib.L.vm_free(out.cigar)
        return cg, 0, out.q_e, out.t_e, 0, 0

    def chain_global_batch(self, prm, kmersize, anchors_list, readlens, want_raw=False):
        n = len(anchors_list)
        aoff = np.zeros(n + 1, np.int64)
        for i, a in enumerate(anchors_list):
            aoff[i + 1] = aoff[i] + len(a)
        rows = np.ascontiguousarray(np.concatenate([np.asarray(a, dtype=np.int64).reshape(-1, 4) for a in anchors_list]) if n else np.zeros((0, 4), np.int64))
        rl = np.ascontiguousarray(readlens, dtype=np.int64)
        out = ChainsOut()
        self.lib.check(self.lib.L.vm_chain_global_batch(self.h, C.byref(prm), kmersize, n, rows.ctypes.data, aoff.ctypes.data, rl.ctypes.data,
                                                        int(want_raw), C.byref(out)))
        res = []
        rpo = np.ctypeslib.as_array(out.read_path_off, shape=(n + 1,)).copy()
        npaths = int(rpo[-1])
        po = np.ctypeslib.as_array(out.path_off, shape=(npaths + 1,)).copy()
        nrows = int(po[-1])
        pa = np.ctypeslib.as_array(out.path_anchors, shape=(max(nrows, 1), 4))[:nrows].copy()
        tot = int(aoff[-1])
        for r in range(n):
            d = {'need_reverse': bool(out.need_reverse[r]), 'mapq': int(out.mapq[r]), 'score': float(out.score[r]),
                 'fast_used': bool(out.fast_used[r]), 'gmax': int(out.gmax[r]), 'opcount': int(out.opcount[r]),
                 'paths': [pa[po[p]:po[p + 1]] for p in range(rpo[r], rpo[r + 1])]}
            if want_raw:
                a, b = int(aoff[r]), int(aoff[r + 1])
                d['S'] = np.ctypeslib.as_array(out.S, shape=(max(tot, 1),))[a:b].copy()
                d['P'] = np.ctypeslib.as_array(out.P, shape=(max(tot, 1),))[a:b].copy()
                d['S_arg'] = np.ctypeslib.as_array(out.S_arg, shape=(max(tot, 1),))[a:b].copy()
            res.append(d)
        self.lib.L.vm_chains_out_free(C.byref(out))
        return res

    def sketch_batch(self, k, w, seqs):
        s, off = _cat(seqs)
        n = len(seqs)
        h = C.POINTER(C.c_uint64)(); p = C.POINTER(C.c_int32)(); z = C.POINTER(C.c_int8)(); oo = C.POINTER(C.c_int64)()
        self.lib.check(self.lib.L.vm_sketch_batch(self.h, k, w, n, s, off.ctypes.data, C.byref(h), C.byref(p), C.byref(z), C.byref(oo)))
        o = self._take(oo, n + 1, np.int64)
        m = int(o[-1])
        H = self._take(h, m, np.uint64); Pp = self._take(p, m, np.int32); Z = self._take(z, m, np.int8)
        return [(H[o[i]:o[i + 1]], Pp[o[i]:o[i + 1]], Z[o[i]:o[i + 1]]) for i in range(n)]

    def map(self, index, seq, check_num=100, mid_occ=-1):
        sq = _b(seq)
        a = C.POINTER(C.c_int64)(); n = C.c_int64(0)
        self.lib.check(self.lib.L.vm_map(self.h, index.h, sq, len(sq), int(check_num), int(mid_occ), C.byref(a), C.byref(n)))
        rows = np.ctypeslib.as_array(a, shape=(max(n.value, 1), 4))[:n.value].copy()
        self.lib.L.vm_free(a)
        return rows

    def chain_linked(self, rows, which, kmersize, skipcost, maxdiff, maxgap, g_max_scores=0., g_max_index=0, pre_S=None, pre_P=None, prereadloc=0):
        a = np.ascontiguousarray(rows, dtype=np.int64).reshape(-1, 4)
        ps = np.ascontiguousarray(pre_S if pre_S is not None else [], dtype=np.float64)
        pp = np.ascontiguousarray(pre_P if pre_P is not None else [], dtype=np.int64)
        out = LinkedOut()
        self.lib.check(self.lib.L.vm_chain_linked(self.h, which, kmersize, float(skipcost), int(maxdiff), int(maxgap), len(a), a.ctypes.data, len(ps), ps.ctypes.data,
                                                  pp.ctypes.data, float(g_max_scores), int(g_max_index), int(prereadloc), C.byref(out)))
        n = len(a)
        r = {'gmax': out.gmax, 'n_hot': out.n_hot, 'n_cold': out.n_cold, 'cold_max': out.cold_max, 'opcount': out.opcount,
             'S': np.ctypeslib.as_array(out.S, shape=(n,)).copy(), 'P': np.ctypeslib.as_array(out.P, shape=(n,)).copy(),
             'S_arg_hot': np.ctypeslib.as_array(out.S_arg_hot, shape=(max(out.n_hot, 1),))[:out.n_hot].copy(),
             'carry_status': out.carry_status, 'saved': out.saved, 'n_carry': out.n_carry}
        if out.carry_status == 0 and out.saved:
            m = out.n_carry
            r.update(carry_S=np.ctypeslib.as_array(out.carry_S, shape=(m,)).copy(), carry_P=np.ctypeslib.as_array(out.carry_P, shape=(m,)).copy(),
                     carry_rows=np.ctypeslib.as_array(out.carry_rows, shape=(m, 4)).copy(), carry_g_max_scores=out.carry_g_max_scores,
                     carry_prereadloc=out.carry_prereadloc)
        self.lib.L.vm_linked_out_free(C.byref(out))
        return r

    def map_batch(self, index, seqs, check_num=100, mid_occ=-1):
        s, off = _cat(seqs)
        n = len(seqs)
        a = C.POINTER(C.c_int64)(); ao = C.POINTER(C.c_int64)()
# ... 564 lines not shown
```

Measured before the change: 3.385.

## Try wide 64-lane anti-diagonal banded DP on redo problems before full fill

The redo pass, which used to run a full-matrix fill for every problem that failed the narrow banded pass, now first tries a wider anti-diagonal band that uses all 64 lanes (up to 128*ns diagonals). It processes two problems per wavefront, and falls back to the full fill only when the band result cannot be proven optimal. The redo path moves into its own templated kernel, and new counters record how many redos were settled by the wide band and how many needed the full fill. The aim is to cut the cost of full quadratic DP on redo problems. In exchange it adds work whenever the wide band fails, plus extra traceback-layout complexity.

```diff
diff --git a/include/vacmapx.h b/include/vacmapx.h
--- a/include/vacmapx.h
+++ b/include/vacmapx.h
@@ -163,6 +163,8 @@
     int64_t n_local_general;
     int64_t n_ext_retries;
     int64_t n_batch_retries;
+    int64_t n_dp_redo_wide;
+    int64_t n_dp_redo_full;
 } vm_batch_stats;
 
 int vm_align_batch(vm_ctx*, const vm_index*, const vm_params*, int64_t n_reads, const char* seqs, const int64_t* offsets,
diff --git a/vacmap_amd/csrc/k_dp.hip b/vacmap_amd/csrc/k_dp.hip
--- a/vacmap_amd/csrc/k_dp.hip
+++ b/vacmap_amd/csrc/k_dp.hip
@@ -384,24 +384,56 @@
         if (pk) vmx_gapfill_fill16(T, Q, tl, ql, match, mismatch, o1, e1, o2, e2, tb, bH, SCORE ? &out_score[p] : &sink, lane);
 }
 
-template <bool SCORE>
+template <bool SCORE, bool REDO = false>
 __device__ __forceinline__ void vmx_gapfill_fill_body(const uint8_t* __restrict__ tcodes, const uint8_t* __restrict__ qcodes,
                                                      const vmx_dp_prob* __restrict__ probs, int n_prob, int match, int mismatch,
                                                      int o1, int e1, int o2, int e2, uint8_t* __restrict__ tb_pool,
                                                      int32_t* __restrict__ bnd_pool, int32_t* __restrict__ out_score,
                                                      const int32_t* __restrict__ order, int32_t* __restrict__ counter,
-                                                     int32_t* __restrict__ redo_list = nullptr, int32_t* __restrict__ redo_cnt = nullptr, int redo_pass = 0,
+                                                     int32_t* __restrict__ redo_list = nullptr, int32_t* __restrict__ redo_cnt = nullptr,
                                                      uint8_t* __restrict__ redo_pool = nullptr) {
     const int lane = vmx_lane();
     int static_next = 4 * (int)blockIdx.x;
-    if (redo_pass) {
+    const bool redo_pass = REDO;
+    if constexpr (REDO) {
         n_prob = redo_cnt[0]; order = redo_list; counter = redo_cnt + 1;
+        const bool ad_ok = vmx_ad_scores_ok(match, mismatch, o1, e1, o2, e2);
         while (true) {
-            int q; { int v = 0; if (lane == 0) v = atomicAdd(redo_cnt + 2, 1); q = vmx_bcast0(v); }
+            int q; { int v = 0; if (lane == 0) v = atomicAdd(redo_cnt + 2, 2); q = vmx_bcast0(v); }
             if (q >= n_prob) break;
-            const int p = order[q];
-            const int tl = probs[p].tl, ql = probs[p].ql;
-            if (VMX_REDO_PK(tl, ql)) vmx_gapfill_fill_one<SCORE>(tcodes, qcodes, probs, p, match, mismatch, o1, e1, o2, e2, tb_pool, bnd_pool, out_score, lane, VMX_PK_FLAG, redo_pool);
+            int pX = vmx_uniform_i32(order[q]), pY = q + 1 < n_prob ? vmx_uniform_i32(order[q + 1]) : -1;
+            if (pY >= 0 && !VMX_REDO_PK(probs[pY].tl, probs[pY].ql)) pY = -1;
+            if (!VMX_REDO_PK(probs[pX].tl, probs[pX].ql)) { pX = pY; pY = -1; }
+            if (pX < 0) continue;
+            vmx_dp_prob prX = probs[pX], prY = prX;
+            if (pY >= 0) prY = probs[pY];
+            const int tlX0 = vmx_uniform_i32(prX.tl), qlX0 = vmx_uniform_i32(prX.ql), tlY0 = pY >= 0 ? vmx_uniform_i32(prY.tl) : 0, qlY0 = pY >= 0 ? vmx_uniform_i32(prY.ql) : 0;
+            const int nsX = ad_ok ? vmx_ad_ns_nd(tlX0, qlX0, match, o1, e1, o2, e2, VMX_ADW_PCT, VMX_ADW_PCT_MIN, VMX_ADW_DPN, VMX_ADW_NS_MIN, VMX_AD_NS_MAX) : 0;
+            const int nsY = ad_ok ? vmx_ad_ns_nd(tlY0, qlY0, match, o1, e1, o2, e2, VMX_ADW_PCT, VMX_ADW_PCT_MIN, VMX_ADW_DPN, VMX_ADW_NS_MIN, VMX_AD_NS_MAX) : 0;
+            const int ns = nsX > nsY ? nsX : nsY;
+            bool keepX = false, keepY = false;
+            if (ns > 0) {
+                int dloX = 0, dloY = 0;
+                const int gX = nsX > 0 ? vmx_ad_geom_nd(tlX0, qlX0, VMX_ADW_DPN * ns, &dloX) : 0, gY = nsY > 0 ? vmx_ad_geom_nd(tlY0, qlY0, VMX_ADW_DPN * ns, &dloY) : 0;
+                const int tlX = gX > 0 ? tlX0 : 0, qlX = gX > 0 ? qlX0 : 0, tlY = gY > 0 ? tlY0 : 0, qlY = gY > 0 ? qlY0 : 0;
+                int scX = 0, scY = 0;
+#define VMX_ADW_RUN(NSV) vmx_gapfill_fill_ad<NSV, 64>(tcodes + prX.t_off, qcodes + prX.q_off, tlX, qlX, dloX, vmx_tb_ptr(tb_pool, redo_pool, prX.tb_off), tcodes + prY.t_off, qcodes + prY.q_off, \
+                                                      tlY, qlY, dloY, vmx_tb_ptr(tb_pool, redo_pool, prY.tb_off), match, mismatch, o1, e1, o2, e2, lane, scX, scY)
+                if (ns == 2) VMX_ADW_RUN(2); else if (ns == 3) VMX_ADW_RUN(3); else VMX_ADW_RUN(4);
+#undef VMX_ADW_RUN
+                keepX = gX > 0 && vmx_ad_proven(scX, tlX0, qlX0, gX, match, o1, e1, o2, e2);
+                keepY = gY > 0 && vmx_ad_proven(scY, tlY0, qlY0, gY, match, o1, e1, o2, e2);
+            }
+            if (lane == 0) {
+                if (keepX) out_score[pX] = VMX_PK_FLAG;
+                if (keepY) out_score[pY] = VMX_PK_FLAG;
+                const int kept = (int)keepX + (int)keepY, full = 1 + (int)(pY >= 0) - kept;
+                if (kept) atomicAdd(redo_cnt + 6, kept);
+                if (full) atomicAdd(redo_cnt + 7, full);
+            }
+            if (!keepX || (pY >= 0 && !keepY)) __syncthreads();
+            if (!keepX) vmx_gapfill_fill_one<SCORE>(tcodes, qcodes, probs, pX, match, mismatch, o1, e1, o2, e2, tb_pool, bnd_pool, out_score, lane, VMX_PK_FLAG, redo_pool);
+            if (pY >= 0 && !keepY) vmx_gapfill_fill_one<SCORE>(tcodes, qcodes, probs, pY, match, mismatch, o1, e1, o2, e2, tb_pool, bnd_pool, out_score, lane, VMX_PK_FLAG, redo_pool);
         }
     }
     while (true) {
@@ -515,12 +547,17 @@
                                                         int o1, int e1, int o2, int e2, uint8_t* __restrict__ tb_pool,
                                                         int32_t* __restrict__ bnd_pool, int32_t* __restrict__ out_score,
                                                         const int32_t* __restrict__ order, const int32_t* __restrict__ range, int32_t* __restrict__ counter,
-                                                        int32_t* __restrict__ redo_list, int32_t* __restrict__ redo_cnt, int redo_pass, int ad_pct,
-                                                        uint8_t* __restrict__ redo_pool, unsigned long long* __restrict__ redo_bytes, const int32_t* __restrict__ n_ptr,
+                                                        int32_t* __restrict__ redo_list, int32_t* __restrict__ redo_cnt, int ad_pct,
+                                                        unsigned long long* __restrict__ redo_bytes, const int32_t* __restrict__ n_ptr,
                                                         unsigned long long redo_cap, int tb_by_ns) {
     if (n_ptr) n_prob = *n_ptr;
-    if (redo_pass) vmx_gapfill_fill_body<false>(tcodes, qcodes, probs, n_prob, match, mismatch, o1, e1, o2, e2, tb_pool, bnd_pool, out_score, order, counter, redo_list, redo_cnt, 1, redo_pool);
-    else vmx_gapfill_ad_pass(tcodes, qcodes, probs, n_prob, match, mismatch, o1, e1, o2, e2, tb_pool, bnd_pool, out_score, order, range, counter, redo_list, redo_cnt, ad_pct, redo_bytes, redo_cap, tb_by_ns);
+    vmx_gapfill_ad_pass(tcodes, qcodes, probs, n_prob, match, mismatch, o1, e1, o2, e2, tb_pool, bnd_pool, out_score, order, range, counter, redo_list, redo_cnt, ad_pct, redo_bytes, redo_cap, tb_by_ns);
+}
+__global__ void __launch_bounds__(64) k_gapfill_redo(const uint8_t* __restrict__ tcodes, const uint8_t* __restrict__ qcodes, const vmx_dp_prob* __restrict__ probs,
+                                                     int match, int mismatch, int o1, int e1, int o2, int e2, uint8_t* __restrict__ tb_pool,
+                                                     int32_t* __restrict__ bnd_pool, int32_t* __restrict__ out_score, int32_t* __restrict__ redo_list,
+                                                     int32_t* __restrict__ redo_cnt, uint8_t* __restrict__ redo_pool) {
+    vmx_gapfill_fill_body<false, true>(tcodes, qcodes, probs, 0, match, mismatch, o1, e1, o2, e2, tb_pool, bnd_pool, out_score, nullptr, nullptr, redo_list, redo_cnt, redo_pool);
 }
 
 __global__ void k_gapfill_trace(const uint8_t* __restrict__ tcodes, const uint8_t* __restrict__ qcodes,
diff --git a/vacmap_amd/csrc/vmx_align.hip b/vacmap_amd/csrc/vmx_align.hip
--- a/vacmap_amd/csrc/vmx_align.hip
+++ b/vacmap_amd/csrc/vmx_align.hip
@@ -182,12 +182,11 @@
         vmx_lowprio lp(c);
         hipLaunchKernelGGL(k_gapfill_fill_ns, dim3((unsigned)std::max<int64_t>(1, std::min<int64_t>(pn, (int64_t)c->num_cu * fill_waves))), dim3(64), 0, lp.stream(), B.tpool.as<uint8_t>(), B.qpool.as<uint8_t>(),
                            probs, (int)pn, sc.match, sc.mismatch, sc.o1, sc.e1, sc.o2, sc.e2, tb_base, B.bnd.as<int32_t>(), score, B.order.as<int32_t>(), d_range, d_cnt,
-                           redo_list, d_redo_cnt, 0, ad_pct, (uint8_t*)nullptr, d_redo_bytes, n_ptr, (unsigned long long)redo_cap, 1);
+                           redo_list, d_redo_cnt, ad_pct, d_redo_bytes, n_ptr, (unsigned long long)redo_cap, 1);
         lp.join();
     }
-    hipLaunchKernelGGL(k_gapfill_fill_ns, dim3((unsigned)std::max<int64_t>(1, std::min<int64_t>(pn, (int64_t)c->num_cu * 4))), dim3(64), 0, c->stream, B.tpool.as<uint8_t>(), B.qpool.as<uint8_t>(),
-                       probs, (int)pn, sc.match, sc.mismatch, sc.o1, sc.e1, sc.o2, sc.e2, tb_base, B.bnd.as<int32_t>(), score, B.order.as<int32_t>(), d_range, d_cnt,
-                       redo_list, d_redo_cnt, 1, ad_pct, B.tbredo.as<uint8_t>(), d_redo_bytes, n_ptr, (unsigned long long)redo_cap, 1);
+    hipLaunchKernelGGL(k_gapfill_redo, dim3((unsigned)std::max<int64_t>(1, std::min<int64_t>(pn, (int64_t)c->num_cu * 4))), dim3(64), 0, c->stream, B.tpool.as<uint8_t>(), B.qpool.as<uint8_t>(),
+                       probs, sc.match, sc.mismatch, sc.o1, sc.e1, sc.o2, sc.e2, tb_base, B.bnd.as<int32_t>(), score, redo_list, d_redo_cnt, B.tbredo.as<uint8_t>());
     if (ke) (void)hipEventRecord(ke[1], c->stream);
     hipLaunchKernelGGL(k_gapfill_trace, dim3((unsigned)std::max<int64_t>(1, (pn * tr_spread + 63) / 64)), dim3(64), 0, c->stream, B.tpool.as<uint8_t>(), B.qpool.as<uint8_t>(), probs, (int)pn, eqx,
                        tb_base, B.run.as<uint32_t>(), B.cig.as<char>(), B.ciglen.as<int32_t>() + p0, score, B.tbredo.as<uint8_t>(), tr_spread, B.cigq.as<int32_t>() + p0, n_ptr);
@@ -671,7 +670,7 @@
             for (int q = 0; q < gf_chunks[pass]; ++q) {
                 const int32_t* ctl = h_ctl.data() + (size_t)(pass * (VMX_MAX_CHUNKS + 1) + q) * VMX_GF_SLOT;
                 unsigned long long rb = 0; memcpy(&rb, ctl + 16, 8);
-                st.n_dp_redo += ctl[12]; st.dp_redo_tb_bytes += (int64_t)rb; st.dp_cells += (int64_t)rb; ad_failed += ctl[15];
+                st.n_dp_redo += ctl[12]; st.n_dp_redo_wide += ctl[18]; st.n_dp_redo_full += ctl[19]; st.dp_redo_tb_bytes += (int64_t)rb; st.dp_cells += (int64_t)rb; ad_failed += ctl[15];
                 need_max = std::max<int64_t>(need_max, (int64_t)rb);
             }
         c->redo_need_max = std::max<long long>(c->redo_need_max, need_max);
@@ -783,7 +782,7 @@
             tot.ms_total += st.ms_total; for (int i = 0; i < 16; ++i) tot.ms_stage[i] += st.ms_stage[i];
             tot.ms_gapfill_fill += st.ms_gapfill_fill; tot.ms_gapfill_trace += st.ms_gapfill_trace; tot.n_gapfill_launches += st.n_gapfill_launches;
             tot.n_ed_full += st.n_ed_full; tot.n_ed_tier2 += st.n_ed_tier2; tot.n_ed_tier1 += st.n_ed_tier1;
-            tot.n_dp_redo += st.n_dp_redo; tot.dp_redo_tb_bytes += st.dp_redo_tb_bytes; tot.ms_local_seed += st.ms_local_seed; tot.ms_cluster += st.ms_cluster; tot.n_host_syncs += st.n_host_syncs; tot.n_local_general += st.n_local_general; tot.n_ext_retries += st.n_ext_retries; tot.n_batch_retries += st.n_batch_retries;
+            tot.n_dp_redo += st.n_dp_redo; tot.n_dp_redo_wide += st.n_dp_redo_wide; tot.n_dp_redo_full += st.n_dp_redo_full; tot.dp_redo_tb_bytes += st.dp_redo_tb_bytes; tot.ms_local_seed += st.ms_local_seed; tot.ms_cluster += st.ms_cluster; tot.n_host_syncs += st.n_host_syncs; tot.n_local_general += st.n_local_general; tot.n_ext_retries += st.n_ext_retries; tot.n_batch_retries += st.n_batch_retries;
         }
     }
     *recs = (vm_record*)malloc(sizeof(vm_record) * std::max<size_t>(all.size(), 1)); *cigar_blob = (char*)malloc(std::max<size_t>(blob.size(), 1));
diff --git a/vacmap_amd/csrc/vmx_capi.hip b/vacmap_amd/csrc/vmx_capi.hip
--- a/vacmap_amd/csrc/vmx_capi.hip
+++ b/vacmap_amd/csrc/vmx_capi.hip
@@ -553,7 +553,7 @@
         small += sm; nb += sm && flag[i] > VMX_AD_FLAG;
         eligible += sm && vmx_ad_ns(probs[i].tl, probs[i].ql, sc->match, sc->o1, sc->e1, sc->o2, sc->e2, ad_pct & 0xffff, (ad_pct >> 16) & 0xffff) > 0;
     }
-    if (stats) { stats[0] = eligible; stats[1] = nb; stats[2] = ctl[12]; stats[3] = n - small; }
+    if (stats) { stats[0] = eligible; stats[1] = nb; stats[2] = ctl[12]; stats[3] = n - small; stats[4] = ctl[18]; stats[5] = ctl[19]; }
     if (band_flag) { *band_flag = host_alloc<int32_t>((size_t)n); memcpy(*band_flag, flag.data(), sizeof(int32_t) * (size_t)n); }
     cigar_strings(n, probs.data(), hc.data(), hl.data(), cigars, cigar_off);
     return VM_OK;
diff --git a/vacmap_amd/csrc/vmx_device.h b/vacmap_amd/csrc/vmx_device.h
--- a/vacmap_amd/csrc/vmx_device.h
+++ b/vacmap_amd/csrc/vmx_device.h
@@ -28,10 +28,12 @@
 #endif
 #ifdef VMX_EMU
 __device__ __forceinline__ int vmx_shr1_in(int v, int in) { int e = __shfl_up(v, 1); return vmx_lane() == 0 ? in : e; }
+__device__ __forceinline__ int vmx_shl1_in(int v, int in) { int e = __shfl(v, (vmx_lane() + 1) & 63); return vmx_lane() == 63 ? in : e; }
 __device__ __forceinline__ int vmx_rol1(int v) { return __shfl(v, (vmx_lane() + 1) & 63); }
 __device__ __forceinline__ int vmx_ror1(int v) { return __shfl(v, (vmx_lane() + 63) & 63); }
 #else
 __device__ __forceinline__ int vmx_shr1_in(int v, int in) { return __builtin_amdgcn_update_dpp(in, v, 0x138, 0xf, 0xf, false); }
+__device__ __forceinline__ int vmx_shl1_in(int v, int in) { return __builtin_amdgcn_update_dpp(in, v, 0x130, 0xf, 0xf, false); }
 __device__ __forceinline__ int vmx_rol1(int v) { return __builtin_amdgcn_update_dpp(v, v, 0x134, 0xf, 0xf, false); }
 __device__ __forceinline__ int vmx_ror1(int v) { return __builtin_amdgcn_update_dpp(v, v, 0x13C, 0xf, 0xf, false); }
 #endif
diff --git a/vacmap_amd/csrc/vmx_dp_ad.h b/vacmap_amd/csrc/vmx_dp_ad.h
--- a/vacmap_amd/csrc/vmx_dp_ad.h
+++ b/vacmap_amd/csrc/vmx_dp_ad.h
@@ -16,6 +16,10 @@
 __device__ __forceinline__ int vmx_r16_shl1_in(int v, int in) { return __builtin_amdgcn_update_dpp(in, v, 0x101, 0xf, 0xf, false); }
 __device__ __forceinline__ unsigned vmx_perm(unsigned s0, unsigned s1, unsigned sel) { return __builtin_amdgcn_perm(s0, s1, sel); }
 #endif
+template <int LW> __device__ __forceinline__ int vmx_ad_shl1_in(int v, int in) { if constexpr (LW == 16) return vmx_r16_shl1_in(v, in); else return vmx_shl1_in(v, in); }
+template <int LW> __device__ __forceinline__ int vmx_ad_shr1_in(int v, int in) { if constexpr (LW == 16) return vmx_r16_shr1_in(v, in); else return vmx_shr1_in(v, in); }
+template <int LW> __device__ __forceinline__ int vmx_ad_rol1(int v) { if constexpr (LW == 16) return vmx_r16_rol1(v); else return vmx_rol1(v); }
+template <int LW> __device__ __forceinline__ int vmx_ad_ror1(int v) { if constexpr (LW == 16) return vmx_r16_ror1(v); else return vmx_ror1(v); }
 
 #define VMX_AD_NEGINF (-4096)
 #define VMX_AD_CSH 12
@@ -77,11 +81,11 @@
     return r;
 }
 
-template <int NS>
+template <int NS, int LW = 16>
 __device__ __forceinline__ void vmx_gapfill_fill_ad(const uint8_t* __restrict__ TX, const uint8_t* __restrict__ QX, int tlX, int qlX, int dloX, uint8_t* __restrict__ tbX,
                                                    const uint8_t* __restrict__ TY, const uint8_t* __restrict__ QY, int tlY, int qlY, int dloY, uint8_t* __restrict__ tbY,
                                                    int match, int mismatch, int o1, int e1, int o2, int e2, int lane, int& scoreX, int& scoreY) {
-    const int l = lane & 15;
+    const int l = LW == 16 ? lane & 15 : lane;
     vmx_ad_consts K;
     K.O1 = vmx_pk(8 * o1, 8 * o1); K.O2 = vmx_pk(8 * o2, 8 * o2); K.E1 = vmx_pk(8 * e1, 8 * e1); K.E2 = vmx_pk(8 * e2, 8 * e2);
     K.MATCH = vmx_pk(8 * match, 8 * match); K.PEN = vmx_pk(8 * (match - mismatch), 8 * (match - mismatch));
@@ -117,36 +121,48 @@
     const int lfX = xfX / (2 * NS), kfX = (xfX % (2 * NS)) >> 1, lfY = xfY / (2 * NS), kfY = (xfY % (2 * NS)) >> 1;
     int finX = 0, finY = 0;
     constexpr int W = VMX_AD_W(NS);
-    uint8_t* const pX = tbX + VMX_AD_TB_OFF_W(0, l, W);
-    uint8_t* const pY = tbY + VMX_AD_TB_OFF_W(0, l, W);
+    uint8_t* const pX = LW == 16 ? tbX + VMX_AD_TB_OFF_W(0, l, W) : tbX;
+    uint8_t* const pY = LW == 16 ? tbY + VMX_AD_TB_OFF_W(0, l, W) : tbY;
     auto put = [&](uint8_t* at, unsigned w01, unsigned w23, bool hi) {
         if constexpr (W == 1) *at = (uint8_t)(hi ? (w01 >> 16) : w01);
         else if constexpr (W == 2) *(uint16_t*)at = (uint16_t)(hi ? (w01 >> 16) : w01);
         else *(uint32_t*)at = vmx_perm(w23, w01, hi ? 0x07060302u : 0x05040100u);
     };
+    auto put_pk = [&](uint8_t* tb, int tl, int ql, int a, int i1, unsigned w01, unsigned w23, bool hi) {
+        const int lo = a - 1 - ql > 0 ? a - 1 - ql : 0, n = (tl < a - 1 ? tl : a - 1) - lo;
+        const int sb = (int)((unsigned)(128 * (ql - 2)) << 8) >> 8, ab = 128 * (a - 2);
+#pragma unroll
+        for (int k = 0; k < NS; ++k) {
+            const int ik = i1 - k;
+            if ((unsigned)(ik - lo) < (unsigned)n && n > 0) {
+                const unsigned w = k < 2 ? w01 : w23;
+                tb[(unsigned)(((ik >> 7) & 7) * sb + (ab + ik))] = (uint8_t)(w >> (8 * (k & 1) + (hi ? 16 : 0)));
+            }
+        }
+    };
     auto load_chunks = [&](int b16, unsigned& tch, unsigned& qch) {
         tch = vmx_pk(tcf(TX, tlX, b16 + 1 + l - hX), tcf(TY, tlY, b16 + 1 + l - hY));
-        qch = vmx_pk(qcf(QX, qlX, b16 + 15 - l + hX + 16 * NS), qcf(QY, qlY, b16 + 15 - l + hY + 16 * NS));
+        qch = vmx_pk(qcf(QX, qlX, b16 + (LW - 1) - l + hX + LW * NS), qcf(QY, qlY, b16 + (LW - 1) - l + hY + LW * NS));
     };
     unsigned tch, qch, ntch, nqch;
     load_chunks(0, ntch, nqch);
-    for (int p0 = 0; p0 < npairs; p0 += 16) {
+    for (int p0 = 0; p0 < npairs; p0 += LW) {
         tch = ntch; qch = nqch;
-        load_chunks(p0 + 16, ntch, nqch);
-        int pend = npairs - p0; if (pend > 16) pend = 16;
+        load_chunks(p0 + LW, ntch, nqch);
+        int pend = npairs - p0; if (pend > LW) pend = LW;
         for (int pp = 0; pp < pend; ++pp) {
             const int p = p0 + pp + 1;
             {
-                const unsigned in = (unsigned)vmx_r16_shl1_in((int)qcode[0], (int)qch);
+                const unsigned in = (unsigned)vmx_ad_shl1_in<LW>((int)qcode[0], (int)qch);
 #pragma unroll
                 for (int k = 0; k + 1 < NS; ++k) qcode[k] = qcode[k + 1];
                 qcode[NS - 1] = in;
-                qch = (unsigned)vmx_r16_ror1((int)qch);
+                qch = (unsigned)vmx_ad_ror1<LW>((int)qch);
             }
             unsigned w[NS][5];
             {
-                const unsigned nH = (unsigned)vmx_r16_shl1_in((int)HA[0], (int)K.NH), nE1 = (unsigned)vmx_r16_shl1_in((int)E1A[0], (int)K.NE1),
-                               nE2 = (unsigned)vmx_r16_shl1_in((int)E2A[0], (int)K.NE2);
+                const unsigned nH = (unsigned)vmx_ad_shl1_in<LW>((int)HA[0], (int)K.NH), nE1 = (unsigned)vmx_ad_shl1_in<LW>((int)E1A[0], (int)K.NE1),
+                               nE2 = (unsigned)vmx_ad_shl1_in<LW>((int)E2A[0], (int)K.NE2);
 #pragma unroll
                 for (int k = 0; k < NS; ++k) {
                     const unsigned uH = k + 1 < NS ? HA[k + 1 < NS ? k + 1 : 0] : nH, uE1 = k + 1 < NS ? E1A[k + 1 < NS ? k + 1 : 0] : nE1, uE2 = k + 1 < NS ? E2A[k + 1 < NS ? k + 1 : 0] : nE2;
@@ -156,20 +172,25 @@
             {
                 unsigned w01, w23;
                 vmx_ad_pack<NS>(w, w01, w23);
+                if constexpr (LW == 16) {
                 const size_t so = VMX_AD_TB_OFF_W(2 * p - 2, 0, W);
                 if (p <= poX) put(pX + so, w01, w23, false);
                 if (p <= poY) put(pY + so, w01, w23, true);
-            }
-            {
-                const unsigned in = (unsigned)vmx_r16_shr1_in((int)tcode[NS - 1], (int)tch);
+                } else {
+                    if (p <= poX) put_pk(pX, tlX, qlX, 2 * p - 1, p - 2 - hX - NS * l, w01, w23, false);
+                    if (p <= poY) put_pk(pY, tlY, qlY, 2 * p - 1, p - 2 - hY - NS * l, w01, w23, true);
+                }
+            }
+            {
+                const unsigned in = (unsigned)vmx_ad_shr1_in<LW>((int)tcode[NS - 1], (int)tch);
 #pragma unroll
                 for (int k = NS - 1; k > 0; --k) tcode[k] = tcode[k - 1];
                 tcode[0] = in;
-                tch = (unsigned)vmx_r16_rol1((int)tch);
-            }
-            {
-                const unsigned nH = (unsigned)vmx_r16_shr1_in((int)HC[NS - 1], (int)K.NH), nF1 = (unsigned)vmx_r16_shr1_in((int)F1C[NS - 1], (int)K.NF1),
-                               nF2 = (unsigned)vmx_r16_shr1_in((int)F2C[NS - 1], (int)K.NF2);
+                tch = (unsigned)vmx_ad_rol1<LW>((int)tch);
+            }
+            {
+                const unsigned nH = (unsigned)vmx_ad_shr1_in<LW>((int)HC[NS - 1], (int)K.NH), nF1 = (unsigned)vmx_ad_shr1_in<LW>((int)F1C[NS - 1], (int)K.NF1),
+                               nF2 = (unsigned)vmx_ad_shr1_in<LW>((int)F2C[NS - 1], (int)K.NF2);
 #pragma unroll
                 for (int k = 0; k < NS; ++k) {
                     const unsigned lH = k > 0 ? HC[k > 0 ? k - 1 : 0] : nH, lF1 = k > 0 ? F1C[k > 0 ? k - 1 : 0] : nF1, lF2 = k > 0 ? F2C[k > 0 ? k - 1 : 0] : nF2;
@@ -179,9 +200,14 @@
             {
                 unsigned w01, w23;
                 vmx_ad_pack<NS>(w, w01, w23);
+                if constexpr (LW == 16) {
                 const size_t so = VMX_AD_TB_OFF_W(2 * p - 1, 0, W);
                 if (p <= peX) put(pX + so, w01, w23, false);
                 if (p <= peY) put(pY + so, w01, w23, true);
+                } else {
+                    if (p <= peX) put_pk(pX, tlX, qlX, 2 * p, p - 1 - hX - NS * l, w01, w23, false);
+                    if (p <= peY) put_pk(pY, tlY, qlY, 2 * p, p - 1 - hY - NS * l, w01, w23, true);
+                }
             }
             if (__any(p == poX || p == poY)) {
                 const unsigned aX = vmx_ad_pick<NS>(HA, kfX), cX = vmx_ad_pick<NS>(HC, kfX), aY = vmx_ad_pick<NS>(HA, kfY), cY = vmx_ad_pick<NS>(HC, kfY);
@@ -191,8 +217,8 @@
             }
         }
     }
-    scoreX = __shfl(finX, (lane & 48) | (lfX & 15));
-    scoreY = __shfl(finY, (lane & 48) | (lfY & 15));
+    scoreX = __shfl(finX, LW == 16 ? (lane & 48) | (lfX & 15) : lfX & 63);
+    scoreY = __shfl(finY, LW == 16 ? (lane & 48) | (lfY & 15) : lfY & 63);
 }
 
 __device__ __forceinline__ bool vmx_ad_proven(int score, int tl, int ql, int g, int match, int o1, int e1, int o2, int e2) {
diff --git a/vacmap_amd/csrc/vmx_host.h b/vacmap_amd/csrc/vmx_host.h
--- a/vacmap_amd/csrc/vmx_host.h
+++ b/vacmap_amd/csrc/vmx_host.h
@@ -268,8 +268,10 @@
                                const int32_t* order, int32_t* counter);
 __global__ void k_gapfill_fill_ns(const uint8_t* tcodes, const uint8_t* qcodes, vmx_dp_prob* probs, int n_prob, int match,
                                   int mismatch, int o1, int e1, int o2, int e2, uint8_t* tb_pool, int32_t* bnd_pool, int32_t* out_score,
-                                  const int32_t* order, const int32_t* range, int32_t* counter, int32_t* redo_list, int32_t* redo_cnt, int redo_pass, int ad_pct,
-                                  uint8_t* redo_pool, unsigned long long* redo_bytes, const int32_t* n_ptr = nullptr, unsigned long long redo_cap = ~0ULL, int tb_by_ns = 0);
+                                  const int32_t* order, const int32_t* range, int32_t* counter, int32_t* redo_list, int32_t* redo_cnt, int ad_pct,
+                                  unsigned long long* redo_bytes, const int32_t* n_ptr = nullptr, unsigned long long redo_cap = ~0ULL, int tb_by_ns = 0);
+__global__ void k_gapfill_redo(const uint8_t* tcodes, const uint8_t* qcodes, const vmx_dp_prob* probs, int match, int mismatch, int o1, int e1, int o2, int e2,
+                               uint8_t* tb_pool, int32_t* bnd_pool, int32_t* out_score, int32_t* redo_list, int32_t* redo_cnt, uint8_t* redo_pool);
 static inline int vmx_ad_pct_env(int mode = 0) {
     int pct = mode == 1 ? 40 : 90, pmin = mode == 1 ? 40 : VMX_AD_PCT_MIN_DEFAULT;
     if (const char* e = getenv("VMX_AD_PCT")) { const int v = atoi(e); if (v >= 0 && v <= 60000) pct = v; }
diff --git a/vacmap_amd/csrc/vmx_kernels.h b/vacmap_amd/csrc/vmx_kernels.h
--- a/vacmap_amd/csrc/vmx_kernels.h
+++ b/vacmap_amd/csrc/vmx_kernels.h
@@ -130,9 +130,9 @@
 #define VMX_DP16X4_OK(tl, ql) ((tl) + (ql) <= VMX_DP16X4_MAX)
 #define VMX_X4_W(ql) ((((ql) + 31) + 15) & ~15)
 #define VMX_AD_NS_MAX 4
-__host__ __device__ static inline int vmx_ad_geom(int tl, int ql, int ns, int* dlo_out) {
+__host__ __device__ static inline int vmx_ad_geom_nd(int tl, int ql, int nd, int* dlo_out) {
     const int dl = ql - tl, lo = dl < 0 ? dl : 0, hi = dl > 0 ? dl : 0;
-    const int slack = 32 * ns - (hi - lo + 1);
+    const int slack = nd - (hi - lo + 1);
     if (slack < 0) return 0;
     int mb = slack / 2, dlo = lo - mb;
     if (dlo & 1) {
@@ -144,22 +144,34 @@
     const int ma = slack - mb;
     return (mb < ma ? mb : ma) + 1;
 }
+__host__ __device__ static inline int vmx_ad_geom(int tl, int ql, int ns, int* dlo_out) { return vmx_ad_geom_nd(tl, ql, 32 * ns, dlo_out); }
 __host__ __device__ static inline long long vmx_ad_margin(int g, int match, int o1, int e1, int o2, int e2) {
     const long long c1 = o1 + (long long)g * e1, c2 = o2 + (long long)g * e2;
     return (long long)match * g + 2 * (c1 < c2 ? c1 : c2);
 }
-__host__ __device__ static inline int vmx_ad_ns(int tl, int ql, int match, int o1, int e1, int o2, int e2, int pct, int pct_min) {
+__host__ __device__ static inline int vmx_ad_ns_nd(int tl, int ql, int match, int o1, int e1, int o2, int e2, int pct, int pct_min, int dpn, int ns_lo, int ns_hi) {
     if (tl <= 0 || ql <= 0) return 0;
     const int mn = tl < ql ? tl : ql;
     int dlo, g = 0;
-    for (int ns = 1; ns <= VMX_AD_NS_MAX; ++ns) {
-        g = vmx_ad_geom(tl, ql, ns, &dlo);
+    for (int ns = ns_lo; ns <= ns_hi; ++ns) {
+        g = vmx_ad_geom_nd(tl, ql, dpn * ns, &dlo);
         if (g >= 1 && (g > mn || vmx_ad_margin(g, match, o1, e1, o2, e2) * 100 >= (long long)pct * mn)) return ns;
     }
-    return (g >= 1 && vmx_ad_margin(g, match, o1, e1, o2, e2) * 100 >= (long long)pct_min * mn) ? VMX_AD_NS_MAX : 0;
+    return (g >= 1 && vmx_ad_margin(g, match, o1, e1, o2, e2) * 100 >= (long long)pct_min * mn) ? ns_hi : 0;
+}
+__host__ __device__ static inline int vmx_ad_ns(int tl, int ql, int match, int o1, int e1, int o2, int e2, int pct, int pct_min) {
+    return vmx_ad_ns_nd(tl, ql, match, o1, e1, o2, e2, pct, pct_min, 32, 1, VMX_AD_NS_MAX);
 }
 #define VMX_AD_PCT_DEFAULT 100
 #define VMX_AD_PCT_MIN_DEFAULT 65
+#ifdef VMX_EMU
+#define VMX_ADW_DPN 36
+#else
+#define VMX_ADW_DPN 128
+#endif
+#define VMX_ADW_NS_MIN 2
+#define VMX_ADW_PCT 100
+#define VMX_ADW_PCT_MIN 65
 #define VMX_AD_FLAG 16
 #define VMX_PK_FLAG 1
 #ifdef VMX_EMU
diff --git a/vacmap_amd/lib.py b/vacmap_amd/lib.py
--- a/vacmap_amd/lib.py
+++ b/vacmap_amd/lib.py
@@ -68,7 +68,8 @@
                                           'dp_string_bytes')] + \
                [('ms_total', C.c_double), ('ms_stage', C.c_double * 16), ('ms_gapfill_fill', C.c_double), ('ms_gapfill_trace', C.c_double),
                 ('n_gapfill_launches', C.c_int64), ('n_ed_full', C.c_int64), ('n_ed_tier2', C.c_int64), ('n_ed_tier1', C.c_int64),
-                ('n_dp_redo', C.c_int64), ('dp_redo_tb_bytes', C.c_int64), ('ms_local_seed', C.c_double), ('ms_cluster', C.c_double), ('n_host_syncs', C.c_int64), ('n_local_general', C.c_int64), ('n_ext_retries', C.c_int64), ('n_batch_retries', C.c_int64)]
+                ('n_dp_redo', C.c_int64), ('dp_redo_tb_bytes', C.c_int64), ('ms_local_seed', C.c_double), ('ms_cluster', C.c_double), ('n_host_syncs', C.c_int64), ('n_local_general', C.c_int64), ('n_ext_retries', C.c_int64), ('n_batch_retries', C.c_int64),
+                ('n_dp_redo_wide', C.c_int64), ('n_dp_redo_full', C.c_int64)]
 
 
 def _b(s):
@@ -304,14 +305,15 @@
         t, to = _cat(targets); q, qo = _cat(queries)
         n = len(targets)
         sc = Score(match, mismatch, o1, e1, o2, e2)
-        cg = C.c_void_p(); co = C.POINTER(C.c_int64)(); fl = C.POINTER(C.c_int32)(); st = (C.c_int64 * 4)()
+        cg = C.c_void_p(); co = C.POINTER(C.c_int64)(); fl = C.POINTER(C.c_int32)(); st = (C.c_int64 * 6)()
         self.lib.check(self.lib.L.vm_k_cigar_batch_banded(self.h, C.byref(sc), int(eqx), n, t, to.ctypes.data, q, qo.ctypes.data,
                                                           C.byref(cg), C.byref(co), C.byref(fl), st))
         off = self._take(co, n + 1, np.int64)
         blob = C.string_at(cg.value, int(off[-1])) if off[-1] else b''
         self.lib.L.vm_free(cg)
         cigars = [blob[off[i]:off[i + 1] - 1].decode() for i in range(n)]
-        return cigars, self._take(fl, n, np.int32), {'eligible': st[0], 'proven': st[1], 'redo': st[2], 'not_eligible': st[3]}
+        return cigars, self._take(fl, n, np.int32), {'eligible': st[0], 'proven': st[1], 'redo': st[2], 'not_eligible': st[3],
+                                                          'redo_wide': st[4], 'redo_full': st[5]}
 
     def k_cigar(self, target, query, match=2, mismatch=-4, gap_open_1=4, gap_extend_1=2, gap_open_2=24, gap_extend_2=1,
                 bw=-1, zdropvalue=-1, eqx=False):
```

Result: faster. 3.508, median of 6 (+3.6%).
